# Kyaw-Thiha/animal-vision

Hardware: AMD Instinct MI355X
Metric: megapixels/sec per-frame pipeline (higher is better)
Workload: dtype f16

## Files before the change

animal-vision_amd/_lib.py:

```python
from __future__ import annotations

import ctypes
import os

_HERE = os.path.dirname(os.path.abspath(__file__))
LIB_PATH = os.path.join(_HERE, "libavx.so")

AVX_OK = 0
AVX_ERR_INVALID, AVX_ERR_NO_DEVICE, AVX_ERR_HIP, AVX_ERR_UNSUPPORTED, AVX_ERR_NOMEM = -1, -2, -3, -4, -5
AVX_COLOR_MATRIX, AVX_COLOR_CAT_MERGE = 0, 1
AVX_POST_NONE, AVX_POST_GAUSS, AVX_POST_ROWGAIN, AVX_POST_STREAK = 0, 1, 2, 3
AVX_MAX_KSIZE = 33
AVX_PIX_FMTS = {"yuv420p": 0, "nv12": 1, "yuv422p": 2, "yuv444p": 3, "gray": 4, "yuv420p10le": 5, "yuv422p10le": 6, "yuv444p10le": 7,
                "p010le": 8}
AVX_TRANSFERS = {"pq": 1, "hlg": 2}
AVX_TONEMAPS = {"clip": 0, "mobius": 1}


class AvxError(RuntimeError):
    def __init__(self, code: int, msg: str):
        super().__init__(f"libavx error {code}: {msg}")
        self.code = code


# ... 9 lines not shown
        ("ksize", ctypes.c_int32),
        ("taps_host", ctypes.POINTER(ctypes.c_double)),
        ("row_gain_host", ctypes.POINTER(ctypes.c_float)),
        ("row_gain_clamp", ctypes.c_int32),
        ("chroma_enable", ctypes.c_int32),
        ("chroma_keep", ctypes.c_float),
        ("variant", ctypes.c_int32),
        ("streak_rows_host", ctypes.POINTER(ctypes.c_float)),
        ("streak_stride", ctypes.c_int32),
        ("in_f32", ctypes.c_int32),
    ]


class DichromatLaunchInfo(ctypes.Structure):

    _fields_ = [("struct_size", ctypes.c_uint32)] + [
        (n, ctypes.c_int32)
        for n in ("family", "R", "f64", "NG", "spec", "sw", "nstrips", "ch", "nchunks", "xcd_remap", "narrow", "tuned_now", "grid", "per_cu")
    ]


AVX_LAUNCH_FAMILIES = ("none", "reference", "tiled", "march", "streak")


class HoneybeeDesc(ctypes.Structure):

    _fields_ = [
        ("struct_size", ctypes.c_uint32),
        ("source", ctypes.c_int32),
        ("rgb_matrix", ctypes.c_float * 9),
        ("hsi", ctypes.c_void_p),
        ("hsi_layout", ctypes.c_int32),
        ("hsi_dtype", ctypes.c_int32),
        ("bands", ctypes.c_int32),
        ("weights_host", ctypes.POINTER(ctypes.c_float)),
        ("adaptation", ctypes.c_int32),
        ("eps", ctypes.c_float),
        ("blur_ksize", ctypes.c_int32),
        ("blur_taps_host", ctypes.POINTER(ctypes.c_double)),
        ("mapping", ctypes.c_int32),
        ("custom_matrix", ctypes.c_float * 9),
        ("mixed_alpha", ctypes.c_float),
        ("out_float", ctypes.c_int32),
        ("catches", ctypes.c_void_p),
        ("catch_partials", ctypes.c_void_p),
        ("n_catch_partials", ctypes.c_int32),
    ]


_fp, _dp = ctypes.POINTER(ctypes.c_float), ctypes.POINTER(ctypes.c_double)


class MantisDesc(ctypes.Structure):

    _fields_ = [
        ("struct_size", ctypes.c_uint32),
        ("n_bands", ctypes.c_int32),
        ("band_matrix_host", _fp),
        ("band_lut_host", _fp),
        ("n_wavelengths", ctypes.c_int32),
        ("lobe_gains_host", _fp),
        ("lobe_denom", ctypes.c_float),
        ("band_weights_host", _fp),
        ("pano_new_w", ctypes.c_int32),
        ("hsi_small_h", ctypes.c_int32),
        ("hsi_small_w", ctypes.c_int32),
        ("red_keep", ctypes.c_float),
        ("haze", ctypes.c_float),
        ("haze_keep", ctypes.c_float),
        ("haze_tint", ctypes.c_float * 3),
        ("pre_soft_ksize", ctypes.c_int32),
        ("pre_soft_taps_host", _dp),
        ("cos2_global", ctypes.c_float),
        ("sin2_global", ctypes.c_float),
        ("orientation_mix", ctypes.c_float),
        ("pol_linear_strength", ctypes.c_float),
        ("pol_linear_gamma", ctypes.c_float),
        ("pol_circular_strength", ctypes.c_float),
        ("unsharp_ksize", ctypes.c_int32),
        ("unsharp_taps_host", _dp),
        ("unsharp_amount", ctypes.c_float),
        ("barcode_saturation", ctypes.c_float),
        ("barcode_opacity", ctypes.c_float),
        ("winner_take_most", ctypes.c_float),
        ("rows_host", _fp),
        ("scan_row_gain", ctypes.c_float),
        ("scan_ksize", ctypes.c_int32),
        ("scan_taps_host", _dp),
        ("periph_ksize", ctypes.c_int32),
        ("periph_taps_host", _dp),
        ("xx_host", _fp),
        ("yy_host", _fp),
        ("periph_radius", ctypes.c_float),
        ("periph_softness", ctypes.c_float),
        ("lin_hwc_in", ctypes.c_void_p),
        ("out_float", ctypes.c_int32),
    ]


class BandStackDesc(ctypes.Structure):

    _fields_ = [
        ("struct_size", ctypes.c_uint32),
        ("n_bands", ctypes.c_int32),
        ("band_matrix_host", _fp),
        ("n_wavelengths", ctypes.c_int32),
        ("lobe_gains_host", _fp),
        ("lobe_denom", ctypes.c_float),
        ("band_weights_host", _fp),
        ("small_h", ctypes.c_int32),
        ("small_w", ctypes.c_int32),
    ]


class GalleryTile(ctypes.Structure):

    _fields_ = [
        ("src", ctypes.c_void_p),
        ("dtype", ctypes.c_int32),
        ("H", ctypes.c_int32),
        ("W", ctypes.c_int32),
        ("h", ctypes.c_int32),
        ("w", ctypes.c_int32),
        ("seg_offset", ctypes.c_int32),
        ("seg_count", ctypes.c_int32),
    ]


class FrameMetricsRecord(ctypes.Structure):

    _fields_ = [("abs_hist", (ctypes.c_uint32 * 256) * 3), ("ssim", ctypes.c_double * 3)]


AVX_METRICS_MAX_FRAMES = 16


class PlaneMetricsRecord(ctypes.Structure):

    _fields_ = [("abs_hist", (ctypes.c_uint32 * 1024) * 3), ("ssim", ctypes.c_double * 3)]


assert ctypes.sizeof(PlaneMetricsRecord) == 3 * 1024 * 4 + 3 * 8


class MsSsimRecord(ctypes.Structure):

    _fields_ = [("cs", (ctypes.c_double * 5) * 3), ("ssim", (ctypes.c_double * 5) * 3)]


assert ctypes.sizeof(MsSsimRecord) == 240

class EwInsn(ctypes.Structure):
    _fields_ = [("op", ctypes.c_uint8), ("dst", ctypes.c_uint8), ("a", ctypes.c_uint8), ("b", ctypes.c_uint8), ("imm", ctypes.c_uint32)]


class EwPlane(ctypes.Structure):
    _fields_ = [("ptr", ctypes.c_void_p), ("stride", ctypes.c_int32), ("kind", ctypes.c_int32)]


class EwProgram(ctypes.Structure):

    _fields_ = [
        ("struct_size", ctypes.c_uint32),
        ("H", ctypes.c_int32),
        ("W", ctypes.c_int32),
        ("n_insn", ctypes.c_int32),
        ("insn_host", ctypes.POINTER(EwInsn)),
        ("n_planes", ctypes.c_int32),
        ("planes_host", ctypes.POINTER(EwPlane)),
        ("n_acc", ctypes.c_int32),
        ("acc_host", ctypes.POINTER(ctypes.c_int32)),
        ("scalars_dev", ctypes.c_void_p),
        ("n_scalars", ctypes.c_int32),
    ]


AVX_EW_MAX_INSN, AVX_EW_MAX_PLANES, AVX_EW_MAX_REGS, AVX_EW_MAX_ACC = 384, 24, 32, 16
AVX_EW_MAX_FRAMES = 16
_EW_OPS = ("CONST SCALAR LOAD STORE ADD SUB MUL DIV MIN MAX POW ATAN2 NEG ABS SQRT EXP LOG SIN COS FLOOR CEIL CLIP01 TANH "
           "LT LE GT GE EQ AND OR NOT SELECT ACCMIN ACCMAX ACCSUM").split()
EW = {name: i + 1 for i, name in enumerate(_EW_OPS)}
EW_PLANE = {"f32": 0, "u8": 1, "u8_lut": 2, "col": 3, "row": 4, "u8_enc": 5}
EW_ACC = {"min": 0, "max": 1, "sum": 2, "mean": 3}

AVX_MAP = {"falsecolor": 0, "custom_matrix": 1, "opponent": 2, "uv_purple_yellow": 3, "falsecolor_uv_mixed": 4}

if not os.path.exists(LIB_PATH):
    raise ImportError(
        f"{LIB_PATH} not found: build it with `python -c 'import __graft_entry__ as g; g.build()'` "
        "or `make -C animal-vision_amd/csrc` (hipcc --offload-arch=gfx950). There is no CPU fallback."
    )


def _preload_torch_hip_runtime():
    import importlib.util

    try:
        spec = importlib.util.find_spec("torch")
    except (ImportError, ValueError):
        spec = None
    if spec is None or not spec.submodule_search_locations:
        return
    cand = os.path.join(list(spec.submodule_search_locations)[0], "lib", "libamdhip64.so")
    if os.path.exists(cand):
        try:
            ctypes.CDLL(cand, mode=ctypes.RTLD_GLOBAL)
        except OSError:
            pass


_preload_torch_hip_runtime()
lib = ctypes.CDLL(LIB_PATH)

_vp, _i, _sz = ctypes.c_void_p, ctypes.c_int, ctypes.c_size_t
_SIGS = {
    "avx_abi_version": (_i, []),
    "avx_device_count": (_i, []),
    "avx_init": (_i, [_i, ctypes.POINTER(_vp)]),
    "avx_destroy": (None, [_vp]),
    "avx_last_error": (ctypes.c_char_p, [_vp]),
    "avx_malloc": (_i, [_vp, _sz, ctypes.POINTER(_vp)]),
    "avx_free": (_i, [_vp, _vp]),
    "avx_host_alloc": (_i, [_vp, _sz, ctypes.POINTER(_vp)]),
    "avx_host_free": (_i, [_vp, _vp]),
    "avx_memcpy_h2d": (_i, [_vp, _vp, _vp, _sz, _vp]),
    "avx_memcpy_d2h": (_i, [_vp, _vp, _vp, _sz, _vp]),
    "avx_memcpy_d2d": (_i, [_vp, _vp, _vp, _sz, _vp]),
    "avx_memset": (_i, [_vp, _vp, _i, _sz, _vp]),
    "avx_stream_create": (_i, [_vp, ctypes.POINTER(_vp)]),
    "avx_stream_destroy": (_i, [_vp, _vp]),
    "avx_sync": (_i, [_vp, _vp]),
    "avx_stream_wait": (_i, [_vp, _vp, _vp]),
    "avx_device_sync": (_i, [_vp]),
    "avx_timer_start": (_i, [_vp, _vp]),
    "avx_timer_stop": (_i, [_vp, _vp, ctypes.POINTER(ctypes.c_float)]),
    "avx_dichromat_u8": (_i, [_vp, _vp, _vp, _i, _i, _i, ctypes.POINTER(DichromatDesc), _vp]),
    "avx_dichromat_last_launch": (_i, [_vp, ctypes.POINTER(DichromatLaunchInfo)]),
    "avx_get_table": (_i, [_i, _vp, _sz]),
    "avx_percentile": (_i, [_vp, _vp, _sz, ctypes.c_double, ctypes.POINTER(ctypes.c_double), _vp]),
    "avx_spectral_integrate": (_i, [_vp, _vp, _i, _i, _i, _i, _i, _vp, _i, _vp, _vp, _vp]),
    "avx_plane_stats": (_i, [_vp, _vp, _i, _sz, _i, ctypes.c_float, _vp, _vp]),
    "avx_planes_gaussian_blur": (_i, [_vp, _vp, _vp, _i, _i, _i, _i, _vp, _i, _vp]),
    "avx_planes_gaussian_blur_batch": (_i, [_vp, _vp, _sz, _vp, _sz, _i, _i, _i, _i, _i, _vp, _i, _vp]),
    "avx_streak_planes_f32": (_i, [_vp, _vp, _vp, _i, _i, _vp, _i, _vp]),
    "avx_rgb_to_hsi_lobes": (_i, [_vp, _vp, _i, _i, _i, _i, _vp, ctypes.c_float, _vp, _vp]),
    "avx_honeybee_u8": (_i, [_vp, _vp, _vp, _i, _i, _i, ctypes.POINTER(HoneybeeDesc), _vp, _vp]),
    "avx_catch_planes_up": (_i, [_vp, _vp, _i, _i, _vp, _i, _i, _vp, ctypes.POINTER(ctypes.c_int), _vp]),
    "avx_uv_front_u8": (_i, [_vp, _vp, _i, _i, _i, _vp, _vp, _vp]),
    "avx_uv_front_u8_batch": (_i, [_vp, _vp, _i, _sz, _i, _i, _i, _vp, _sz, _vp, _sz, _vp]),
    "avx_panorama_warp_f32": (_i, [_vp, _vp, _i, _i, _i, _vp, _vp]),
    "avx_band_stack": (_i, [_vp, _vp, _i, _i, ctypes.POINTER(BandStackDesc), _vp, _vp]),
    "avx_band_stack_batch": (_i, [_vp, _vp, _i, _sz, _i, _i, ctypes.POINTER(BandStackDesc), _vp, _sz, _vp]),
    "avx_percentile_dev": (_i, [_vp, _vp, _sz, ctypes.c_double, _vp, _vp]),
    "avx_percentiles_dev": (_i, [_vp, _i, ctypes.POINTER(ctypes.c_void_p), ctypes.POINTER(ctypes.c_size_t), ctypes.POINTER(ctypes.c_double),
                                 ctypes.POINTER(ctypes.c_void_p), _vp]),
    "avx_ew_run": (_i, [_vp, ctypes.POINTER(EwProgram), _vp]),
    "avx_ew_run_batch": (_i, [_vp, ctypes.POINTER(EwProgram), _i, ctypes.POINTER(ctypes.c_size_t), _sz, _vp]),
    "avx_ew_spec_stats": (_i, [ctypes.POINTER(ctypes.c_ulonglong), ctypes.POINTER(ctypes.c_ulonglong)]),
    "avx_mantis_u8": (_i, [_vp, _vp, _vp, _vp, _i, _i, ctypes.POINTER(MantisDesc), _vp]),
    "avx_mantis_u8_batch": (_i, [_vp, _vp, _vp, _vp, _i, _i, _i, ctypes.POINTER(MantisDesc), _vp]),
    "avx_resize_hwc": (_i, [_vp, _vp, _i, _i, _i, _i, _vp, _i, _i, _i, _vp]),
    "avx_binocular_warp_u8": (_i, [_vp, _vp, _i, _i, _vp, _vp, _vp, _vp, _vp, _i, _i, _vp, _vp]),
    "avx_cat_wide_u8": (_i, [_vp, _vp, _vp, _i, _i, _i, ctypes.POINTER(DichromatDesc), _vp, _vp, _vp, _vp, _vp, _vp]),
    "avx_center_zoom_u8": (_i, [_vp, _vp, _vp, _i, _i, _i, _i, _i, _i, _i, _vp]),
    "avx_split_compose_u8": (_i, [_vp, _vp, _vp, _vp, _i, _i, _i, _vp]),
    "avx_draw_label_u8": (_i, [_vp, _vp, _i, _i, ctypes.POINTER(ctypes.c_int), _fp, _i, ctypes.c_float, ctypes.c_float, _i, _vp]),
    "avx_gallery_compose_u8": (_i, [_vp, ctypes.POINTER(GalleryTile), _i, _fp, _i, _i, _i, _i, ctypes.POINTER(ctypes.c_int), _vp, _i, _i, _vp]),
    "avx_wall_max_tiles": (_i, []),
    "avx_wall_layout_create": (_i, [_vp, _i, _i, _i, _i, _i, ctypes.POINTER(ctypes.c_int), ctypes.POINTER(ctypes.c_int), _fp, _i, _i, _i, _i,
                                    ctypes.POINTER(ctypes.c_int), ctypes.POINTER(_vp)]),
    "avx_wall_layout_destroy": (_i, [_vp, _vp]),
    "avx_wall_canvas_size": (_i, [_vp, ctypes.POINTER(_i), ctypes.POINTER(_i)]),
    "avx_wall_layout_info": (_i, [_vp, ctypes.POINTER(_i), ctypes.POINTER(_i), ctypes.POINTER(_i), ctypes.POINTER(_sz)]),
    "avx_wall_compose_u8": (_i, [_vp, _vp, ctypes.POINTER(_vp), _sz, _i, _vp, _sz, _vp]),
    "avx_i420_to_rgb_u8": (_i, [_vp, _vp, _vp, _i, _i, _i, _i, _i, _vp]),
    "avx_rgb_to_i420_u8": (_i, [_vp, _vp, _vp, _i, _i, _i, _i, _i, _vp]),
    "avx_yuv_coefficients": (_i, [_i, _i, ctypes.POINTER(ctypes.c_int), ctypes.POINTER(ctypes.c_int)]),
    "avx_yuv_coefficients_d": (_i, [_i, _i, _i, ctypes.POINTER(ctypes.c_int), ctypes.POINTER(ctypes.c_int)]),
    "avx_yuv_frame_size": (_sz, [_i, _i, _i]),
    "avx_yuv_to_rgb_u8": (_i, [_vp, _i, _vp, _vp, _i, _i, _i, _i, _i, _vp]),
    "avx_rgb_to_yuv_u8": (_i, [_vp, _i, _vp, _vp, _i, _i, _i, _i, _i, _vp]),
    "avx_yuv_hdr_to_rgb_u8": (_i, [_vp, _i, _vp, _vp, _i, _i, _i, _i, _i, _i, ctypes.c_double, ctypes.c_double, _vp]),
    "avx_yuv_to_rgb_scaled_u8": (_i, [_vp, _i, _vp, _vp, _i, _i, _i, _i, _i, _i, _i, _vp]),
    "avx_yuv_hdr_to_rgb_scaled_u8": (_i, [_vp, _i, _vp, _vp, _i, _i, _i, _i, _i, _i, _i, _i, ctypes.c_double, ctypes.c_double, _vp]),
    "avx_frame_metrics_u8": (_i, [_vp, _vp, _vp, _i, _i, _i, _i, _vp, _vp]),
    "avx_plane_metrics": (_i, [_vp, _i, _vp, _i, _vp, _i, _i, _i, _i, _vp, _vp]),
    "avx_frame_metrics_ms_u8": (_i, [_vp, _vp, _vp, _i, _i, _i, _vp, _vp, _vp]),
    "avx_remap_linear_planes": (_i, [_vp, _vp, _i, _i, _i, _vp, _vp, _vp, ctypes.c_float, _vp]),
    "avx_sobel3_plane": (_i, [_vp, _vp, _i, _i, _vp, _vp, _vp]),
    "avx_mst_gram": (_i, [_vp, _vp, _i, _sz, _i, _i, _vp, _vp, _vp, _vp]),
    "avx_mst_qkv_gram": (_i, [_vp, _vp, _vp, _sz, _i, _vp, _vp, _vp, _vp, _vp]),
    "avx_mst_qkv_gram16": (_i, [_vp, _vp, _vp, _sz, _i, _vp, _vp, _vp, _vp, _vp]),
    "avx_mst_ln_gemm_gelu": (_i, [_vp, _vp, _vp, _vp, ctypes.c_float, _vp, _sz, _i, _vp, _vp]),
    "avx_mst_convt2x2": (_i, [_vp, _vp, _vp, _vp, _vp, _i, _i, _i, _i, _vp]),
    "avx_mst_convt2x2_fuse": (_i, [_vp, _vp, _vp, _vp, _vp, _vp, _vp, _i, _i, _i, _i, _vp]),
    "avx_mst_posemb": (_i, [_vp, _vp, _vp, _vp, _vp, _vp, _vp, _i, _i, _i, _i, _vp]),
    "avx_mst_conv3x3_add": (_i, [_vp, _vp, _vp, _vp, _vp, _i, _i, _i, _i, _vp]),
    "avx_mst_attn_pack": (_i, [_vp, _vp, _vp, _vp, _vp, _vp, _i, _vp, _vp]),
    "avx_mst_rowgemm_add": (_i, [_vp, _vp, _vp, _vp, _vp, _vp, _vp, _sz, _i, _vp]),
    "avx_mst_conv_in_u8": (_i, [_vp, _vp, _i, _i, _i, _i, _i, _i, _vp, _vp, _vp]),
    "avx_mst_conv3x3_lds": (_i, [_vp, _vp, _vp, _vp, _vp, _i, _i, _i, _i, _vp]),
    "avx_mst_down4x4": (_i, [_vp, _vp, _vp, _vp, _i, _i, _i, _i, _vp]),
    "avx_mst_conv3x3_lds_gram": (_i, [_vp, _vp, _vp, _vp, _vp, _i, _i, _i, _vp, _vp, _vp, _vp, _vp]),
    "avx_mst_convt2x2_fuse_gram": (_i, [_vp, _vp, _vp, _vp, _vp, _vp, _vp, _i, _i, _i, _vp, _vp, _vp, _vp, _vp]),
    "avx_mst_attn_pack16": (_i, [_vp, _vp, _vp, _vp, _vp, _vp, _i, _vp, _vp]),
    "avx_mst_attn_pack_mx": (_i, [_vp, _vp, _vp, _vp, _vp, _vp, _i, _vp, _vp]),
    "avx_mst_attn_tail_mx": (_i, [_vp, _vp, _vp, _vp, _vp, _vp, _vp, _vp, _i, _i, _i, _i, _vp]),
    "avx_mst_attn_tail_sp": (_i, [_vp, _vp, _vp, _vp, _vp, _vp, _vp, _vp, _i, _i, _i, _i, _vp]),
    "avx_mst_attn_tail": (_i, [_vp, _vp, _vp, _vp, _vp, _vp, _vp, _vp, _i, _i, _i, _i, _vp]),
    "avx_mst_attn_tail_x": (_i, [_vp, _vp, _vp, _vp, _vp, _vp, _vp, _vp, _i, _i, _i, _i, _vp]),
    "avx_mst_ffn_fused": (_i, [_vp, _vp, _vp, _vp, ctypes.c_float, _vp, _vp, _vp, _vp, _i, _i, _i, _i, _vp]),
    "avx_mst_conv3x3_lds_spectral": (_i, [_vp, _vp, _vp, _vp, _i, _i, _i, _fp, _i, _i, _i, _i, _vp, _vp, ctypes.POINTER(ctypes.c_int), _vp]),
    "avx_mst_ffn_fused_mx": (_i, [_vp, _vp, _vp, _vp, ctypes.c_float, _vp, _vp, _vp, _vp, _i, _i, _i, _i, _vp]),
    "avx_mst_ffn_fused_sp": (_i, [_vp, _vp, _vp, _vp, ctypes.c_float, _vp, _vp, _vp, _vp, _i, _i, _i, _i, _vp]),
    "avx_mst_gelu_prescale": (ctypes.c_float, []),
    "avx_mst_tile_order": (_i, [_i, _i, _i, _i, _i, ctypes.POINTER(ctypes.c_longlong), _i, ctypes.POINTER(ctypes.c_int)]),
    "avx_mst_dw_gemm_add": (_i, [_vp, _vp, _vp, _vp, _vp, _vp, _i, _i, _i, _i, _vp]),
    "avx_dwconv3x3_nhwc_add": (_i, [_vp, _vp, _vp, _vp, _i, _i, _i, _i, _i, _vp, _vp, _vp]),
    "avx_dwconv3x3_nhwc": (_i, [_vp, _vp, _vp, _vp, _i, _i, _i, _i, _i, _i, _vp]),
    "avx_layernorm_rows": (_i, [_vp, _vp, _vp, _vp, _vp, _i, _sz, _i, ctypes.c_float, _vp]),
    "avx_layernorm_rows_grouped": (_i, [_vp, _vp, _vp, _vp, _vp, _i, _sz, _i, ctypes.c_float, _i, _i, _vp]),
}
for _name, (_res, _args) in _SIGS.items():
    _fn = getattr(lib, _name)
    _fn.restype = _res
    _fn.argtypes = _args

if lib.avx_abi_version() != 1:
    raise ImportError(f"libavx.so ABI {lib.avx_abi_version()} != 1 expected by this package: rebuild")
```

animal-vision_amd/csrc/mst_fused.hip:

```cpp
#include <hip/hip_fp16.h>

#include <cstdio>
#include <cstdlib>
#include <cstring>

#include "avx_internal.h"
#include "mst_common.h"
#include "mst_tile_order.h"

namespace {

typedef float float4_t __attribute__((ext_vector_type(4)));
#ifndef AVX_FFN32_GM2
#define AVX_FFN32_GM2 1
#endif
constexpr int kFT = 512;
constexpr int TS = 16;
constexpr int HS = TS + 2;
#ifndef AVX_FFN_TH
#define AVX_FFN_TH 16
#endif
constexpr int kFfnTH = AVX_FFN_TH;
static_assert(kFfnTH == 14 || kFfnTH == 16, "FeedForward tile rows");
constexpr int kFfnNGRP = (HS * (kFfnTH + 2) + 31) / 32;
// ... 614 lines not shown
}

template <int C, int MINW>
int launch_attn_tail(avx_ctx* ctx, const void* v, const void* x, const void* mpack, const void* taps1, const void* taps2, const float* bias, void* out, int B,
                     int H, int W, hipStream_t s, const void* wvpack) {
    constexpr int PP = C * 2 + 16, VRP = (VS * PP + 255) / 256 * 256, MRP = VRP;
    const size_t lds = (size_t)2 * VS * VRP + (size_t)2 * 9 * C * 2 + sizeof(float) * C;
    (void)MRP;
    const long total = (long)B * ((H + TS - 1) / TS) * ((W + TS - 1) / TS);
    const long cap = (long)ctx->num_cus * (MINW / 2);
    auto k = k_mst_attn_tail<C, MINW>;
    AVX_HIP(ctx, hipFuncSetAttribute((const void*)k, hipFuncAttributeMaxDynamicSharedMemorySize, (int)lds));
    hipLaunchKernelGGL(k, dim3((unsigned)(total < cap ? total : cap)), dim3(kFT), lds, s, (const __half*)v, (const __half*)x, (const uint4*)mpack,
                       (const __half*)taps1, (const __half*)taps2, bias, (__half*)out, B, H, W, (const uint4*)wvpack);
    AVX_HIP(ctx, hipGetLastError());
    return AVX_OK;
}


template <int C, int TR, int MINW, bool STAMP = false, int NW = 8, bool DWS = false>
__global__ __launch_bounds__(64 * NW, MINW) void k_mst_attn_tail_mx(const __half* __restrict__ x , const uint4* __restrict__ wvpack ,
                                                                const uint4* __restrict__ mpack , const uint4* __restrict__ dw1 ,
                                                                const uint4* __restrict__ dw2 , const float* __restrict__ bias ,
                                                                __half* __restrict__ out, int B, int H, int W, unsigned long long* __restrict__ stamps , int order ) {
    constexpr int TW = 14, VW = 18, VR = TR + 4, MR = TR + 2, NOCT = C / 8, NK = C / 16, NT = C / 32, NS = C / 16, LNV = C / 16;
    constexpr int PP = C * 2 + 16, RP = (VW * PP + 255) / 256 * 256, MP = 16 * PP;
    constexpr int NTHR = 64 * NW, NG = (VR * VW + 31) / 32, NGW = (NG + NW - 1) / NW;
    constexpr int WPO = NOCT >= NW ? 1 : NW / NOCT, OPW = NOCT > NW ? NOCT / NW : 1;
    constexpr int NOUT = (TR / 2) / WPO, NMID = NOUT + 1;
    static_assert(C == 32 || C == 64 || C == 128, "31-, 62- or 124-channel blocks");
    static_assert(MP % 256 == 0 && (NW % NOCT == 0 || NOCT % NW == 0) && (TR / 2) % WPO == 0, "pitches / row split");
    extern __shared__ __align__(16) unsigned char smem[];
    unsigned char* vt = smem;
    unsigned char* mt = vt + (size_t)VR * RP;
    uint4* wvl = reinterpret_cast<uint4*>(mt + (size_t)MR * MP);
    constexpr bool STASH = C <= 64 && NW == 8;
    unsigned char* xs = reinterpret_cast<unsigned char*>(wvl + NT * NS * 64);
    const int tid = threadIdx.x, lane = tid & 63, wave = tid >> 6, p = lane & 31, h = lane >> 5, n16 = lane & 15, q = lane >> 4;
    unsigned long long seg[8] = {0, 0, 0, 0, 0, 0, 0, 0}, tlast = 0;
    auto stamp = [&](int kk) {
        if constexpr (STAMP) {
            const unsigned long long now = __builtin_readcyclecounter();
            seg[kk] += now - tlast;
            tlast = now;
        }
    };
    if constexpr (STAMP) tlast = __builtin_readcyclecounter();
    const int tx = (W + TW - 1) / TW, ty = (H + TR - 1) / TR;
    for (int i = tid; i < NT * NS * 64; i += NTHR) wvl[i] = wvpack[i];
    const int o = wave % NOCT, rpo = (wave / NOCT) * NOUT;
    half8_t a1[3], a2[3], am[NK];
    float bs[4];
    auto load_frags = [&](int oc) {
#pragma unroll
        for (int i = 0; i < 3; ++i) {
            a1[i] = dw_frag<DWS>(dw1 + ((size_t)oc * 3 + i) * 64 + lane, i);
            a2[i] = dw_frag<DWS>(dw2 + ((size_t)oc * 3 + i) * 64 + lane, i);
        }
#pragma unroll
        for (int t2 = 0; t2 < NK; ++t2) am[t2] = __builtin_bit_cast(half8_t, mpack[((size_t)oc * NK + t2) * 64 + lane]);
#pragma unroll
        for (int j = 0; j < 4; ++j) bs[j] = bias ? bias[8 * oc + 4 * (q & 1) + j] : 0.f;
    };
    load_frags(o);
#pragma unroll
    for (int i = 0; i < 3; ++i) asm volatile("" ::"v"(a1[i]), "v"(a2[i]));
#pragma unroll
    for (int t2 = 0; t2 < NK; ++t2) asm volatile("" ::"v"(am[t2]));
    asm volatile("" ::"v"(bs[0]), "v"(bs[1]), "v"(bs[2]), "v"(bs[3]));
    const unsigned char* rbB = vt + (size_t)q * RP + (size_t)n16 * PP + 16 * o;
    unsigned char* wbB = mt + (size_t)(q >> 1) * MP + (size_t)n16 * PP + 16 * o + 8 * (q & 1);
    const unsigned char* rbC = mt + (size_t)q * MP + (size_t)n16 * PP + 16 * o;
    const unsigned char* rbG = vt + (size_t)(2 + (q & 1)) * RP + (size_t)(n16 + 2) * PP + 16 * (q >> 1);
    unsigned f_rel[NGW];
    int v_dst[NGW], p_row[NGW], p_col[NGW];
#pragma unroll
    for (int gi = 0; gi < NGW; ++gi) {
        const int g = wave + NW * gi, qq = 32 * g + p, qc = qq < VR * VW ? qq : VR * VW - 1;
        p_row[gi] = qc / VW; p_col[gi] = qc % VW;
        f_rel[gi] = (unsigned)((p_row[gi] * W + p_col[gi]) * C + h * (C / 2)) * 2u;
        v_dst[gi] = (g < NG && qq < VR * VW) ? p_row[gi] * RP + p_col[gi] * PP + 32 * h : -1;
    }
    uint4 pre[NGW][LNV];
    auto fetch = [&](const Tile& t) {
        if (t.y0 >= 2 && t.y0 + VR - 2 <= H && t.x0 >= 2 && t.x0 + VW - 2 <= W) {
            const char* origin = reinterpret_cast<const char*>(x + ((t.b * H + t.y0 - 2) * (size_t)W + t.x0 - 2) * C);
#pragma unroll
            for (int gi = 0; gi < NGW; ++gi) {
                if (wave + NW * gi >= NG) break;
                unsigned of = f_rel[gi];
                asm volatile("" : "+v"(of));
                const uint4* src = reinterpret_cast<const uint4*>(origin + of);
#pragma unroll
                for (int v = 0; v < LNV; ++v) pre[gi][v] = src[v];
            }
            return;
        }
#pragma unroll
        for (int gi = 0; gi < NGW; ++gi) {
            if (wave + NW * gi >= NG) break;
            const int yy = t.y0 - 2 + p_row[gi], xx = t.x0 - 2 + p_col[gi];
            const bool ok = yy >= 0 && yy < H && xx >= 0 && xx < W;
            const int yc = yy < 0 ? 0 : (yy >= H ? H - 1 : yy), xc = xx < 0 ? 0 : (xx >= W ? W - 1 : xx);
            const uint4* src = reinterpret_cast<const uint4*>(x + ((t.b * H + yc) * (size_t)W + xc) * C + h * (C / 2));
#pragma unroll
            for (int v = 0; v < LNV; ++v) {
                uint4 r = src[v];
                r.x = ok ? r.x : 0u; r.y = ok ? r.y : 0u; r.z = ok ? r.z : 0u; r.w = ok ? r.w : 0u;
                pre[gi][v] = r;
            }
        }
    };
    TileWalk ahead;
    ahead.init(blockIdx.x, gridDim.x, B, ty, tx, order);
    if (!ahead.live) return;
    Tile t = tile_at(ahead, TW, TR);
    ahead.advance();
    fetch(t);
    __syncthreads();
    for (;;) {
#pragma unroll
        for (int gi = 0; gi < NGW; ++gi) {
            if (wave + NW * gi >= NG) break;
#pragma unroll
            for (int nt = 0; nt < NT; ++nt) {
                float16_t d;
#pragma unroll
                for (int vv = 0; vv < 16; ++vv) d[vv] = 0.f;
#pragma unroll
                for (int s2 = 0; s2 < NS; ++s2) d = mfma16(__builtin_bit_cast(half8_t, wvl[(nt * NS + s2) * 64 + lane]), __builtin_bit_cast(half8_t, pre[gi][s2]), d);
                if (v_dst[gi] >= 0) {
                    half8_t w0, w1;
#pragma unroll
                    for (int vv = 0; vv < 8; ++vv) { w0[vv] = (_Float16)d[vv]; w1[vv] = (_Float16)d[8 + vv]; }
                    reinterpret_cast<uint4*>(vt + v_dst[gi] + 64 * nt)[0] = __builtin_bit_cast(uint4, w0);
                    reinterpret_cast<uint4*>(vt + v_dst[gi] + 64 * nt)[1] = __builtin_bit_cast(uint4, w1);
                }
            }
            if constexpr (STASH) {
                const unsigned sr = (unsigned)(p_row[gi] - 2), sc = (unsigned)(p_col[gi] - 2);
                if (v_dst[gi] >= 0 && sr < (unsigned)TR && sc < (unsigned)TW) {
                    unsigned char* dst = xs + (sr * TW + sc) * PP + h * C;
#pragma unroll
                    for (int v = 0; v < LNV; ++v) *reinterpret_cast<uint4*>(dst + 16 * v) = pre[gi][v];
                }
            }
        }
        stamp(0);
        __syncthreads();
        stamp(1);
        if (ahead.live) fetch(tile_at(ahead, TW, TR));
#pragma unroll
        for (int kk = 0; kk < OPW; ++kk) {
        const int oc = o + NW * kk, ob = 16 * NW * kk;
        if constexpr (OPW > 1) load_frags(oc);
        uint2 xr[STASH ? 1 : NOUT];
        const int yo0 = t.y0 + 2 * rpo + (q >> 1), xo = t.x0 + n16;
        const bool livex = n16 < TW && xo < W;
        const size_t e0 = ((t.b * H + (yo0 < H ? yo0 : 0)) * (size_t)W + (livex ? xo : 0)) * C + 8 * oc + 4 * (q & 1), estep = (size_t)2 * W * C;
        auto live = [&](int u) { return livex && yo0 + 2 * u < H; };
        if constexpr (!STASH) {
#pragma unroll
            for (int u = 0; u < NOUT; ++u) xr[u] = live(u) ? *reinterpret_cast<const uint2*>(x + e0 + u * estep) : uint2{0, 0};
        }
        {
            const bool mid_inside = t.y0 >= 1 && t.y0 + MR - 1 <= H && t.x0 >= 1 && t.x0 + 15 <= W;
            uint4 bq[3];
            auto rd = [&](int u) {
#pragma unroll
                for (int i = 0; i < 3; ++i) bq[i] = *reinterpret_cast<const uint4*>(rbB + (size_t)(2 * (rpo + u)) * RP + i * PP + ob);
            };
            auto finish = [&](int u, float4_t a) {
                float2_t gp[2] = {float2_t{a[0], a[1]}, float2_t{a[2], a[3]}};
                if constexpr (C >= 64) gelu_mx<2>(gp);
                else { float2_t g0[1] = {gp[0]}, g1[1] = {gp[1]}; gelu_mx<1>(g0); gelu_mx<1>(g1); gp[0] = g0[0]; gp[1] = g1[0]; }
                uint2 ov = uint2{pack_f16(gp[0].x, gp[0].y), pack_f16(gp[1].x, gp[1].y)};
                if (!mid_inside) {
                    const int yy = t.y0 - 1 + 2 * (rpo + u) + (q >> 1), xx = t.x0 - 1 + n16;
                    const unsigned keep = (yy >= 0 && yy < H && xx >= 0 && xx < W) ? 0xffffffffu : 0u;
                    ov.x &= keep; ov.y &= keep;
                }
                *reinterpret_cast<uint2*>(wbB + (size_t)(2 * (rpo + u)) * MP + ob) = ov;
            };
            rd(0);
            float4_t prev = {0.f, 0.f, 0.f, 0.f};
#pragma unroll
            for (int u = 0; u < NMID; ++u) {
                const float4_t acc = dw_unit<DWS>(a1, bq);
                if (u + 1 < NMID) rd(u + 1);
                __builtin_amdgcn_sched_barrier(0);
                if (u > 0) finish(u - 1, prev);
                __builtin_amdgcn_sched_barrier(0);
                prev = acc;
            }
            finish(NMID - 1, prev);
        }
        stamp(2);
        {
            uint4 bq[3], bg[NK];
            uint2 xn = uint2{0, 0};
            const unsigned char* rbX = xs + (size_t)((q >> 1) * TW + n16) * PP + 16 * o + 8 * (q & 1);
            auto rd = [&](int u) {
#pragma unroll
                for (int i = 0; i < 3; ++i) bq[i] = *reinterpret_cast<const uint4*>(rbC + (size_t)(2 * (rpo + u)) * MP + i * PP + ob);
#pragma unroll
                for (int t2 = 0; t2 < NK; ++t2) bg[t2] = *reinterpret_cast<const uint4*>(rbG + (size_t)(2 * (rpo + u)) * RP + 32 * t2);
                if constexpr (STASH) xn = *reinterpret_cast<const uint2*>(rbX + (size_t)(2 * (rpo + u)) * TW * PP);
            };
            auto finish = [&](int u, float4_t acc, uint2 xu) {
                if (live(u)) {
                    constexpr unsigned kOnes = 0x3c003c00u;
                    float s0 = acc[0] + bs[0], s1 = acc[1] + bs[1], s2 = acc[2] + bs[2], s3 = acc[3] + bs[3];
                    fma_mix_lo(s0, xu.x, kOnes); fma_mix_hi(s1, xu.x, kOnes);
                    fma_mix_lo(s2, xu.y, kOnes); fma_mix_hi(s3, xu.y, kOnes);
                    *reinterpret_cast<uint2*>(out + e0 + u * estep) = uint2{pack_f16(s0, s1), pack_f16(s2, s3)};
                }
            };
            rd(0);
#ifndef AVX_TAIL_PIPE2
#define AVX_TAIL_PIPE2 1
#endif
            if constexpr (STASH && (AVX_TAIL_PIPE2 == 2 || (AVX_TAIL_PIPE2 == 1 && C == 64))) {
                float4_t prev = {0.f, 0.f, 0.f, 0.f};
                uint2 xp = uint2{0, 0};
#pragma unroll
                for (int u = 0; u < NOUT; ++u) {
                    const uint2 xu = xn;
                    float4_t acc = dw_unit<DWS>(a2, bq);
#pragma unroll
                    for (int t2 = 0; t2 < NK; ++t2) acc = __builtin_amdgcn_mfma_f32_16x16x32_f16(am[t2], __builtin_bit_cast(half8_t, bg[t2]), acc, 0, 0, 0);
                    if (u + 1 < NOUT) rd(u + 1);
                    __builtin_amdgcn_sched_barrier(0);
                    if (u > 0) finish(u - 1, prev, xp);
                    __builtin_amdgcn_sched_barrier(0);
                    prev = acc; xp = xu;
                }
                finish(NOUT - 1, prev, xp);
            } else {
#pragma unroll
                for (int u = 0; u < NOUT; ++u) {
                    const uint2 xu = STASH ? xn : xr[STASH ? 0 : u];
                    float4_t acc = dw_unit<DWS>(a2, bq);
#pragma unroll
                    for (int t2 = 0; t2 < NK; ++t2) acc = __builtin_amdgcn_mfma_f32_16x16x32_f16(am[t2], __builtin_bit_cast(half8_t, bg[t2]), acc, 0, 0, 0);
                    if (u + 1 < NOUT) rd(u + 1);
                    finish(u, acc, xu);
                }
            }
        }
        }
        stamp(3);
        if (!ahead.live) break;
        t = tile_at(ahead, TW, TR);
        ahead.advance();
        __syncthreads();
        stamp(4);
    }
    if constexpr (STAMP) {
        if (lane == 0 && stamps)
#pragma unroll
            for (int kk = 0; kk < 8; ++kk) stamps[((size_t)blockIdx.x * NW + wave) * 8 + kk] = seg[kk];
    }
}

template <int C, int TR, int MINW, int NW = 8, bool DWS = false>
int launch_attn_tail_mx(avx_ctx* ctx, const void* x, const void* wvpack, const void* mpack, const void* dw1, const void* dw2, const float* bias, void* out, int B, int H, int W,
                        hipStream_t s) {
    constexpr int PP = C * 2 + 16, RP = (18 * PP + 255) / 256 * 256;
    const size_t lds = (size_t)(TR + 4) * RP + (size_t)(TR + 2) * 16 * PP + (size_t)(C / 32) * (C / 16) * 1024 + ((C <= 64 && NW == 8) ? (size_t)(TR * 14 + 2) * PP : 0) ;
    const long total = (long)B * ((H + TR - 1) / TR) * ((W + 13) / 14);
    const long cap = (long)ctx->num_cus * (NW == 16 ? 1 : MINW / 2);
    AVX_REQUIRE(ctx, total <= 0x7fffffffl, "avx_mst_attn_tail_mx: 2^31 tiles or more");
    const unsigned blocks = (unsigned)(total < cap ? total : cap);
    if (getenv("AVX_TAIL_STAMPS")) {
        auto ks = k_mst_attn_tail_mx<C, TR, MINW, true, NW, DWS>;
        unsigned long long* d_st = nullptr;
        const size_t n = (size_t)blocks * NW * 8;
        AVX_HIP(ctx, hipMalloc((void**)&d_st, n * sizeof(unsigned long long)));
        AVX_HIP(ctx, hipFuncSetAttribute((const void*)ks, hipFuncAttributeMaxDynamicSharedMemorySize, (int)lds));
        hipLaunchKernelGGL(ks, dim3(blocks), dim3(64 * NW), lds, s, (const __half*)x, (const uint4*)wvpack, (const uint4*)mpack, (const uint4*)dw1, (const uint4*)dw2, bias, (__half*)out, B, H, W, d_st, mst_tile_order());
        AVX_HIP(ctx, hipStreamSynchronize(s));
        unsigned long long* h_st = (unsigned long long*)malloc(n * sizeof(unsigned long long));
        AVX_HIP(ctx, hipMemcpy(h_st, d_st, n * sizeof(unsigned long long), hipMemcpyDeviceToHost));
        double tot[8] = {0}, all = 0;
        for (size_t i = 0; i < n; ++i) { tot[i & 7] += (double)h_st[i]; all += (double)h_st[i]; }
        const char* nm[8] = {"v from x", "bar1", "conv1+gelu", "conv2+proj+store", "bar2", "-", "-", "-"};
        fprintf(stderr, "[tail stamps C=%d] %u blocks, %ld tiles, mean cycles per wave %.0f:", C, blocks, total, all / (blocks * (double)NW));
        for (int k2 = 0; k2 < 8; ++k2) fprintf(stderr, "  %s %.1f%%", nm[k2], 100 * tot[k2] / all);
        fprintf(stderr, "\n");
        free(h_st);
        (void)hipFree(d_st);
        return AVX_OK;
    }
    auto k = k_mst_attn_tail_mx<C, TR, MINW, false, NW, DWS>;
    AVX_HIP(ctx, hipFuncSetAttribute((const void*)k, hipFuncAttributeMaxDynamicSharedMemorySize, (int)lds));
    hipLaunchKernelGGL(k, dim3(blocks), dim3(64 * NW), lds, s, (const __half*)x, (const uint4*)wvpack, (const uint4*)mpack, (const uint4*)dw1,
                       (const uint4*)dw2, bias, (__half*)out, B, H, W, (unsigned long long*)nullptr, mst_tile_order());
    AVX_HIP(ctx, hipGetLastError());
    return AVX_OK;
}


struct SpecStat3 { float mn, mx; double sum; };
template <int MINW, bool GRAM, bool SPEC = false>
__global__ __launch_bounds__(kFT, MINW) void k_mst_conv3x3_lds(const __half* __restrict__ x , const uint4* __restrict__ wpack ,
                                                               const __half* __restrict__ add , __half* __restrict__ out, int B, int H, int W,
                                                               const uint4* __restrict__ wqk , float* __restrict__ partial ,
                                                               const float* __restrict__ specw = nullptr ,
                                                               float* __restrict__ planes = nullptr , SpecStat3* __restrict__ spart = nullptr ,
                                                               int crop_t = 0, int crop_l = 0, int Hc = 0, int Wc = 0, int order = AVX_TILE_ORDER_RASTER ) {
    constexpr int C = 32, PP = C * 2 + 16, RP = (HS * PP + 255) / 256 * 256, NFILL = (HS * HS * 4 + kFT - 1) / kFT;
    __shared__ __align__(16) unsigned char xt[HS * RP];
    __shared__ uint4 wl[18 * 64];
    const int tid = threadIdx.x, lane = tid & 63, wave = tid >> 6, p = lane & 31, h = lane >> 5;
    for (int i = tid; i < 18 * 64; i += kFT) wl[i] = wpack[i];
    __shared__ uint4 wq[GRAM ? 4 * 64 : 1];
    float16_t G;
    float nq = 0.f, nk = 0.f;
    if constexpr (GRAM) {
        if (tid < 4 * 64) wq[tid] = wqk[tid];
#pragma unroll
        for (int v = 0; v < 16; ++v) G[v] = 0.f;
    }
    float smn[3] = {3.4e38f, 3.4e38f, 3.4e38f}, smx[3] = {-3.4e38f, -3.4e38f, -3.4e38f};
    double ssum[3] = {0.0, 0.0, 0.0};
    const int tx = (W + TS - 1) / TS, ty = (H + TS - 1) / TS;
    uint4 pre[NFILL];
    unsigned f_rel[NFILL];
#pragma unroll
    for (int k = 0; k < NFILL; ++k) {
        const int it = tid + k * kFT, itc = it < HS * HS * 4 ? it : 0, q = itc >> 2, part = itc & 3;
        f_rel[k] = (unsigned)(((q / HS) * W + q % HS) * C + 8 * part) * 2u;
    }
    auto fetch = [&](const Tile& t) {
        if (t.y0 >= 1 && t.y0 + HS - 1 <= H && t.x0 >= 1 && t.x0 + HS - 1 <= W) {
            const char* origin = reinterpret_cast<const char*>(x + ((t.b * H + t.y0 - 1) * (size_t)W + t.x0 - 1) * C);
#pragma unroll
            for (int k = 0; k < NFILL; ++k) {
                unsigned o = f_rel[k];
                asm volatile("" : "+v"(o));
                pre[k] = *reinterpret_cast<const uint4*>(origin + o);
            }
            return;
        }
#pragma unroll
        for (int k = 0; k < NFILL; ++k) {
            const int it = tid + k * kFT, q = it >> 2, part = it & 3;
            const int yy = t.y0 - 1 + q / HS, xx = t.x0 - 1 + q % HS;
            const bool ok = it < HS * HS * 4 && yy >= 0 && yy < H && xx >= 0 && xx < W;
            const int yc = yy < 0 ? 0 : (yy >= H ? H - 1 : yy), xc = xx < 0 ? 0 : (xx >= W ? W - 1 : xx);
            uint4 r = *reinterpret_cast<const uint4*>(x + ((t.b * H + yc) * (size_t)W + xc) * C + 8 * part);
            r.x = ok ? r.x : 0u; r.y = ok ? r.y : 0u; r.z = ok ? r.z : 0u; r.w = ok ? r.w : 0u;
            pre[k] = r;
        }
    };
    TileWalk ahead;
    ahead.init(blockIdx.x, gridDim.x, B, ty, tx, (GRAM || SPEC) ? (int)AVX_TILE_ORDER_RASTER : order);
    if (!ahead.live) return;
    Tile t = tile_at(ahead, TS, TS);
    ahead.advance();
    fetch(t);
    for (;;) {
#pragma unroll
        for (int k = 0; k < NFILL; ++k) {
            const int it = tid + k * kFT, q = it >> 2, part = it & 3;
            if (it < HS * HS * 4) *reinterpret_cast<uint4*>(xt + (size_t)(q / HS) * RP + (size_t)(q % HS) * PP + 16 * part) = pre[k];
        }
        __syncthreads();
        if (ahead.live) fetch(tile_at(ahead, TS, TS));
        {
            const int r = 2 * wave + (p >> 4), c = p & 15;
            const int yo = t.y0 + r, xo = t.x0 + c;
            const bool live = yo < H && xo < W;
            const size_t off = ((t.b * H + (live ? yo : 0)) * (size_t)W + (live ? xo : 0)) * C + 16 * h;
            uint4 ar[2] = {uint4{0, 0, 0, 0}, uint4{0, 0, 0, 0}};
            if (add) { ar[0] = reinterpret_cast<const uint4*>(add + off)[0]; ar[1] = reinterpret_cast<const uint4*>(add + off)[1]; }
            float16_t d;
#pragma unroll
            for (int v = 0; v < 16; ++v) d[v] = 0.f;
            const unsigned char* src = xt + (size_t)r * RP + (size_t)c * PP + 16 * h;
#pragma unroll
            for (int tap = 0; tap < 9; ++tap)
#pragma unroll
                for (int s2 = 0; s2 < 2; ++s2)
                    d = mfma16(__builtin_bit_cast(half8_t, wl[(2 * tap + s2) * 64 + lane]), __builtin_bit_cast(half8_t, *reinterpret_cast<const uint4*>(src + (size_t)(tap / 3) * RP + (size_t)(tap % 3) * PP + 32 * s2)), d);
            half8_t o0, o1;
            {
                const half8_t r0 = __builtin_bit_cast(half8_t, ar[0]), r1 = __builtin_bit_cast(half8_t, ar[1]);
#pragma unroll
                for (int v = 0; v < 8; ++v) { o0[v] = (_Float16)(d[v] + (float)r0[v]); o1[v] = (_Float16)(d[8 + v] + (float)r1[v]); }
            }
            if constexpr (SPEC) {
                float a3[3] = {0.f, 0.f, 0.f};
                auto chain = [&]() {
#pragma unroll
                    for (int j = 0; j < 16; ++j) {
                        const float v = (float)(j < 8 ? o0[j] : o1[j - 8]);
                        const float* wb = specw + (16 * h + j) * 4;
#pragma unroll
                        for (int k = 0; k < 3; ++k) a3[k] = __builtin_fmaf(v, wb[k], a3[k]);
                    }
                };
                if (h == 0) chain();
#pragma unroll
                for (int k = 0; k < 3; ++k) { const float lo = __shfl_xor(a3[k], 32); a3[k] = h ? lo : a3[k]; }
                if (h == 1) chain();
                const int yc = yo - crop_t, xc = xo - crop_l;
                if (h == 1 && live && yc >= 0 && yc < Hc && xc >= 0 && xc < Wc) {
#pragma unroll
                    for (int k = 0; k < 3; ++k) {
                        planes[(size_t)k * Hc * Wc + (size_t)yc * Wc + xc] = a3[k];
                        smn[k] = fminf(smn[k], a3[k]); smx[k] = fmaxf(smx[k], a3[k]); ssum[k] += (double)a3[k];
                    }
                }
            } else if (live) {
                reinterpret_cast<uint4*>(out + off)[0] = __builtin_bit_cast(uint4, o0);
                reinterpret_cast<uint4*>(out + off)[1] = __builtin_bit_cast(uint4, o1);
            }
            if constexpr (GRAM) {
                if (!live) { o0 = half8_t{0, 0, 0, 0, 0, 0, 0, 0}; o1 = o0; }
                float16_t dq, dk;
#pragma unroll
                for (int v = 0; v < 16; ++v) { dq[v] = 0.f; dk[v] = 0.f; }
                dq = mfma16(o0, __builtin_bit_cast(half8_t, wq[0 * 64 + lane]), dq);
                dq = mfma16(o1, __builtin_bit_cast(half8_t, wq[1 * 64 + lane]), dq);
                dk = mfma16(o0, __builtin_bit_cast(half8_t, wq[2 * 64 + lane]), dk);
                dk = mfma16(o1, __builtin_bit_cast(half8_t, wq[3 * 64 + lane]), dk);
                unsigned aq[8], ak[8];
#pragma unroll
                for (int j = 0; j < 8; ++j) {
                    aq[j] = pack_f16(dq[2 * j], dq[2 * j + 1]);
                    ak[j] = pack_f16(dk[2 * j], dk[2 * j + 1]);
                    fma_mix_lo(nq, aq[j], aq[j]); fma_mix_hi(nq, aq[j], aq[j]);
                    fma_mix_lo(nk, ak[j], ak[j]); fma_mix_hi(nk, ak[j], ak[j]);
                }
#pragma unroll
                for (int b2 = 0; b2 < 2; ++b2)
                    G = mfma16(__builtin_bit_cast(half8_t, uint4{ak[4 * b2], ak[4 * b2 + 1], ak[4 * b2 + 2], ak[4 * b2 + 3]}),
                               __builtin_bit_cast(half8_t, uint4{aq[4 * b2], aq[4 * b2 + 1], aq[4 * b2 + 2], aq[4 * b2 + 3]}), G);
            }
        }
        if (!ahead.live) break;
        t = tile_at(ahead, TS, TS);
        ahead.advance();
        __syncthreads();
    }
    if constexpr (SPEC) {
        __syncthreads();
        float* redf = reinterpret_cast<float*>(xt);
        double* redd = reinterpret_cast<double*>(xt + 256);
#pragma unroll
        for (int k = 0; k < 3; ++k) {
            float a = smn[k], b2 = smx[k];
            double c2 = ssum[k];
#pragma unroll
            for (int o = 32; o > 0; o >>= 1) { a = fminf(a, __shfl_xor(a, o)); b2 = fmaxf(b2, __shfl_xor(b2, o)); c2 += __shfl_xor(c2, o); }
            if (lane == 0) { redf[(wave * 3 + k) * 2] = a; redf[(wave * 3 + k) * 2 + 1] = b2; redd[wave * 3 + k] = c2; }
        }
        __syncthreads();
        if (tid < 3) {
            float a = 3.4e38f, b2 = -3.4e38f;
            double c2 = 0.0;
            for (int w8 = 0; w8 < 8; ++w8) { a = fminf(a, redf[(w8 * 3 + tid) * 2]); b2 = fmaxf(b2, redf[(w8 * 3 + tid) * 2 + 1]); c2 += redd[w8 * 3 + tid]; }
            spart[(size_t)blockIdx.x * 3 + tid] = SpecStat3{a, b2, c2};
        }
    }
    if constexpr (GRAM) {
        static_assert(sizeof(xt) >= sizeof(float) * 4 * 34 * 32, "the halo tile's LDS holds four waves' results at a time");
        float* red = reinterpret_cast<float*>(xt);
        const float sq = nq + __shfl_xor(nq, 32), sk = nk + __shfl_xor(nk, 32);
        float sum[3] = {0.f, 0.f, 0.f};
#pragma unroll
        for (int half = 0; half < 2; ++half) {
            __syncthreads();
            if ((wave >> 2) == half) {
                float* mine = red + (size_t)(wave & 3) * 34 * 32;
#pragma unroll
                for (int v = 0; v < 16; ++v) mine[(8 * (v / 4) + 4 * h + (v % 4)) * 32 + p] = G[v];
                if (h == 0) { mine[32 * 32 + p] = sq; mine[33 * 32 + p] = sk; }
            }
            __syncthreads();
#pragma unroll
            for (int q = 0; q < 3; ++q) {
                const int i = tid + q * kFT;
                if (i < 34 * 32)
#pragma unroll
                    for (int w4 = 0; w4 < 4; ++w4) sum[q] += red[(size_t)w4 * 34 * 32 + i];
            }
        }
#pragma unroll
        for (int q = 0; q < 3; ++q) {
            const int i = tid + q * kFT;
            if (i < 34 * 32) partial[(size_t)blockIdx.x * 34 * 32 + i] = sum[q];
        }
    }
}


template <int C>
struct DownGeo {
    static constexpr int OH = C == 32 ? 8 : 4, OW = 16, IH = 2 * OH + 2, IW = 2 * OW + 2;
    static constexpr int NP = C / 8;
    static constexpr int RPS = IW * NP + (C == 32 ? 2 : 4);
    static constexpr int NI = ((IH * RPS + 63) / 64 + 7) / 8 * 8;
    static constexpr int PER_WAVE = NI / 8, BUF = NI * 1024, NBUF = C == 32 ? 3 : 2, GROUPS = OH / 2;
    static constexpr int PART = C == 32 ? 0 : 2 * 4 * 4096;
    __device__ static int swz(int col) { return C == 32 ? (col >> 2) & 3 : (col >> 1) & 7; }
};
#pragma clang diagnostic push
#pragma clang diagnostic ignored "-Winline-asm"
__device__ __forceinline__ void lds_dma16(const void* g, unsigned lds_base ) {
    asm volatile("s_mov_b32 m0, %0\n\ts_nop 0\n\tglobal_load_lds_dwordx4 %1, off" ::"s"(__builtin_amdgcn_readfirstlane(lds_base)), "v"(g) : "memory", "m0");
}
__device__ __forceinline__ void lds_dma16(const void* base , unsigned ofs, unsigned lds_base) {
    asm volatile("s_mov_b32 m0, %0\n\ts_nop 0\n\tglobal_load_lds_dwordx4 %1, %2" ::"s"(__builtin_amdgcn_readfirstlane(lds_base)), "v"(ofs), "s"(base) : "memory", "m0");
}
#pragma clang diagnostic pop
template <int C>
__global__ __launch_bounds__(kFT, 2) void k_mst_down4x4_dma(const __half* __restrict__ x , const uint4* __restrict__ wpack ,
                                                            __half* __restrict__ out , const void* __restrict__ zero, int B, int H, int W, int order ) {
    using G = DownGeo<C>;
    constexpr int CO = 2 * C, NT = CO / 32, KS = C / 16;
    __shared__ __align__(1024) unsigned char lds[G::NBUF * G::BUF + G::PART];
    const int tid = threadIdx.x, lane = tid & 63, wave = __builtin_amdgcn_readfirstlane(tid >> 6) , p = lane & 31, h = lane >> 5;
    const int g0 = C == 32 ? wave & 3 : 0, nt = C == 32 ? wave >> 2 : wave & 3, kh = C == 32 ? 0 : wave >> 2;
    half8_t wf[32];
#pragma unroll
    for (int i = 0; i < 32; ++i) {
        const int tap = C == 32 ? i >> 1 : 8 * kh + (i >> 2), s2 = C == 32 ? i & 1 : i & 3;
        wf[i] = __builtin_bit_cast(half8_t, wpack[((size_t)(tap * NT + nt) * KS + s2) * 64 + lane]);
    }
    const int Ho = H / 2, Wo = W / 2;
    const int tx = (Wo + G::OW - 1) / G::OW, ty = (Ho + G::OH - 1) / G::OH;
    struct T2 { int ox0, oy0, b; };
    auto tile_at = [&](const TileWalk& w) { return T2{w.xi * G::OW, w.yi * G::OH, w.b}; };
    int rel[G::PER_WAVE], rc[G::PER_WAVE];
#pragma unroll
    for (int k = 0; k < G::PER_WAVE; ++k) {
        const int L = (wave + 8 * k) * 64 + lane, row = L / G::RPS, rem = L - row * G::RPS, col = rem / G::NP, j = (rem - col * G::NP) ^ G::swz(col);
        const bool inside = row < G::IH && col < G::IW;
        rel[k] = inside ? (row * W + col) * (C * 2) + 16 * j : 0;
        rc[k] = inside ? row << 8 | col : -1;
    }
    const unsigned lds0 = __builtin_amdgcn_readfirstlane((unsigned)(size_t)(__attribute__((address_space(3))) unsigned char*)lds);
    auto fill = [&](const TileWalk& w, int slot) {
        const bool exists = w.live;
        const T2 t = tile_at(w);
        const int y0 = 2 * t.oy0 - 1, x0 = 2 * t.ox0 - 1;
        const char* origin = reinterpret_cast<const char*>(x) + (((long)t.b * H + y0) * W + x0) * (long)(C * 2);
        const unsigned lb = lds0 + slot * G::BUF + wave * 1024;
        if (exists && y0 >= 0 && y0 + G::IH <= H && x0 >= 0 && x0 + G::IW <= W) {
#pragma unroll
            for (int k = 0; k < G::PER_WAVE; ++k) lds_dma16(origin , (unsigned)rel[k], lb + k * 8192);
        } else {
#pragma unroll
            for (int k = 0; k < G::PER_WAVE; ++k) {
                const int yy = y0 + (rc[k] >> 8), xx = x0 + (rc[k] & 255);
                const bool ok = exists && rc[k] >= 0 && yy >= 0 && yy < H && xx >= 0 && xx < W;
                lds_dma16(ok ? (const void*)(origin + rel[k]) : zero, lb + k * 8192);
            }
        }
    };
    TileWalk walk, look;
    walk.init(blockIdx.x, gridDim.x, B, ty, tx, order);
    if (!walk.live) return;
    look = walk;
#pragma unroll
    for (int a = 0; a < G::NBUF - 1; ++a) { fill(look, a); look.advance(); }
    const int c2 = 2 * (p & 15);
    int colofs[4];
#pragma unroll
    for (int kx = 0; kx < 4; ++kx) colofs[kx] = (c2 + kx) * G::NP;
    int slot = 0, plain_stores = 0;
    for (;;) {
        if (plain_stores == G::NBUF - 1 && (C == 32 || kh == 0)) asm volatile("s_waitcnt vmcnt(%0)" ::"n"(G::PER_WAVE * (G::NBUF - 2) + 2 * (C == 32 ? 1 : G::GROUPS) * (G::NBUF - 1)) : "memory");
        else asm volatile("s_waitcnt vmcnt(%0)" ::"n"(G::PER_WAVE * (G::NBUF - 2)) : "memory");
        __syncthreads();
        {
            int nslot = slot + G::NBUF - 1;
            nslot -= nslot >= G::NBUF ? G::NBUF : 0;
            fill(look, nslot);
            look.advance();
        }
        const T2 t = tile_at(walk);
        const bool whole = t.oy0 + G::OH <= Ho && t.ox0 + G::OW <= Wo;
        const unsigned char* bt = lds + slot * G::BUF;
#pragma unroll 1
        for (int g = g0; g < (C == 32 ? g0 + 1 : G::GROUPS); ++g) {
            const int r = 2 * g + (p >> 4);
            float16_t d, d1;
#pragma unroll
            for (int v = 0; v < 16; ++v) d[v] = 0.f, d1[v] = 0.f;
            const unsigned char* src = bt + (size_t)(2 * r) * (G::RPS * 16);
            auto frag = [&](int i) {
                const int tap = C == 32 ? i >> 1 : 8 * kh + (i >> 2), s2 = C == 32 ? i & 1 : i & 3, ky = tap >> 2, kx = tap & 3;
                return *reinterpret_cast<const uint4*>(src + ky * (G::RPS * 16) + (colofs[kx] + ((2 * s2 + h) ^ G::swz(c2 + kx))) * 16);
            };
            constexpr int AHEAD = 6;
            uint4 bq[AHEAD];
#pragma unroll
            for (int i = 0; i < AHEAD; ++i) bq[i] = frag(i);
#pragma unroll
            for (int i = 0; i < 32; ++i) {
                if (i & 1) d1 = mfma16(wf[i], __builtin_bit_cast(half8_t, bq[i % AHEAD]), d1);
                else d = mfma16(wf[i], __builtin_bit_cast(half8_t, bq[i % AHEAD]), d);
                if (i + AHEAD < 32) bq[i % AHEAD] = frag(i + AHEAD);
            }
            __builtin_amdgcn_sched_group_barrier(0x100, AHEAD, 0);
#pragma unroll
            for (int i = 0; i < 32; ++i) {
                __builtin_amdgcn_sched_group_barrier(0x008, 1, 0);
                if (i + AHEAD < 32) __builtin_amdgcn_sched_group_barrier(0x100, 1, 0);
            }
#pragma unroll
            for (int v = 0; v < 16; ++v) d[v] += d1[v];
            if constexpr (C == 64) {
                float4* part = reinterpret_cast<float4*>(lds + G::NBUF * G::BUF + ((g & 1) * 4 + nt) * 4096);
                if (kh == 1) {
#pragma unroll
                    for (int v4 = 0; v4 < 4; ++v4) part[v4 * 64 + lane] = float4{d[4 * v4], d[4 * v4 + 1], d[4 * v4 + 2], d[4 * v4 + 3]};
                }
                __syncthreads();
                if (kh == 1) continue;
#pragma unroll
                for (int v4 = 0; v4 < 4; ++v4) {
                    const float4 q = part[v4 * 64 + lane];
                    d[4 * v4] += q.x; d[4 * v4 + 1] += q.y; d[4 * v4 + 2] += q.z; d[4 * v4 + 3] += q.w;
                }
            }
            const int yo = t.oy0 + r, xo = t.ox0 + (p & 15);
            half8_t o0, o1;
#pragma unroll
            for (int v = 0; v < 8; ++v) { o0[v] = (_Float16)d[v]; o1[v] = (_Float16)d[8 + v]; }
            __half* dst = out + (((size_t)t.b * Ho + yo) * Wo + xo) * CO + 32 * nt + 16 * h;
            if (whole) {
                reinterpret_cast<uint4*>(dst)[0] = __builtin_bit_cast(uint4, o0);
                reinterpret_cast<uint4*>(dst)[1] = __builtin_bit_cast(uint4, o1);
            } else if (yo < Ho && xo < Wo) {
                reinterpret_cast<uint4*>(dst)[0] = __builtin_bit_cast(uint4, o0);
                reinterpret_cast<uint4*>(dst)[1] = __builtin_bit_cast(uint4, o1);
            }
        }
        plain_stores = whole ? (plain_stores < G::NBUF - 1 ? plain_stores + 1 : plain_stores) : 0;
        walk.advance();
        if (!walk.live) break;
        slot = slot + 1 == G::NBUF ? 0 : slot + 1;
    }
    asm volatile("s_waitcnt vmcnt(0)" ::: "memory");
}

__global__ __launch_bounds__(256) void k_mst_conv_in_u8(const uint8_t* __restrict__ frame , const float* __restrict__ w ,
                                                        __half* __restrict__ out , int H, int W, int pt, int pl, int Hp, int Wp) {
    __shared__ __align__(16) float wl[27 * 32];
    for (int i = threadIdx.x; i < 27 * 32; i += 256) wl[i] = w[i];
    __syncthreads();
    const size_t total = (size_t)Hp * Wp;
    for (size_t i = (size_t)blockIdx.x * 256 + threadIdx.x; i < total; i += (size_t)gridDim.x * 256) {
        const int y = (int)(i / Wp), x = (int)(i - (size_t)y * Wp);
        float in[27];
#pragma unroll
        for (int t = 0; t < 9; ++t) {
            const int yy = y + t / 3 - 1, xx = x + t % 3 - 1;
            const bool ok = yy >= 0 && yy < Hp && xx >= 0 && xx < Wp;
            int sy = (ok ? yy : 0) - pt, sx = (ok ? xx : 0) - pl;
            sy = sy < 0 ? -sy : (sy >= H ? 2 * (H - 1) - sy : sy);
            sx = sx < 0 ? -sx : (sx >= W ? 2 * (W - 1) - sx : sx);
            const uint8_t* q = frame + ((size_t)sy * W + sx) * 3;
#pragma unroll
            for (int c = 0; c < 3; ++c) in[3 * t + c] = ok ? (float)(_Float16)((float)q[c] / 255.0f) : 0.f;
        }
        uint4* dst = reinterpret_cast<uint4*>(out + i * 32);
#pragma unroll 1
        for (int v = 0; v < 4; ++v) {
            float acc[8];
#pragma unroll
            for (int j = 0; j < 8; ++j) acc[j] = 0.f;
#pragma unroll
            for (int k = 0; k < 27; ++k) {
                const float4 wa = *reinterpret_cast<const float4*>(wl + k * 32 + 8 * v), wb = *reinterpret_cast<const float4*>(wl + k * 32 + 8 * v + 4);
                acc[0] = __builtin_fmaf(in[k], wa.x, acc[0]); acc[1] = __builtin_fmaf(in[k], wa.y, acc[1]);
                acc[2] = __builtin_fmaf(in[k], wa.z, acc[2]); acc[3] = __builtin_fmaf(in[k], wa.w, acc[3]);
                acc[4] = __builtin_fmaf(in[k], wb.x, acc[4]); acc[5] = __builtin_fmaf(in[k], wb.y, acc[5]);
                acc[6] = __builtin_fmaf(in[k], wb.z, acc[6]); acc[7] = __builtin_fmaf(in[k], wb.w, acc[7]);
            }
            half8_t o8;
#pragma unroll
            for (int j = 0; j < 8; ++j) o8[j] = (_Float16)acc[j];
            dst[v] = __builtin_bit_cast(uint4, o8);
        }
    }
}

__global__ __launch_bounds__(256) void k_mst_conv_in_u8_mfma(const uint8_t* __restrict__ frame , const float* __restrict__ w ,
                                                             __half* __restrict__ out , int H, int W, int pt, int pl, int Hp, int Wp) {
    const int lane = threadIdx.x & 63, p = lane & 31, h = lane >> 5;
    const int col = 16 * ((p % 8) / 4) + 4 * (p / 8) + p % 4;
    const int tap0 = 5 * h, ntap = 5 - h;
    half8_t af[2];
#pragma unroll
    for (int s = 0; s < 2; ++s)
#pragma unroll
        for (int j = 0; j < 8; ++j) {
            const int q = 8 * s + j, k = 3 * tap0 + q;
            af[s][j] = q < 3 * ntap ? (_Float16)w[k * 32 + col] : (_Float16)0.f;
        }
    int dy[5], dx[5];
#pragma unroll
    for (int t = 0; t < 5; ++t) {
        const int tap = tap0 + (t < ntap ? t : 0);
        dy[t] = tap / 3 - 1; dx[t] = tap % 3 - 1;
    }
    const size_t total = (size_t)Hp * Wp, ngroups = (total + 31) / 32;
    const float inv255 = 1.0f / 255.0f;
    for (size_t g = (size_t)blockIdx.x * 4 + (threadIdx.x >> 6); g < ngroups; g += (size_t)gridDim.x * 4) {
        const size_t i = g * 32 + p, ic = i < total ? i : total - 1;
        const int y = (int)(ic / Wp), x = (int)(ic - (size_t)y * Wp);
        float v[16];
        v[15] = 0.f;
#pragma unroll
        for (int t = 0; t < 5; ++t) {
            const int yy = y + dy[t], xx = x + dx[t];
            const bool ok = t < ntap && yy >= 0 && yy < Hp && xx >= 0 && xx < Wp;
            int sy = (ok ? yy : 0) - pt, sx = (ok ? xx : 0) - pl;
            sy = sy < 0 ? -sy : (sy >= H ? 2 * (H - 1) - sy : sy);
            sx = sx < 0 ? -sx : (sx >= W ? 2 * (W - 1) - sx : sx);
            const uint8_t* q = frame + ((size_t)sy * W + sx) * 3;
#pragma unroll
            for (int c = 0; c < 3; ++c) v[3 * t + c] = ok ? (float)q[c] * inv255 : 0.f;
        }
        const half8_t b0 = __builtin_bit_cast(half8_t, uint4{pack_f16(v[0], v[1]), pack_f16(v[2], v[3]), pack_f16(v[4], v[5]), pack_f16(v[6], v[7])});
        const half8_t b1 = __builtin_bit_cast(half8_t, uint4{pack_f16(v[8], v[9]), pack_f16(v[10], v[11]), pack_f16(v[12], v[13]), pack_f16(v[14], v[15])});
        float16_t d;
#pragma unroll
        for (int vv = 0; vv < 16; ++vv) d[vv] = 0.f;
        d = mfma16(af[0], b0, d);
        d = mfma16(af[1], b1, d);
        if (i < total) {
            unsigned o[8];
#pragma unroll
            for (int vv = 0; vv < 8; ++vv) o[vv] = pack_f16(d[2 * vv], d[2 * vv + 1]);
            reinterpret_cast<uint4*>(out + i * 32 + 16 * h)[0] = uint4{o[0], o[1], o[2], o[3]};
            reinterpret_cast<uint4*>(out + i * 32 + 16 * h)[1] = uint4{o[4], o[5], o[6], o[7]};
        }
    }
}

}

static int ffn_fused_launch(avx_ctx* ctx, const void* x, const float* gamma, const float* beta, float eps, const void* w1pack, const void* taps_9xhid, const void* dwpack,
                            const void* w2pack, void* out, int B, int H, int W, int C, void* stream, bool sparse = false);

extern "C" float avx_mst_gelu_prescale(void) { return kGeluPrescale; }

extern "C" int avx_mst_tile_order(int frames, int ty, int tx, int nwg, int raster, long long* visit, int steps_cap, int* steps_out) {
    if (frames <= 0 || ty <= 0 || tx <= 0 || nwg <= 0 || (visit && steps_cap <= 0) || (long long)frames * ty * tx > 0x7fffffffll) return AVX_ERR_INVALID;
    int most = 0;
    for (int wg = 0; wg < nwg; ++wg) {
        TileWalk wk;
        wk.init((unsigned)wg, (unsigned)nwg, frames, ty, tx, raster ? AVX_TILE_ORDER_RASTER : AVX_TILE_ORDER_XCD);
        int k = 0;
        for (; wk.live; wk.advance(), ++k)
            if (visit && k < steps_cap) visit[(size_t)wg * steps_cap + k] = ((long long)wk.b * ty + wk.yi) * tx + wk.xi;
        if (visit)
            for (int r = k; r < steps_cap; ++r) visit[(size_t)wg * steps_cap + r] = -1;
        most = k > most ? k : most;
    }
    if (steps_out) *steps_out = most;
    return AVX_OK;
}

extern "C" int avx_mst_ffn_fused(avx_ctx* ctx, const void* x, const float* gamma, const float* beta, float eps, const void* w1pack, const void* taps_9xhid,
                                 const void* w2pack, void* out, int B, int H, int W, int C, void* stream) {
    if (!ctx) return AVX_ERR_INVALID;
    AVX_REQUIRE(ctx, taps_9xhid, "avx_mst_ffn_fused: NULL pointer");
    return ffn_fused_launch(ctx, x, gamma, beta, eps, w1pack, taps_9xhid, nullptr, w2pack, out, B, H, W, C, stream);
}

extern "C" int avx_mst_ffn_fused_mx(avx_ctx* ctx, const void* x, const float* gamma, const float* beta, float eps, const void* w1pack, const void* dwpack,
                                    const void* w2pack, void* out, int B, int H, int W, int C, void* stream) {
    if (!ctx) return AVX_ERR_INVALID;
    AVX_REQUIRE(ctx, dwpack && (((uintptr_t)dwpack) & 15u) == 0, "avx_mst_ffn_fused_mx: dwpack NULL or not 16-byte aligned");
    return ffn_fused_launch(ctx, x, gamma, beta, eps, w1pack, nullptr, dwpack, w2pack, out, B, H, W, C, stream);
}

extern "C" int avx_mst_ffn_fused_sp(avx_ctx* ctx, const void* x, const float* gamma, const float* beta, float eps, const void* w1pack, const void* dwpack,
                                    const void* w2pack, void* out, int B, int H, int W, int C, void* stream) {
    if (!ctx) return AVX_ERR_INVALID;
    AVX_REQUIRE(ctx, dwpack && (((uintptr_t)dwpack) & 15u) == 0, "avx_mst_ffn_fused_sp: dwpack NULL or not 16-byte aligned");
    return ffn_fused_launch(ctx, x, gamma, beta, eps, w1pack, nullptr, dwpack, w2pack, out, B, H, W, C, stream, true);
}

static int ffn_fused_launch(avx_ctx* ctx, const void* x, const float* gamma, const float* beta, float eps, const void* w1pack, const void* taps_9xhid, const void* dwpack,
                            const void* w2pack, void* out, int B, int H, int W, int C, void* stream, bool sparse) {
    AVX_REQUIRE(ctx, x && gamma && beta && w1pack && w2pack && out && B > 0 && H > 0 && W > 0, "avx_mst_ffn_fused: NULL pointer or empty tensor");
    AVX_REQUIRE(ctx, C == 32 || C == 64 || C == 128, "avx_mst_ffn_fused: C=%d (32, 64 or 128: 31-channel groups stored 32 wide)", C);
    AVX_REQUIRE(ctx, ((((uintptr_t)x | (uintptr_t)w1pack | (uintptr_t)w2pack | (uintptr_t)out | (uintptr_t)taps_9xhid)) & 15u) == 0,
                "avx_mst_ffn_fused: pointers must be 16-byte aligned");
    AVX_REQUIRE(ctx, x != out, "avx_mst_ffn_fused: neighbouring tiles read each other's halo: the output cannot be the input");
    AVX_HIP(ctx, hipSetDevice(ctx->device));
    hipStream_t s = avx_pick_stream(ctx, stream);
    const long total = (long)B * ((H + kFfnTH - 1) / kFfnTH) * ((W + TS - 1) / TS);
    const char* hp = getenv("AVX_MST_FFN_HPASS");
    const bool small = C == 32 && !(hp && atoi(hp) == 128);
    const int hpass = (small || C == 128) ? 64 : 128, hpitch = hpass * 2 + 16, rpitch = (HS * hpitch + 255) / 256 * 256;
    const long cap = (long)ctx->num_cus * (small ? 2 : 1);
    const bool nw16 = C == 64 && dwpack && !(getenv("AVX_MST_FFN_NW") && atoi(getenv("AVX_MST_FFN_NW")) == 8);
    const size_t lds = (size_t)kFfnNGRP * 32 * (C * 2 + 16) + (size_t)(kFfnTH + 2) * rpitch + (dwpack ? 0 : (size_t)9 * 4 * C * 2) + sizeof(float) * 2 * C + (nw16 ? (size_t)(C / 32) * (hpass / 16) * 1024 : 0);
    AVX_REQUIRE(ctx, total <= 0x7fffffffl, "avx_mst_ffn_fused: 2^31 tiles or more");
    const dim3 grid((unsigned)(total < cap ? total : cap));
    const int order = mst_tile_order();
#define AVX_FFN1S(CV, HP, MW, DW, NWV, SP)                                                                                                       \
    {                                                                                                                                            \
        auto k = k_mst_ffn_fused<CV, HP, MW, DW, false, NWV, SP>;                                                                                \
        AVX_HIP(ctx, hipFuncSetAttribute((const void*)k, hipFuncAttributeMaxDynamicSharedMemorySize, (int)lds));                                 \
        hipLaunchKernelGGL(k, grid, dim3(64 * NWV), lds, s, (const __half*)x, gamma, beta, eps, (const uint4*)w1pack, (const __half*)taps_9xhid, \
                           (const uint4*)w2pack, (__half*)out, B, H, W, (const uint4*)dwpack, (unsigned long long*)nullptr, order);              \
    }
#define AVX_FFN1(CV, HP, MW, DW, NWV) AVX_FFN1S(CV, HP, MW, DW, NWV, false)
#define AVX_FFN(CV, HP, MW) { if (dwpack && sparse) AVX_FFN1S(CV, HP, MW, true, 8, true) else if (dwpack) AVX_FFN1(CV, HP, MW, true, 8) else AVX_FFN1(CV, HP, MW, false, 8) }
    if (dwpack && getenv("AVX_FFN_STAMPS") && ((C == 32 && small) || C == 64 || C == 128)) {
        unsigned long long* d_st = nullptr;
        const int nwv = nw16 ? 16 : 8;
        const size_t n = (size_t)grid.x * nwv * 8;
        AVX_HIP(ctx, hipMalloc((void**)&d_st, n * sizeof(unsigned long long)));
#define AVX_FFN_ST1(CV, HP, MW, NWV, SP)                                                                                                         \
    {                                                                                                                                            \
        auto k = k_mst_ffn_fused<CV, HP, MW, true, true, NWV, SP>;                                                                               \
        AVX_HIP(ctx, hipFuncSetAttribute((const void*)k, hipFuncAttributeMaxDynamicSharedMemorySize, (int)lds));                                 \
        hipLaunchKernelGGL(k, grid, dim3(64 * NWV), lds, s, (const __half*)x, gamma, beta, eps, (const uint4*)w1pack, (const __half*)taps_9xhid, \
                           (const uint4*)w2pack, (__half*)out, B, H, W, (const uint4*)dwpack, d_st, order);                                      \
    }
#define AVX_FFN_ST(CV, HP, MW, NWV) { if (sparse) AVX_FFN_ST1(CV, HP, MW, NWV, true) else AVX_FFN_ST1(CV, HP, MW, NWV, false) }
        if (C == 32) AVX_FFN_ST(32, 64, 4, 8) else if (nw16) AVX_FFN_ST(64, 128, 1, 16) else if (C == 64) AVX_FFN_ST(64, 128, 2, 8) else AVX_FFN_ST(128, 64, 2, 8)
#undef AVX_FFN_ST
#undef AVX_FFN_ST1
        AVX_HIP(ctx, hipStreamSynchronize(s));
        unsigned long long* h_st = (unsigned long long*)malloc(n * sizeof(unsigned long long));
        AVX_HIP(ctx, hipMemcpy(h_st, d_st, n * sizeof(unsigned long long), hipMemcpyDeviceToHost));
        double tot[8] = {0}, w0[8] = {0}, w7[8] = {0};
        for (size_t i = 0; i < n; ++i) { tot[i & 7] += (double)h_st[i]; if (((i >> 3) % nwv) == 0) w0[i & 7] += (double)h_st[i]; if (((i >> 3) % nwv) == (size_t)nwv - 1) w7[i & 7] += (double)h_st[i]; }
        double all = 0;
        for (int k2 = 0; k2 < 8; ++k2) all += tot[k2];
        fprintf(stderr, "[ffn stamps C=%d] %u blocks x %d waves, mean cycles per wave %.0f; share per segment (all waves | first wave | last wave): ", C, grid.x, nwv, all / (grid.x * (double)nwv));
        const char* nm[8] = {"bar1", "phase1", "bar2", "phase2a", "bar3", "phase2b", "epilogue", "ln+fetch"};
        for (int k2 = 0; k2 < 8; ++k2) fprintf(stderr, "%s %.1f%% | %.1f%% | %.1f%%  ", nm[k2], 100 * tot[k2] / all, 100 * w0[k2] * nwv / all, 100 * w7[k2] * nwv / all);
        fprintf(stderr, "\n");
        free(h_st);
        (void)hipFree(d_st);
    } else if (C == 32 && small) AVX_FFN(32, 64, 4) else if (C == 32) AVX_FFN(32, 128, 2)
    else if (nw16 && sparse) AVX_FFN1S(64, 128, 1, true, 16, true)
    else if (nw16) AVX_FFN1(64, 128, 1, true, 16)
    else if (C == 64) AVX_FFN(64, 128, 2) else AVX_FFN(128, 64, 2)
#undef AVX_FFN
#undef AVX_FFN1
#undef AVX_FFN1S
    AVX_HIP(ctx, hipGetLastError());
    return AVX_OK;
}

extern "C" int avx_mst_attn_tail(avx_ctx* ctx, const void* v, const void* x, const void* mpack16, const void* taps1_9xc, const void* taps2_9xc, const float* bias,
                                 void* out, int B, int H, int W, int C, void* stream) {
    if (!ctx) return AVX_ERR_INVALID;
    AVX_REQUIRE(ctx, v && x && mpack16 && taps1_9xc && taps2_9xc && out && B > 0 && H > 0 && W > 0, "avx_mst_attn_tail: NULL pointer or empty tensor");
    AVX_REQUIRE(ctx, C == 32 || C == 64, "avx_mst_attn_tail: C=%d (32 or 64)", C);
    AVX_REQUIRE(ctx, ((((uintptr_t)v | (uintptr_t)x | (uintptr_t)mpack16 | (uintptr_t)out | (uintptr_t)taps1_9xc | (uintptr_t)taps2_9xc)) & 15u) == 0,
                "avx_mst_attn_tail: pointers must be 16-byte aligned");
    AVX_REQUIRE(ctx, v != out, "avx_mst_attn_tail: tiles read their neighbours' rows of v: the output cannot be v (it may be x)");
    AVX_HIP(ctx, hipSetDevice(ctx->device));
    hipStream_t s = avx_pick_stream(ctx, stream);
    if (C == 32) return launch_attn_tail<32, 4>(ctx, v, x, mpack16, taps1_9xc, taps2_9xc, bias, out, B, H, W, s, nullptr);
    return launch_attn_tail<64, 2>(ctx, v, x, mpack16, taps1_9xc, taps2_9xc, bias, out, B, H, W, s, nullptr);
}

extern "C" int avx_mst_attn_tail_x(avx_ctx* ctx, const void* x, const void* wvpack16, const void* mpack16, const void* taps1_9xc, const void* taps2_9xc,
                                   const float* bias, void* out, int B, int H, int W, int C, void* stream) {
    if (!ctx) return AVX_ERR_INVALID;
    AVX_REQUIRE(ctx, x && wvpack16 && mpack16 && taps1_9xc && taps2_9xc && out && B > 0 && H > 0 && W > 0, "avx_mst_attn_tail_x: NULL pointer or empty tensor");
    AVX_REQUIRE(ctx, C == 32 || C == 64, "avx_mst_attn_tail_x: C=%d (32 or 64)", C);
    AVX_REQUIRE(ctx, ((((uintptr_t)x | (uintptr_t)wvpack16 | (uintptr_t)mpack16 | (uintptr_t)out | (uintptr_t)taps1_9xc | (uintptr_t)taps2_9xc)) & 15u) == 0,
                "avx_mst_attn_tail_x: pointers must be 16-byte aligned");
    AVX_REQUIRE(ctx, x != out, "avx_mst_attn_tail_x: tiles read their neighbours' rows of x: the output cannot be x");
    AVX_HIP(ctx, hipSetDevice(ctx->device));
    hipStream_t s = avx_pick_stream(ctx, stream);
    if (C == 32) return launch_attn_tail<32, 4>(ctx, x, x, mpack16, taps1_9xc, taps2_9xc, bias, out, B, H, W, s, wvpack16);
    return launch_attn_tail<64, 2>(ctx, x, x, mpack16, taps1_9xc, taps2_9xc, bias, out, B, H, W, s, wvpack16);
}

template <bool DWS>
static int attn_tail_mx_launch(avx_ctx* ctx, const void* x, const void* wvpack16, const void* mpack_mx, const void* dw1pack, const void* dw2pack, const float* bias, void* out,
                               int B, int H, int W, int C, void* stream) {
    AVX_REQUIRE(ctx, x && wvpack16 && mpack_mx && dw1pack && dw2pack && out && B > 0 && H > 0 && W > 0, "avx_mst_attn_tail_mx: NULL pointer or empty tensor");
    AVX_REQUIRE(ctx, C == 32 || C == 64 || C == 128, "avx_mst_attn_tail_mx: C=%d (32, 64 or 128)", C);
    AVX_REQUIRE(ctx, ((((uintptr_t)x | (uintptr_t)wvpack16 | (uintptr_t)mpack_mx | (uintptr_t)out | (uintptr_t)dw1pack | (uintptr_t)dw2pack)) & 15u) == 0,
                "avx_mst_attn_tail_mx: pointers must be 16-byte aligned");
    AVX_REQUIRE(ctx, x != out, "avx_mst_attn_tail_mx: tiles read their neighbours' rows of x: the output cannot be x");
    AVX_HIP(ctx, hipSetDevice(ctx->device));
    hipStream_t s = avx_pick_stream(ctx, stream);
    if (C == 32) return launch_attn_tail_mx<32, 16, 4, 8, DWS>(ctx, x, wvpack16, mpack_mx, dw1pack, dw2pack, bias, out, B, H, W, s);
    if (C == 128) return launch_attn_tail_mx<128, 8, 2, 8, DWS>(ctx, x, wvpack16, mpack_mx, dw1pack, dw2pack, bias, out, B, H, W, s);
    if (getenv("AVX_MST_TAIL_NW") && atoi(getenv("AVX_MST_TAIL_NW")) == 16) return launch_attn_tail_mx<64, 16, 1, 16, DWS>(ctx, x, wvpack16, mpack_mx, dw1pack, dw2pack, bias, out, B, H, W, s);
    return launch_attn_tail_mx<64, 16, 2, 8, DWS>(ctx, x, wvpack16, mpack_mx, dw1pack, dw2pack, bias, out, B, H, W, s);
}
extern "C" int avx_mst_attn_tail_mx(avx_ctx* ctx, const void* x, const void* wvpack16, const void* mpack_mx, const void* dw1pack, const void* dw2pack,
                                    const float* bias, void* out, int B, int H, int W, int C, void* stream) {
    if (!ctx) return AVX_ERR_INVALID;
    return attn_tail_mx_launch<false>(ctx, x, wvpack16, mpack_mx, dw1pack, dw2pack, bias, out, B, H, W, C, stream);
}
extern "C" int avx_mst_attn_tail_sp(avx_ctx* ctx, const void* x, const void* wvpack16, const void* mpack_mx, const void* dw1pack, const void* dw2pack,
                                    const float* bias, void* out, int B, int H, int W, int C, void* stream) {
    if (!ctx) return AVX_ERR_INVALID;
    return attn_tail_mx_launch<true>(ctx, x, wvpack16, mpack_mx, dw1pack, dw2pack, bias, out, B, H, W, C, stream);
}

extern "C" int avx_mst_conv3x3_lds(avx_ctx* ctx, const void* x, const void* wpack16, const void* add, void* out, int B, int H, int W, int C, void* stream) {
    if (!ctx) return AVX_ERR_INVALID;
    AVX_REQUIRE(ctx, x && wpack16 && out && B > 0 && H > 0 && W > 0, "avx_mst_conv3x3_lds: NULL pointer or empty tensor");
    AVX_REQUIRE(ctx, C == 32, "avx_mst_conv3x3_lds: C=%d (32: the 31-channel full-resolution convs)", C);
    AVX_REQUIRE(ctx, ((((uintptr_t)x | (uintptr_t)wpack16 | (uintptr_t)add | (uintptr_t)out)) & 15u) == 0, "avx_mst_conv3x3_lds: pointers must be 16-byte aligned");
    AVX_REQUIRE(ctx, x != out, "avx_mst_conv3x3_lds: in-place convolution is not possible");
    AVX_HIP(ctx, hipSetDevice(ctx->device));
    hipStream_t s = avx_pick_stream(ctx, stream);
    const long total = (long)B * ((H + TS - 1) / TS) * ((W + TS - 1) / TS);
    const long cap = (long)ctx->num_cus * 3;
    AVX_REQUIRE(ctx, total <= 0x7fffffffl, "avx_mst_conv3x3_lds: 2^31 tiles or more");
    hipLaunchKernelGGL((k_mst_conv3x3_lds<6, false>), dim3((unsigned)(total < cap ? total : cap)), dim3(kFT), 0, s, (const __half*)x, (const uint4*)wpack16, (const __half*)add,
                       (__half*)out, B, H, W, (const uint4*)nullptr, (float*)nullptr, (const float*)nullptr, (float*)nullptr, (SpecStat3*)nullptr, 0, 0, 0, 0, mst_tile_order());
    AVX_HIP(ctx, hipGetLastError());
    return AVX_OK;
}

extern "C" int avx_mst_conv3x3_lds_spectral(avx_ctx* ctx, const void* x, const void* wpack16, const void* add, int H, int W, int C, const float* weights_host, int crop_t,
                                            int crop_l, int Hc, int Wc, float* planes_out, void* partials_out, int* n_partials, void* stream) {
    if (!ctx) return AVX_ERR_INVALID;
    AVX_REQUIRE(ctx, x && wpack16 && weights_host && planes_out && partials_out && n_partials && H > 0 && W > 0, "avx_mst_conv3x3_lds_spectral: NULL pointer or empty tensor");
    AVX_REQUIRE(ctx, C == 32, "avx_mst_conv3x3_lds_spectral: C=%d (32: the 31-band cube as stored)", C);
    AVX_REQUIRE(ctx, crop_t >= 0 && crop_l >= 0 && Hc > 0 && Wc > 0 && crop_t + Hc <= H && crop_l + Wc <= W, "avx_mst_conv3x3_lds_spectral: the crop window must lie inside the frame");
    AVX_REQUIRE(ctx, ((((uintptr_t)x | (uintptr_t)wpack16 | (uintptr_t)add | (uintptr_t)partials_out)) & 15u) == 0, "avx_mst_conv3x3_lds_spectral: pointers must be 16-byte aligned");
    AVX_HIP(ctx, hipSetDevice(ctx->device));
    hipStream_t s = avx_pick_stream(ctx, stream);
    avx_ws* ws = avx_workspace(ctx, s);
    if (!ws) return AVX_ERR_NOMEM;
    float wT[32 * 4];
    for (int b = 0; b < 32; ++b)
        for (int k = 0; k < 4; ++k) wT[b * 4 + k] = k < 3 ? weights_host[(size_t)k * 32 + b] : 0.0f;
    float* dwT = nullptr;
    int rc = avx_const_upload(ctx, ws, 2, wT, sizeof(wT), s, (void**)&dwT);
    if (rc) return rc;
    const long total = (long)((H + TS - 1) / TS) * ((W + TS - 1) / TS);
    const long cap = (long)ctx->num_cus * 2;
    const long blocks = total < cap ? total : cap;
    *n_partials = (int)blocks;
    hipLaunchKernelGGL((k_mst_conv3x3_lds<4, false, true>), dim3((unsigned)blocks), dim3(kFT), 0, s, (const __half*)x, (const uint4*)wpack16, (const __half*)add, (__half*)nullptr, 1, H, W,
                       (const uint4*)nullptr, (float*)nullptr, (const float*)dwT, planes_out, (SpecStat3*)partials_out, crop_t, crop_l, Hc, Wc);
    AVX_HIP(ctx, hipGetLastError());
    return AVX_OK;
}

extern "C" int avx_mst_conv3x3_lds_gram(avx_ctx* ctx, const void* x, const void* wpack16, const void* add, void* out, int H, int W, int C, const void* wqk16, float* gram,
                                        float* nq, float* nk, void* stream) {
    if (!ctx) return AVX_ERR_INVALID;
    AVX_REQUIRE(ctx, x && wpack16 && out && wqk16 && gram && nq && nk && H > 0 && W > 0, "avx_mst_conv3x3_lds_gram: NULL pointer or empty tensor");
    AVX_REQUIRE(ctx, C == 32, "avx_mst_conv3x3_lds_gram: C=%d (32: the 31-channel full-resolution convs)", C);
    AVX_REQUIRE(ctx, ((((uintptr_t)x | (uintptr_t)wpack16 | (uintptr_t)add | (uintptr_t)out | (uintptr_t)wqk16)) & 15u) == 0, "avx_mst_conv3x3_lds_gram: pointers must be 16-byte aligned");
    AVX_REQUIRE(ctx, x != out, "avx_mst_conv3x3_lds_gram: in-place convolution is not possible");
    AVX_HIP(ctx, hipSetDevice(ctx->device));
    hipStream_t s = avx_pick_stream(ctx, stream);
    avx_ws* ws = avx_workspace(ctx, s);
    if (!ws) return AVX_ERR_NOMEM;
    const long total = (long)((H + TS - 1) / TS) * ((W + TS - 1) / TS);
    const long cap = (long)ctx->num_cus * 2;
    const long blocks = total < cap ? total : cap;
    int rc = avx_ensure_scratch(ctx, ws, sizeof(float) * (size_t)blocks * 34 * 32);
    if (rc) return rc;
    float* partial = (float*)ws->d_scratch;
    hipLaunchKernelGGL((k_mst_conv3x3_lds<4, true>), dim3((unsigned)blocks), dim3(kFT), 0, s, (const __half*)x, (const uint4*)wpack16, (const __half*)add, (__half*)out, 1, H, W,
                       (const uint4*)wqk16, partial);
    AVX_HIP(ctx, hipGetLastError());
    return avx_mst_qkv_final_launch(ctx, partial, (int)blocks, 1, gram, nq, nk, s);
}

extern "C" int avx_mst_conv_in_u8(avx_ctx* ctx, const uint8_t* frame_hwc, int H, int W, int pad_top, int pad_bottom, int pad_left, int pad_right,
                                  const float* w_27x32_dev, void* out, void* stream) {
    if (!ctx) return AVX_ERR_INVALID;
    AVX_REQUIRE(ctx, frame_hwc && w_27x32_dev && out && H > 1 && W > 1, "avx_mst_conv_in_u8: NULL pointer or a frame too small to reflect");
    AVX_REQUIRE(ctx, pad_top >= 0 && pad_bottom >= 0 && pad_left >= 0 && pad_right >= 0 && pad_top < H && pad_bottom < H && pad_left < W && pad_right < W,
                "avx_mst_conv_in_u8: reflect padding must be smaller than the frame");
    AVX_REQUIRE(ctx, ((uintptr_t)out & 15u) == 0, "avx_mst_conv_in_u8: out must be 16-byte aligned");
    AVX_HIP(ctx, hipSetDevice(ctx->device));
    hipStream_t s = avx_pick_stream(ctx, stream);
    const int Hp = H + pad_top + pad_bottom, Wp = W + pad_left + pad_right;
    const size_t total = (size_t)Hp * Wp;
    const size_t want = (total + 255) / 256, cap = (size_t)ctx->num_cus * 16;
    if (getenv("AVX_MST_CONV_IN_VALU"))
        hipLaunchKernelGGL(k_mst_conv_in_u8, dim3((unsigned)(want < cap ? want : cap)), dim3(256), 0, s, frame_hwc, w_27x32_dev, (__half*)out, H, W, pad_top, pad_left, Hp, Wp);
    else {
        const size_t wantm = (total + 127) / 128;
        hipLaunchKernelGGL(k_mst_conv_in_u8_mfma, dim3((unsigned)(wantm < cap ? wantm : cap)), dim3(256), 0, s, frame_hwc, w_27x32_dev, (__half*)out, H, W, pad_top,
                           pad_left, Hp, Wp);
    }
    AVX_HIP(ctx, hipGetLastError());
    return AVX_OK;
}

extern "C" int avx_mst_down4x4(avx_ctx* ctx, const void* x, const void* wpack16, void* out, int B, int H, int W, int C, void* stream) {
    if (!ctx) return AVX_ERR_INVALID;
    AVX_REQUIRE(ctx, x && wpack16 && out && B > 0 && H > 0 && W > 0, "avx_mst_down4x4: NULL pointer or empty tensor");
    AVX_REQUIRE(ctx, C == 32 || C == 64, "avx_mst_down4x4: C=%d (32 or 64: the encoder steps 31 -> 62 and 62 -> 124 channels as stored)", C);
    AVX_REQUIRE(ctx, H % 2 == 0 && W % 2 == 0, "avx_mst_down4x4: H and W must be even (the model pads frames to multiples of 8)");
    AVX_REQUIRE(ctx, (long)B * H * W * C * 2 < (1l << 31), "avx_mst_down4x4: input larger than 2 GiB");
    AVX_REQUIRE(ctx, ((((uintptr_t)x | (uintptr_t)wpack16 | (uintptr_t)out)) & 15u) == 0, "avx_mst_down4x4: pointers must be 16-byte aligned");
    AVX_HIP(ctx, hipSetDevice(ctx->device));
    hipStream_t s = avx_pick_stream(ctx, stream);
    const long cap = (long)ctx->num_cus;
    if (C == 32) {
        using G = DownGeo<32>;
        const long total = (long)B * ((H / 2 + G::OH - 1) / G::OH) * ((W / 2 + G::OW - 1) / G::OW);
        hipLaunchKernelGGL(k_mst_down4x4_dma<32>, dim3((unsigned)(total < cap ? total : cap)), dim3(kFT), 0, s, (const __half*)x, (const uint4*)wpack16, (__half*)out, (const void*)ctx->d_zero, B, H, W, mst_tile_order());
    } else {
        using G = DownGeo<64>;
        const long total = (long)B * ((H / 2 + G::OH - 1) / G::OH) * ((W / 2 + G::OW - 1) / G::OW);
        hipLaunchKernelGGL(k_mst_down4x4_dma<64>, dim3((unsigned)(total < cap ? total : cap)), dim3(kFT), 0, s, (const __half*)x, (const uint4*)wpack16, (__half*)out, (const void*)ctx->d_zero, B, H, W, mst_tile_order());
    }
    AVX_HIP(ctx, hipGetLastError());
    return AVX_OK;
}
```

animal-vision_amd/ml/mst_plus_plus.py:

```python
from __future__ import annotations

from typing import Dict, List

import torch
import torch.nn.functional as F

DIM = 31
PAD = 32


def padded(n: int) -> int:
    assert n % DIM == 0
    return n // DIM * PAD


def pad_index(n: int, device=None) -> torch.Tensor:
    i = torch.arange(n, device=device)
    return (i // DIM) * PAD + i % DIM


def pad_channels(t: torch.Tensor, dims) -> torch.Tensor:
    for d in dims:
        n = t.shape[d]
        shape = list(t.shape)
        shape[d] = padded(n)
        out = torch.zeros(shape, dtype=t.dtype, device=t.device)
        out.index_copy_(d, pad_index(n, t.device), t)
        t = out
    return t


def pack_fragments(w_kn: torch.Tensor, transposed: bool) -> torch.Tensor:
    K, N = w_kn.shape
    assert K % 32 == 0 and N % 32 == 0
    dev = w_kn.device
    key = (K, N, transposed, str(dev))
    idx = _FRAG_INDEX.get(key)
    if idx is None:
        lane = torch.arange(64, device=dev)
        c, h = lane % 32, lane // 32
        if transposed:
            c = 16 * ((c % 8) // 4) + 4 * (c // 8) + c % 4
        s = torch.arange(K // 8, device=dev)
        j = torch.arange(4, device=dev)
        k = (h[None, :, None] * (K // 2) + 4 * s[:, None, None] + j[None, None, :])[None]
        col = 32 * torch.arange(N // 32, device=dev)[:, None, None, None] + c[None, None, :, None]
        idx = (k * N + col).contiguous()
        _FRAG_INDEX[key] = idx
    return torch.take(w_kn.contiguous(), idx)


_FRAG_INDEX: Dict[tuple, torch.Tensor] = {}


def pack_fragments16(w_kn: torch.Tensor, halfrow: bool = False) -> torch.Tensor:
    K, N = w_kn.shape
    assert K % 16 == 0 and N % 32 == 0
    dev = w_kn.device
    key = (K, N, "k16h" if halfrow else "k16", str(dev))
    idx = _FRAG_INDEX.get(key)
    if idx is None:
        lane = torch.arange(64, device=dev)
        m, h = lane % 32, lane // 32
        col = 16 * ((m % 8) // 4) + 4 * (m // 8) + m % 4
        s = torch.arange(K // 16, device=dev)
        j = torch.arange(8, device=dev)
        if halfrow:
            k = (8 * s[:, None, None] + (K // 2) * h[None, :, None] + j[None, None, :])[None]
        else:
            k = (16 * s[:, None, None] + 8 * h[None, :, None] + j[None, None, :])[None]
        n = 32 * torch.arange(N // 32, device=dev)[:, None, None, None] + col[None, None, :, None]
        idx = (k * N + n).contiguous()
        _FRAG_INDEX[key] = idx
    return torch.take(w_kn.contiguous(), idx)


def pack_qkv16(wqkv: torch.Tensor) -> torch.Tensor:
    K, N = wqkv.shape
    assert N == 3 * K and K % 32 == 0
    dev = wqkv.device
    key = (K, N, "qkv16", str(dev))
    idx = _FRAG_INDEX.get(key)
    if idx is None:
        lane = torch.arange(64, device=dev)
        m, h = lane % 32, lane // 32
        perm = 16 * ((m % 8) // 4) + 4 * (m // 8) + m % 4
        t = torch.arange(N // 32, device=dev)
        col = 32 * t[:, None] + torch.where(t[:, None] >= 2 * (K // 32), perm[None, :], m[None, :])
        q = torch.arange(K // 16, device=dev)
        j = torch.arange(8, device=dev)
        k = h[None, :, None] * (K // 2) + 8 * q[:, None, None] + j[None, None, :]
        idx = (k[None] * N + col[:, None, :, None]).contiguous()
        _FRAG_INDEX[key] = idx
    return torch.take(wqkv.contiguous(), idx)


def pack_dw_mfma(w: torch.Tensor) -> torch.Tensor:
    ch = w.shape[0]
    assert ch % 8 == 0 and tuple(w.shape[1:]) == (1, 3, 3)
    dev = w.device
    lane = torch.arange(64, device=dev)
    m, q = lane % 16, lane // 16
    s_, c = m // 8, m % 8
    dy = q - s_
    ok = (dy >= 0) & (dy <= 2)
    w8 = w.reshape(ch // 8, 8, 3, 3)
    vals = w8[:, c, dy.clamp(0, 2), :]
    vals = torch.where(ok[None, :, None], vals, torch.zeros_like(vals))
    out = torch.zeros((ch // 8, 3, 64, 8), dtype=w.dtype, device=dev)
    out[:, :, lane, c] = vals.permute(0, 2, 1)
    return out.contiguous()


def pack_dw_smfmac(w: torch.Tensor) -> torch.Tensor:
    ch = w.shape[0]
    assert ch % 8 == 0 and tuple(w.shape[1:]) == (1, 3, 3)
    dev = w.device
    lane = torch.arange(64, device=dev)
    m, qa = lane % 16, lane // 16
    s_, c = m // 8, m % 8
    w8 = w.reshape(ch // 8, 8, 3, 3)
    out = torch.zeros((ch // 8, 3, 64, 8), dtype=w.dtype, device=dev)
    out[:, 1] = pack_dw_mfma(w)[:, 2]
    t = c % 4
    idx = torch.full((64,), 0x4444, dtype=torch.int64, device=dev)
    for hh in range(2):
        r = 2 * (qa % 2) + hh
        dy = r - s_
        ok = (dy >= 0) & (dy <= 2)
        vals = w8[:, c, dy.clamp(0, 2), qa // 2]
        vals = torch.where(ok[None, :], vals, torch.zeros_like(vals))
        e = 4 * hh + 2 * (c // 4) + (t == 3).long()
        out[:, 0, lane, e] = vals
        pair = torch.where(t == 3, 2 | (3 << 2), t | (3 << 2))
        sh = 4 * (2 * hh + c // 4)
        idx = (idx & ~(0xF << sh)) | (pair << sh)
    lo = (((idx & 0xFFFF) ^ 0x8000) - 0x8000).to(torch.int16)
    out.view(torch.int16)[:, 2, :, 0] = lo[None]
    return out.contiguous()


def fold_layernorm(w1_kn: torch.Tensor, gamma: torch.Tensor, beta: torch.Tensor, scale: float) -> torch.Tensor:
    w = w1_kn.float()
    out = w * gamma.float()[:, None]
    out[31, :] = beta.float() @ w
    return (out / scale).contiguous()


def pack_down4x4(w: torch.Tensor) -> torch.Tensor:
    return torch.stack([pack_fragments16(w[:, :, t // 4, t % 4].t().contiguous()) for t in range(16)]).contiguous()


class _AvxOps:

    def __init__(self):
        import os

        self.enabled = os.environ.get("AVX_MST_TORCH_ONLY", "") == ""
        self._mfma = os.environ.get("AVX_MST_NO_MFMA", "") == ""
        self._ffn2 = os.environ.get("AVX_MST_NO_FFN2", "") == ""
        self._posemb = os.environ.get("AVX_MST_NO_POSEMB", "") == ""
        self._conv_lds = os.environ.get("AVX_MST_NO_CONV_LDS", "") == ""
        self._conv_in = os.environ.get("AVX_MST_NO_CONV_IN", "") == ""
        self._upfuse = os.environ.get("AVX_MST_NO_UPFUSE", "") == ""
        self._tail = os.environ.get("AVX_MST_NO_TAIL", "") == ""
        self._tailx = os.environ.get("AVX_MST_NO_TAILX", "") == ""
        self._down = os.environ.get("AVX_MST_NO_DOWN4X4", "") == ""
        self._qkv16 = os.environ.get("AVX_MST_NO_QKV16", "") == ""
        self._convgram = os.environ.get("AVX_MST_NO_CONVGRAM", "") == ""
        self._ffn = os.environ.get("AVX_MST_NO_FFN_FUSED", "") == ""
        self._gelu_pre = None
        self._dwmx = os.environ.get("AVX_MST_NO_DW_MFMA", "") == ""
        self._dwsp = os.environ.get("AVX_MST_NO_DW_SPARSE", "") == ""
        self.DW_SPARSE_FFN_C = (32, 64, 128)
        self.DW_SPARSE_TAIL_C = (32, 64)
        self._specfuse = os.environ.get("AVX_MST_NO_SPEC_FUSE", "") == ""
        self.FFN_FUSED_C = tuple(int(v) for v in os.environ.get("AVX_MST_FFN_FUSED_C", "32,64,128").split(",") if v)
        self._ctx = {}

    def ctx(self, device: torch.device):
        from ..runtime import get_context

        idx = device.index if device.index is not None else torch.cuda.current_device()
        c = get_context(idx)
        if c.device != idx:
            raise RuntimeError(f"libavx context is on device {c.device}, tensor on cuda:{idx} (one process per GPU)")
        return c

    @staticmethod
    def _dt(t: torch.Tensor) -> int:
        if t.dtype == torch.float32:
            return 0
        if t.dtype == torch.float16:
            return 1
        raise TypeError(f"csrc/mst.hip kernels take float32/float16, got {t.dtype}")

    def gram(self, qkv: torch.Tensor, heads: int):
        from .._lib import lib

        b, n, c3 = qkv.shape
        c = c3 // 3
        d = c // heads
        ctx = self.ctx(qkv.device)
        g = torch.empty((b, heads, 32, 32), dtype=torch.float32, device=qkv.device)
        nq = torch.empty((b, c), dtype=torch.float32, device=qkv.device)
        nk = torch.empty((b, c), dtype=torch.float32, device=qkv.device)
        st = torch.cuda.current_stream(qkv.device).cuda_stream
        for i in range(b):
            ctx._check(lib.avx_mst_gram(ctx._h, qkv[i].data_ptr(), self._dt(qkv), n, c, heads, g[i].data_ptr(), nq[i].data_ptr(), nk[i].data_ptr(), st))
        return g[:, :, :d, :d], nq, nk

    def gelu_prescale(self) -> float:
        if self._gelu_pre is None:
            from .. import _lib
            self._gelu_pre = float(_lib.lib.avx_mst_gelu_prescale())
        return self._gelu_pre

    def fused_ok(self, x: torch.Tensor) -> bool:
        return self.enabled and x.is_cuda and x.dtype == torch.float16 and x.shape[-1] in (32, 64, 128) and self._mfma

    def qkv_gram(self, x2: torch.Tensor, wpack: torch.Tensor, heads: int, want_v: bool = True, k16: bool = False):
        from .._lib import lib

        b, n, c = x2.shape
        x2 = x2.contiguous()
        ctx = self.ctx(x2.device)
        v = torch.empty_like(x2) if want_v else None
        g = torch.empty((b, heads, 32, 32), dtype=torch.float32, device=x2.device)
        nq = torch.empty((b, c), dtype=torch.float32, device=x2.device)
        nk = torch.empty((b, c), dtype=torch.float32, device=x2.device)
        st = torch.cuda.current_stream(x2.device).cuda_stream
        fn = lib.avx_mst_qkv_gram16 if k16 else lib.avx_mst_qkv_gram
        for i in range(b):
            ctx._check(fn(ctx._h, x2[i].data_ptr(), wpack.data_ptr(), n, c, v[i].data_ptr() if want_v else None, g[i].data_ptr(), nq[i].data_ptr(), nk[i].data_ptr(), st))
        return v, g, nq, nk

    def ln_gemm_gelu(self, x2: torch.Tensor, gamma: torch.Tensor, beta: torch.Tensor, wpack: torch.Tensor, eps: float = 1e-5) -> torch.Tensor:
        from .._lib import lib

        rows, c = x2.shape
        x2 = x2.contiguous()
        ctx = self.ctx(x2.device)
        out = torch.empty((rows, 4 * c), dtype=torch.float16, device=x2.device)
        ctx._check(lib.avx_mst_ln_gemm_gelu(ctx._h, x2.data_ptr(), gamma.data_ptr(), beta.data_ptr(), eps, wpack.data_ptr(), rows, c, out.data_ptr(),
                                            torch.cuda.current_stream(x2.device).cuda_stream))
        return out

    def convt2x2(self, x: torch.Tensor, wpack: torch.Tensor, bias: torch.Tensor, skip: torch.Tensor = None, wskip: torch.Tensor = None) -> torch.Tensor:
        from .._lib import lib

        b, h, w, c = x.shape
        x = x.contiguous()
        out = torch.empty((b, 2 * h, 2 * w, c // 2), dtype=torch.float16, device=x.device)
        ctx = self.ctx(x.device)
        st = torch.cuda.current_stream(x.device).cuda_stream
        if skip is None:
            ctx._check(lib.avx_mst_convt2x2(ctx._h, x.data_ptr(), wpack.data_ptr(), bias.data_ptr(), out.data_ptr(), b, h, w, c, st))
        else:
            assert skip.is_contiguous() and skip.shape == out.shape
            ctx._check(lib.avx_mst_convt2x2_fuse(ctx._h, x.data_ptr(), wpack.data_ptr(), bias.data_ptr(), skip.data_ptr(), wskip.data_ptr(), out.data_ptr(), b, h, w, c, st))
        return out

    def convt2x2_gram(self, x: torch.Tensor, wpack: torch.Tensor, bias: torch.Tensor, skip: torch.Tensor, wskip: torch.Tensor, wqk16: torch.Tensor):
        from .._lib import lib

        b, h, w, c = x.shape
        assert c == 64 and skip.is_contiguous() and skip.shape == (b, 2 * h, 2 * w, 32)
        x = x.contiguous()
        out = torch.empty((b, 2 * h, 2 * w, 32), dtype=torch.float16, device=x.device)
        g = torch.empty((b, 1, 32, 32), dtype=torch.float32, device=x.device)
        nq = torch.empty((b, 32), dtype=torch.float32, device=x.device)
        nk = torch.empty((b, 32), dtype=torch.float32, device=x.device)
        ctx = self.ctx(x.device)
        st = torch.cuda.current_stream(x.device).cuda_stream
        for i in range(b):
            ctx._check(lib.avx_mst_convt2x2_fuse_gram(ctx._h, x[i].data_ptr(), wpack.data_ptr(), bias.data_ptr(), skip[i].data_ptr(), wskip.data_ptr(), out[i].data_ptr(), h, w, c,
                                                      wqk16.data_ptr(), g[i].data_ptr(), nq[i].data_ptr(), nk[i].data_ptr(), st))
        return out, g, nq, nk

    def posemb(self, v: torch.Tensor, w1_c9: torch.Tensor, w2_c9: torch.Tensor, residual: torch.Tensor = None, bias: torch.Tensor = None) -> torch.Tensor:
        from .._lib import lib

        b, h, w, c = v.shape
        v = v.contiguous()
        residual = residual.contiguous() if residual is not None else None
        out = torch.empty_like(v)
        ctx = self.ctx(v.device)
        ctx._check(lib.avx_mst_posemb(ctx._h, v.data_ptr(), w1_c9.data_ptr(), w2_c9.data_ptr(), residual.data_ptr() if residual is not None else None,
                                      bias.data_ptr() if bias is not None else None, out.data_ptr(), b, h, w, c, torch.cuda.current_stream(v.device).cuda_stream))
        return out

    def conv3x3(self, x: torch.Tensor, wpack: torch.Tensor, add: torch.Tensor = None) -> torch.Tensor:
        from .._lib import lib

        b, h, w, c = x.shape
        x = x.contiguous()
        add = add.contiguous() if add is not None else None
        out = torch.empty_like(x)
        ctx = self.ctx(x.device)
        ctx._check(lib.avx_mst_conv3x3_add(ctx._h, x.data_ptr(), wpack.data_ptr(), add.data_ptr() if add is not None else None, out.data_ptr(), b, h, w, c,
                                           torch.cuda.current_stream(x.device).cuda_stream))
        return out

    def conv_in_u8(self, frame: torch.Tensor, pads, w_27x32: torch.Tensor) -> torch.Tensor:
        from .._lib import lib

        H, W, _ = frame.shape
        t, b, l, r = pads
        frame = frame.contiguous()
        out = torch.empty((1, H + t + b, W + l + r, 32), dtype=torch.float16, device=frame.device)
        ctx = self.ctx(frame.device)
        ctx._check(lib.avx_mst_conv_in_u8(ctx._h, frame.data_ptr(), H, W, t, b, l, r, w_27x32.data_ptr(), out.data_ptr(),
                                          torch.cuda.current_stream(frame.device).cuda_stream))
        return out

    def down4x4(self, x: torch.Tensor, wpack16: torch.Tensor) -> torch.Tensor:
        from .._lib import lib

        b, h, w, c = x.shape
        assert x.is_contiguous() and c in (32, 64) and h % 2 == 0 and w % 2 == 0
        out = torch.empty((b, h // 2, w // 2, 2 * c), dtype=torch.float16, device=x.device)
        ctx = self.ctx(x.device)
        st = torch.cuda.current_stream(x.device).cuda_stream
        per = max(1, (2**31 - 1) // (h * w * c * 2))
        for i in range(0, b, per):
            ctx._check(lib.avx_mst_down4x4(ctx._h, x[i : i + per].data_ptr(), wpack16.data_ptr(), out[i : i + per].data_ptr(), min(per, b - i), h, w, c, st))
        return out

    def conv3x3_lds_gram(self, x: torch.Tensor, wpack16: torch.Tensor, add: torch.Tensor, wqk16: torch.Tensor):
        from .._lib import lib

        b, h, w, c = x.shape
        x = x.contiguous()
        add = add.contiguous() if add is not None else None
        out = torch.empty_like(x)
        g = torch.empty((b, 1, 32, 32), dtype=torch.float32, device=x.device)
        nq = torch.empty((b, c), dtype=torch.float32, device=x.device)
        nk = torch.empty((b, c), dtype=torch.float32, device=x.device)
        ctx = self.ctx(x.device)
        st = torch.cuda.current_stream(x.device).cuda_stream
        for i in range(b):
            ctx._check(lib.avx_mst_conv3x3_lds_gram(ctx._h, x[i].data_ptr(), wpack16.data_ptr(), add[i].data_ptr() if add is not None else None, out[i].data_ptr(), h, w, c,
                                                    wqk16.data_ptr(), g[i].data_ptr(), nq[i].data_ptr(), nk[i].data_ptr(), st))
        return out, g, nq, nk

    def conv3x3_lds_spectral(self, x: torch.Tensor, wpack16: torch.Tensor, add: torch.Tensor, weights, crop):
        import ctypes

        import numpy as np

        from .._lib import lib

        b, h, w, c = x.shape
        assert b == 1 and c == 32 and x.is_contiguous() and (add is None or add.is_contiguous())
        t, l, H, W = crop
        ctx = self.ctx(x.device)
        planes = torch.empty((3, H, W), dtype=torch.float32, device=x.device)
        ncu = torch.cuda.get_device_properties(x.device).multi_processor_count
        partials = torch.empty((ncu * 3, 3, 2), dtype=torch.float64, device=x.device)
        wh = np.ascontiguousarray(weights, dtype=np.float32)
        assert wh.shape == (3, 32)
        n = ctypes.c_int(0)
        ctx._check(lib.avx_mst_conv3x3_lds_spectral(ctx._h, x.data_ptr(), wpack16.data_ptr(), add.data_ptr() if add is not None else None, h, w, c,
                                                    wh.ctypes.data_as(ctypes.POINTER(ctypes.c_float)), t, l, H, W, planes.data_ptr(), partials.data_ptr(), ctypes.byref(n),
                                                    torch.cuda.current_stream(x.device).cuda_stream))
        return planes, partials, int(n.value)

    def conv3x3_lds(self, x: torch.Tensor, wpack16: torch.Tensor, add: torch.Tensor = None) -> torch.Tensor:
        from .._lib import lib

        b, h, w, c = x.shape
        x = x.contiguous()
        add = add.contiguous() if add is not None else None
        out = torch.empty_like(x)
        ctx = self.ctx(x.device)
        ctx._check(lib.avx_mst_conv3x3_lds(ctx._h, x.data_ptr(), wpack16.data_ptr(), add.data_ptr() if add is not None else None, out.data_ptr(), b, h, w, c,
                                           torch.cuda.current_stream(x.device).cuda_stream))
        return out

    def attn_pack(self, gram: torch.Tensor, nq: torch.Tensor, nk: torch.Tensor, rescale: torch.Tensor, wproj_t: torch.Tensor) -> torch.Tensor:
        from .._lib import lib

        c = nq.numel()
        ctx = self.ctx(gram.device)
        out = torch.empty((c // 32, c // 8, 64, 4), dtype=torch.float16, device=gram.device)
        ctx._check(lib.avx_mst_attn_pack(ctx._h, gram.data_ptr(), nq.data_ptr(), nk.data_ptr(), rescale.data_ptr(), wproj_t.data_ptr(), c, out.data_ptr(),
                                         torch.cuda.current_stream(gram.device).cuda_stream))
        return out

    def attn_pack16(self, gram: torch.Tensor, nq: torch.Tensor, nk: torch.Tensor, rescale: torch.Tensor, wproj_t: torch.Tensor) -> torch.Tensor:
        from .._lib import lib

        c = nq.numel()
        ctx = self.ctx(gram.device)
        out = torch.empty((c // 32, c // 16, 64, 8), dtype=torch.float16, device=gram.device)
        ctx._check(lib.avx_mst_attn_pack16(ctx._h, gram.data_ptr(), nq.data_ptr(), nk.data_ptr(), rescale.data_ptr(), wproj_t.data_ptr(), c, out.data_ptr(),
                                           torch.cuda.current_stream(gram.device).cuda_stream))
        return out

    def attn_pack_mx(self, gram: torch.Tensor, nq: torch.Tensor, nk: torch.Tensor, rescale: torch.Tensor, wproj_t: torch.Tensor) -> torch.Tensor:
        from .._lib import lib

        c = nq.numel()
        ctx = self.ctx(gram.device)
        out = torch.empty((c // 8, c // 16, 64, 8), dtype=torch.float16, device=gram.device)
        ctx._check(lib.avx_mst_attn_pack_mx(ctx._h, gram.data_ptr(), nq.data_ptr(), nk.data_ptr(), rescale.data_ptr(), wproj_t.data_ptr(), c, out.data_ptr(),
                                            torch.cuda.current_stream(gram.device).cuda_stream))
        return out

    def attn_tail_mx(self, x: torch.Tensor, wvpack16: torch.Tensor, mpack_mx: torch.Tensor, dw1: torch.Tensor, dw2: torch.Tensor, bias: torch.Tensor,
                     out: torch.Tensor = None, sparse: bool = False) -> torch.Tensor:
        from .._lib import lib

        h, w, c = x.shape
        assert x.is_contiguous()
        out = torch.empty_like(x) if out is None else out
        ctx = self.ctx(x.device)
        fn = lib.avx_mst_attn_tail_sp if sparse else lib.avx_mst_attn_tail_mx
        ctx._check(fn(ctx._h, x.data_ptr(), wvpack16.data_ptr(), mpack_mx.data_ptr(), dw1.data_ptr(), dw2.data_ptr(), bias.data_ptr(),
                      out.data_ptr(), 1, h, w, c, torch.cuda.current_stream(x.device).cuda_stream))
        return out

    def attn_tail(self, v: torch.Tensor, x: torch.Tensor, mpack16: torch.Tensor, taps1: torch.Tensor, taps2: torch.Tensor, bias: torch.Tensor,
                  out: torch.Tensor = None) -> torch.Tensor:
        from .._lib import lib

        h, w, c = v.shape
        assert v.is_contiguous() and x.is_contiguous() and x.shape == v.shape
        out = torch.empty_like(v) if out is None else out
        ctx = self.ctx(v.device)
        ctx._check(lib.avx_mst_attn_tail(ctx._h, v.data_ptr(), x.data_ptr(), mpack16.data_ptr(), taps1.data_ptr(), taps2.data_ptr(), bias.data_ptr(), out.data_ptr(),
                                         1, h, w, c, torch.cuda.current_stream(v.device).cuda_stream))
        return out

    def attn_tail_x(self, x: torch.Tensor, wvpack16: torch.Tensor, mpack16: torch.Tensor, taps1: torch.Tensor, taps2: torch.Tensor, bias: torch.Tensor,
                    out: torch.Tensor = None) -> torch.Tensor:
        from .._lib import lib

        h, w, c = x.shape
        assert x.is_contiguous()
        out = torch.empty_like(x) if out is None else out
        ctx = self.ctx(x.device)
        ctx._check(lib.avx_mst_attn_tail_x(ctx._h, x.data_ptr(), wvpack16.data_ptr(), mpack16.data_ptr(), taps1.data_ptr(), taps2.data_ptr(), bias.data_ptr(),
                                           out.data_ptr(), 1, h, w, c, torch.cuda.current_stream(x.device).cuda_stream))
        return out

    def rowgemm_add(self, a: torch.Tensor, wpack: torch.Tensor, add: torch.Tensor = None, a2: torch.Tensor = None, wpack2: torch.Tensor = None) -> torch.Tensor:
        from .._lib import lib

        rows, c = a.shape
        assert a.is_contiguous() and (add is None or (add.is_contiguous() and add.shape == a.shape)) and (a2 is None or (a2.is_contiguous() and a2.shape == a.shape))
        out = add if add is not None else torch.empty_like(a)
        ctx = self.ctx(a.device)
        ctx._check(lib.avx_mst_rowgemm_add(ctx._h, a.data_ptr(), wpack.data_ptr(), a2.data_ptr() if a2 is not None else None,
                                           wpack2.data_ptr() if a2 is not None else None, add.data_ptr() if add is not None else None, out.data_ptr(), rows, c,
                                           torch.cuda.current_stream(a.device).cuda_stream))
        return out

    def ffn_fused(self, x: torch.Tensor, gamma: torch.Tensor, beta: torch.Tensor, w1p: torch.Tensor, taps: torch.Tensor, w2p: torch.Tensor,
                  eps: float = 1e-5, dwpack: torch.Tensor = None, sparse: bool = False) -> torch.Tensor:
        from .._lib import lib

        b, h, w, c = x.shape
        x = x.contiguous()
        out = torch.empty_like(x)
        ctx = self.ctx(x.device)
        st = torch.cuda.current_stream(x.device).cuda_stream
        if dwpack is not None:
            fn = lib.avx_mst_ffn_fused_sp if sparse else lib.avx_mst_ffn_fused_mx
            ctx._check(fn(ctx._h, x.data_ptr(), gamma.data_ptr(), beta.data_ptr(), eps, w1p.data_ptr(), dwpack.data_ptr(), w2p.data_ptr(), out.data_ptr(), b, h, w, c, st))
        else:
            ctx._check(lib.avx_mst_ffn_fused(ctx._h, x.data_ptr(), gamma.data_ptr(), beta.data_ptr(), eps, w1p.data_ptr(), taps.data_ptr(), w2p.data_ptr(),
                                             out.data_ptr(), b, h, w, c, st))
        return out

    def dw_gemm_add(self, hidden: torch.Tensor, w_c9: torch.Tensor, w2pack: torch.Tensor, x: torch.Tensor) -> torch.Tensor:
        from .._lib import lib

        b, h, w, c = x.shape
        assert hidden.is_contiguous() and x.is_contiguous() and hidden.shape == (b, h, w, 4 * c)
        ctx = self.ctx(x.device)
        ctx._check(lib.avx_mst_dw_gemm_add(ctx._h, hidden.data_ptr(), w_c9.data_ptr(), w2pack.data_ptr(), x.data_ptr(), x.data_ptr(), b, h, w, c,
                                           torch.cuda.current_stream(x.device).cuda_stream))
        return x

    def dwconv(self, x: torch.Tensor, w_c9: torch.Tensor, gelu: bool, residual: torch.Tensor = None, bias: torch.Tensor = None) -> torch.Tensor:
        from .._lib import lib

        b, h, w, c = x.shape
        x = x.contiguous()
        y = torch.empty_like(x)
        ctx = self.ctx(x.device)
        if residual is not None or bias is not None:
            residual = residual.contiguous() if residual is not None else None
            ctx._check(lib.avx_dwconv3x3_nhwc_add(ctx._h, x.data_ptr(), w_c9.data_ptr(), y.data_ptr(), b, h, w, c, 1 if gelu else 0,
                                                  residual.data_ptr() if residual is not None else None, bias.data_ptr() if bias is not None else None,
                                                  torch.cuda.current_stream(x.device).cuda_stream))
            return y
        ctx._check(lib.avx_dwconv3x3_nhwc(ctx._h, x.data_ptr(), w_c9.data_ptr(), y.data_ptr(), self._dt(x), b, h, w, c, 1 if gelu else 0,
                                          torch.cuda.current_stream(x.device).cuda_stream))
        return y

    def layernorm(self, x: torch.Tensor, gamma: torch.Tensor, beta: torch.Tensor, eps: float = 1e-5, group: int = 0, real: int = 0) -> torch.Tensor:
        from .._lib import lib

        c = x.shape[-1]
        x = x.contiguous()
        y = torch.empty_like(x)
        ctx = self.ctx(x.device)
        ctx._check(lib.avx_layernorm_rows_grouped(ctx._h, x.data_ptr(), gamma.data_ptr(), beta.data_ptr(), y.data_ptr(), self._dt(x), x.numel() // c, c, eps,
                                                  group or c, real or c, torch.cuda.current_stream(x.device).cuda_stream))
        return y


_AVX = _AvxOps()


def _msab_keys(prefix: str, dim: int) -> Dict[str, tuple]:
    a, f = f"{prefix}.blocks.0.0", f"{prefix}.blocks.0.1"
    return {
        f"{a}.to_q.weight": (dim, dim), f"{a}.to_k.weight": (dim, dim), f"{a}.to_v.weight": (dim, dim),
        f"{a}.rescale": (dim // DIM, 1, 1), f"{a}.proj.weight": (dim, dim), f"{a}.proj.bias": (dim,),
        f"{a}.pos_emb.0.weight": (dim, 1, 3, 3), f"{a}.pos_emb.2.weight": (dim, 1, 3, 3),
        f"{f}.fn.net.0.weight": (4 * dim, dim, 1, 1), f"{f}.fn.net.2.weight": (4 * dim, 1, 3, 3),
        f"{f}.fn.net.4.weight": (dim, 4 * dim, 1, 1), f"{f}.norm.weight": (dim,), f"{f}.norm.bias": (dim,),
    }


def reference_key_names(stage: int = 3) -> Dict[str, tuple]:
    keys: Dict[str, tuple] = {"conv_in.weight": (DIM, 3, 3, 3)}
    for s in range(stage):
        p = f"body.{s}"
        keys[f"{p}.embedding.weight"] = (DIM, DIM, 3, 3)
        d = DIM
        for i in range(2):
            keys.update(_msab_keys(f"{p}.encoder_layers.{i}.0", d))
            keys[f"{p}.encoder_layers.{i}.1.weight"] = (2 * d, d, 4, 4)
            d *= 2
        keys.update(_msab_keys(f"{p}.bottleneck", d))
        for i in range(2):
            keys[f"{p}.decoder_layers.{i}.0.weight"] = (d, d // 2, 2, 2)
            keys[f"{p}.decoder_layers.{i}.0.bias"] = (d // 2,)
            keys[f"{p}.decoder_layers.{i}.1.weight"] = (d // 2, d, 1, 1)
            keys.update(_msab_keys(f"{p}.decoder_layers.{i}.2", d // 2))
            d //= 2
        keys[f"{p}.mapping.weight"] = (DIM, DIM, 3, 3)
    keys["conv_out.weight"] = (DIM, DIM, 3, 3)
    return keys


class MSTPlusPlus(torch.nn.Module):
    def __init__(self, stage: int = 3):
        super().__init__()
        self.stage = stage
        self._shapes = reference_key_names(stage)
        self.w = torch.nn.ParameterDict({self._pk(k): torch.nn.Parameter(torch.zeros(s), requires_grad=False) for k, s in self._shapes.items()})
        self._prepared: Dict[str, torch.Tensor] = {}
        self.capture_attn = None

    def _capture(self, gram: torch.Tensor, nq: torch.Tensor, nk: torch.Tensor, p: str, heads: int):
        b = gram.shape[0]
        a = gram[:, :, :DIM, :DIM].float() / (nk.reshape(b, heads, PAD, 1)[:, :, :DIM].clamp_min(1e-12) * nq.reshape(b, heads, 1, PAD)[..., :DIM].clamp_min(1e-12))
        a = a * self._p(p + ".rescale").float().reshape(1, heads, 1, 1)
        self.capture_attn.append(a.softmax(dim=-1).cpu())

    @staticmethod
    def _pk(k: str) -> str:
        return k.replace(".", "__")

    def load_reference_state_dict(self, sd: Dict[str, torch.Tensor], strict: bool = True) -> "MSTPlusPlus":
        if "state_dict" in sd and not any(k.endswith(".weight") for k in sd):
            sd = sd["state_dict"]
        sd = {k.replace("module.", "", 1) if k.startswith("module.") else k: v for k, v in sd.items()}
        missing = [k for k in self._shapes if k not in sd]
        extra = [k for k in sd if k not in self._shapes]
        if strict and (missing or extra):
            raise KeyError(f"state_dict mismatch: missing {missing[:3]}..., unexpected {extra[:3]}...")
        with torch.no_grad():
            for k, shape in self._shapes.items():
                if k in sd:
                    t = torch.as_tensor(sd[k])
                    if tuple(t.shape) != tuple(shape):
                        raise ValueError(f"{k}: shape {tuple(t.shape)} != {shape}")
                    self.w[self._pk(k)].copy_(t.to(self.w[self._pk(k)].dtype))
        self._prepared.clear()
        return self

    def reference_state_dict(self) -> Dict[str, torch.Tensor]:
        return {k: self.w[self._pk(k)].detach() for k in self._shapes}

    def init_seeded(self, seed: int = 0) -> "MSTPlusPlus":
        g = torch.Generator().manual_seed(seed)
        with torch.no_grad():
            for k, shape in self._shapes.items():
                p = self.w[self._pk(k)]
                if k.endswith("norm.weight") or k.endswith("rescale"):
                    p.fill_(1.0)
                elif k.endswith("bias"):
                    p.zero_()
                elif len(shape) == 2:
                    p.copy_(torch.randn(shape, generator=g) * 0.02)
                else:
                    fan_in = shape[1] * shape[2] * shape[3]
                    bound = (1.0 / fan_in) ** 0.5
                    p.copy_((torch.rand(shape, generator=g) * 2 - 1) * bound)
        self._prepared.clear()
        return self

    def _p(self, k: str) -> torch.Tensor:
        return self.w[self._pk(k)]

    def _prep(self, name: str, build):
        ref = self._p("conv_in.weight")
        key = f"{name}|{ref.dtype}|{ref.device}"
        t = self._prepared.get(key)
        if t is None:
            t = build()
            self._prepared[key] = t
        return t

    def _w(self, k: str, dims) -> torch.Tensor:
        return self._prep(k + ".pad" + "".join(map(str, dims)), lambda: pad_channels(self._p(k), dims).contiguous())

    def _conv3(self, x: torch.Tensor, key: str, add: torch.Tensor = None) -> torch.Tensor:
        if _AVX.fused_ok(x) and x.shape[-1] == 32 and _AVX._conv_lds:
            wq = self._prep(key + ".frag9k16", lambda: torch.stack([pack_fragments16(self._w(key, (0, 1))[:, :, t // 3, t % 3].t().contiguous()) for t in range(9)]).contiguous())
            return _AVX.conv3x3_lds(x, wq, add)
        if _AVX.fused_ok(x) and x.shape[-1] == 32:
            wp = self._prep(key + ".frag9", lambda: torch.stack([pack_fragments(self._w(key, (0, 1))[:, :, t // 3, t % 3].t().contiguous(), True) for t in range(9)]).contiguous())
            return _AVX.conv3x3(x, wp, add)
        y = self._conv_nhwc(x, self._w(key, (0, 1)), padding=1)
        return y + add if add is not None else y

    def _conv_nhwc(self, x: torch.Tensor, w: torch.Tensor, **kw) -> torch.Tensor:
        y = F.conv2d(x.permute(0, 3, 1, 2), w, **kw)
        return y.permute(0, 2, 3, 1)

    def _ms_msa(self, x: torch.Tensor, p: str, heads: int, pre=None) -> torch.Tensor:
        b, h, w, c = x.shape
        n = h * w
        x2 = x.reshape(b, n, c)
        wqkv = self._prep(p + ".qkv", lambda: torch.cat([self._w(p + ".to_q.weight", (0, 1)), self._w(p + ".to_k.weight", (0, 1)),
                                                         self._w(p + ".to_v.weight", (0, 1))], 0).t().contiguous())
        d = c // heads
        if _AVX.fused_ok(x):
            tailx = _AVX._tail and _AVX._tailx and (c in (32, 64) or (c == 128 and _AVX._dwmx))
            if _AVX._qkv16:
                wpk = self._prep(p + ".qkv.frag16", lambda: pack_qkv16(wqkv))
            else:
                wpk = self._prep(p + ".qkv.frag", lambda: torch.cat([pack_fragments(wqkv[:, : 2 * c], False), pack_fragments(wqkv[:, 2 * c :], True)], 0).contiguous())
            if pre is not None and tailx:
                v, (gram, nq, nk) = None, pre
            else:
                v, gram, nq, nk = _AVX.qkv_gram(x2, wpk, heads, want_v=not tailx, k16=_AVX._qkv16)
            if self.capture_attn is not None:
                self._capture(gram, nq, nk, p, heads)
            resc = self._prep(p + ".rescale32", lambda: self._p(p + ".rescale").float().reshape(heads).contiguous())
            wpt = self._prep(p + ".proj.t32", lambda: self._w(p + ".proj.weight", (0, 1)).t().float().contiguous())
            bias32 = self._prep(p + ".proj.bias32", lambda: self._w(p + ".proj.bias", (0,)).float().contiguous())
            vi = v.reshape(b, h, w, c) if v is not None else None
            if _AVX._tail and (c in (32, 64) or tailx):
                k1, k2 = p + ".pos_emb.0.weight", p + ".pos_emb.2.weight"
                t1 = self._prep(k1 + ".t9h", lambda: self._w(k1, (0,)).reshape(c, 9).t().contiguous())
                t2 = self._prep(k2 + ".t9h", lambda: self._w(k2, (0,)).reshape(c, 9).t().contiguous())
                xc = x.contiguous()
                out = torch.empty_like(xc)
                if tailx and _AVX._dwmx:
                    wv16 = self._prep(p + ".wv.frag16h", lambda: pack_fragments16(wqkv[:, 2 * c :].contiguous(), halfrow=True))
                    gs = _AVX.gelu_prescale()
                    sp = _AVX._dwsp and c in _AVX.DW_SPARSE_TAIL_C
                    pk, tag = (pack_dw_smfmac, ".dwsp") if sp else (pack_dw_mfma, ".dwmx")
                    d1 = self._prep(k1 + f"{tag}/{gs}", lambda: pk((self._w(k1, (0,)).float() / gs).to(x.dtype)))
                    d2 = self._prep(k2 + f"{tag}*{gs}", lambda: pk((self._w(k2, (0,)).float() * gs).to(x.dtype)))
                    for i in range(b):
                        _AVX.attn_tail_mx(xc[i], wv16, _AVX.attn_pack_mx(gram[i], nq[i], nk[i], resc, wpt), d1, d2, bias32, out[i], sparse=sp)
                    return out
                if tailx:
                    wv16 = self._prep(p + ".wv.frag16", lambda: pack_fragments16(wqkv[:, 2 * c :].contiguous()))
                    for i in range(b):
                        _AVX.attn_tail_x(xc[i], wv16, _AVX.attn_pack16(gram[i], nq[i], nk[i], resc, wpt), t1, t2, bias32, out[i])
                    return out
                for i in range(b):
                    _AVX.attn_tail(vi[i], xc[i], _AVX.attn_pack16(gram[i], nq[i], nk[i], resc, wpt), t1, t2, bias32, out[i])
                return out
            if _AVX._posemb:
                k1, k2 = p + ".pos_emb.0.weight", p + ".pos_emb.2.weight"
                w91 = self._prep(k1 + ".c9f32", lambda: self._w(k1, (0,)).reshape(c, 9).float().contiguous())
                w92 = self._prep(k2 + ".c9f32", lambda: self._w(k2, (0,)).reshape(c, 9).float().contiguous())
                pe = _AVX.posemb(vi, w91, w92, x, bias32)
            else:
                pe = self._dw(self._dw(vi, p + ".pos_emb.0.weight", gelu=True), p + ".pos_emb.2.weight", gelu=False, residual=x, bias=bias32)
            for i in range(b):
                _AVX.rowgemm_add(v[i], _AVX.attn_pack(gram[i], nq[i], nk[i], resc, wpt), pe[i].reshape(n, c))
            return pe
        qkv = x2 @ wqkv
        q, k, v = qkv[..., :c], qkv[..., c : 2 * c], qkv[..., 2 * c :]
        if x.is_cuda and _AVX.enabled:
            gram, nq, nk = _AVX.gram(qkv, heads)
            nq = nq.reshape(b, heads, 1, d).clamp_min(1e-12)
            nk = nk.reshape(b, heads, d, 1).clamp_min(1e-12)
        else:
            qh = q.reshape(b, n, heads, d).permute(0, 2, 1, 3)
            kh = k.reshape(b, n, heads, d).permute(0, 2, 1, 3)
            gram = torch.matmul(kh.transpose(-2, -1), qh).float()
            nq = torch.linalg.vector_norm(q.float(), dim=1).reshape(b, heads, 1, d).clamp_min(1e-12)
            nk = torch.linalg.vector_norm(k.float(), dim=1).reshape(b, heads, d, 1).clamp_min(1e-12)
        attn = gram / (nk * nq)
        attn = attn * self._p(p + ".rescale").float().reshape(1, heads, 1, 1)
        attn[..., DIM:] = float("-inf")
        attn = attn.softmax(dim=-1)
        if self.capture_attn is not None:
            self.capture_attn.append(attn[:, :, :DIM, :DIM].float().cpu())
        wp = self._w(p + ".proj.weight", (0, 1))
        wp_h = wp.t().reshape(heads, d, c).float()
        M = torch.matmul(attn.transpose(-2, -1), wp_h.unsqueeze(0)).reshape(b, c, c).to(x.dtype)
        vi = v.reshape(b, h, w, c)
        out_c = torch.baddbmm(self._w(p + ".proj.bias", (0,)).to(x.dtype).reshape(1, 1, c), v, M).reshape(b, h, w, c)
        pe = self._dw(self._dw(vi, p + ".pos_emb.0.weight", gelu=True), p + ".pos_emb.2.weight", gelu=False)
        return out_c + pe + x

    def _dw(self, x: torch.Tensor, key: str, gelu: bool, residual: torch.Tensor = None, bias: torch.Tensor = None) -> torch.Tensor:
        c = x.shape[-1]
        if x.is_cuda and _AVX.enabled:
            w9 = self._prep(key + ".c9f32", lambda: self._w(key, (0,)).reshape(c, 9).float().contiguous())
            return _AVX.dwconv(x, w9, gelu, residual, bias)
        y = self._conv_nhwc(x, self._w(key, (0,)), padding=1, groups=c)
        y = F.gelu(y) if gelu else y
        if residual is not None:
            y = y + residual
        return y + bias.to(y.dtype) if bias is not None else y

    def _ffn(self, x: torch.Tensor, p: str) -> torch.Tensor:
        b, h, w, c = x.shape
        g32 = self._prep(p + ".g32", lambda: self._w(p + ".norm.weight", (0,)).float().contiguous())
        b32 = self._prep(p + ".b32", lambda: self._w(p + ".norm.bias", (0,)).float().contiguous())
        w2 = self._prep(p + ".w2", lambda: self._w(p + ".fn.net.4.weight", (0, 1)).reshape(c, 4 * c).t().contiguous())
        if _AVX.fused_ok(x) and _AVX._ffn and c in _AVX.FFN_FUSED_C:
            key = p + ".fn.net.2.weight"
            if _AVX._dwmx:
                gs = _AVX.gelu_prescale()
                w1s = self._prep(p + f".w1.frag16.ln/{gs}", lambda: pack_fragments16(fold_layernorm(self._w(p + ".fn.net.0.weight", (0, 1)).reshape(4 * c, c).t(), g32, b32, gs).to(x.dtype)))
                w2s = self._prep(p + f".w2.frag16*{gs}", lambda: pack_fragments16((w2.float() * gs).to(x.dtype).contiguous()))
                if _AVX._dwsp and c in _AVX.DW_SPARSE_FFN_C:
                    return _AVX.ffn_fused(x, g32, b32, w1s, None, w2s, dwpack=self._prep(key + ".dwsp", lambda: pack_dw_smfmac(self._w(key, (0,)))), sparse=True)
                return _AVX.ffn_fused(x, g32, b32, w1s, None, w2s, dwpack=self._prep(key + ".dwmx", lambda: pack_dw_mfma(self._w(key, (0,)))))
            w1q = self._prep(p + ".w1.frag16", lambda: pack_fragments16(self._w(p + ".fn.net.0.weight", (0, 1)).reshape(4 * c, c).t().contiguous()))
            w2q = self._prep(p + ".w2.frag16", lambda: pack_fragments16(w2))
            t9 = self._prep(key + ".t9h", lambda: self._w(key, (0,)).reshape(4 * c, 9).t().contiguous())
            return _AVX.ffn_fused(x, g32, b32, w1q, t9, w2q)
        if _AVX.fused_ok(x):
            w1p = self._prep(p + ".w1.frag", lambda: pack_fragments(self._w(p + ".fn.net.0.weight", (0, 1)).reshape(4 * c, c).t().contiguous(), True))
            y = _AVX.ln_gemm_gelu(x.reshape(b * h * w, c), g32, b32, w1p).reshape(b, h, w, 4 * c)
            if c in (32, 64) and x.is_contiguous() and _AVX._ffn2:
                key = p + ".fn.net.2.weight"
                w9 = self._prep(key + ".c9f32", lambda: self._w(key, (0,)).reshape(4 * c, 9).float().contiguous())
                w2p = self._prep(p + ".w2.frag", lambda: pack_fragments(w2, True))
                return _AVX.dw_gemm_add(y, w9, w2p, x)
            y = self._dw(y, p + ".fn.net.2.weight", gelu=True)
            return x.reshape(b * h * w, c).addmm_(y.reshape(b * h * w, 4 * c), w2).reshape(b, h, w, c)
        if x.is_cuda and _AVX.enabled:
            y = _AVX.layernorm(x, g32, b32, group=PAD, real=DIM)
        else:
            real = self._prep(p + ".real", lambda: pad_index(c // PAD * DIM, x.device))
            yr = F.layer_norm(x.float().index_select(-1, real), (real.numel(),), g32.index_select(0, real), b32.index_select(0, real))
            y = torch.zeros_like(x, dtype=torch.float32).index_copy_(-1, real, yr).to(x.dtype)
        w1 = self._prep(p + ".w1", lambda: self._w(p + ".fn.net.0.weight", (0, 1)).reshape(4 * c, c).t().contiguous())
        y = F.gelu(y.reshape(b, h * w, c) @ w1).reshape(b, h, w, 4 * c)
        y = self._dw(y, p + ".fn.net.2.weight", gelu=True)
        return (y.reshape(b, h * w, 4 * c) @ w2).reshape(b, h, w, c) + x

    def _msab(self, x: torch.Tensor, p: str, heads: int, pre=None) -> torch.Tensor:
        x = self._ms_msa(x, p + ".blocks.0.0", heads, pre)
        return self._ffn(x, p + ".blocks.0.1")

    def _mst(self, x: torch.Tensor, p: str) -> torch.Tensor:
        pre = None
        ekey, a0 = p + ".embedding.weight", f"{p}.encoder_layers.0.0.blocks.0.0"
        if _AVX.fused_ok(x) and x.shape[-1] == 32 and _AVX._conv_lds and _AVX._convgram and _AVX._qkv16 and _AVX._tail and _AVX._tailx:
            wq = self._prep(ekey + ".frag9k16", lambda: torch.stack([pack_fragments16(self._w(ekey, (0, 1))[:, :, t // 3, t % 3].t().contiguous()) for t in range(9)]).contiguous())
            wqkv = self._prep(a0 + ".qkv", lambda: torch.cat([self._w(a0 + ".to_q.weight", (0, 1)), self._w(a0 + ".to_k.weight", (0, 1)),
                                                              self._w(a0 + ".to_v.weight", (0, 1))], 0).t().contiguous())
            wqk = self._prep(a0 + ".qkv.frag16", lambda: pack_qkv16(wqkv))
            fea, g, nq, nk = _AVX.conv3x3_lds_gram(x, wq, None, wqk)
            pre = (g, nq, nk)
        else:
            fea = self._conv3(x, ekey)
        skips: List[torch.Tensor] = []
        heads = 1
        for i in range(2):
            fea = self._msab(fea, f"{p}.encoder_layers.{i}.0", heads, pre if i == 0 else None)
            skips.append(fea)
            dkey = f"{p}.encoder_layers.{i}.1.weight"
            if _AVX.fused_ok(fea) and _AVX._down and fea.shape[-1] in (32, 64) and fea.is_contiguous():
                fea = _AVX.down4x4(fea, self._prep(dkey + ".frag16", lambda: pack_down4x4(self._w(dkey, (0, 1)))))
            else:
                fea = self._conv_nhwc(fea, self._w(dkey, (0, 1)), stride=2, padding=1)
            heads *= 2
        fea = self._msab(fea, p + ".bottleneck", heads)
        for i in range(2):
            kw = f"{p}.decoder_layers.{i}.0.weight"
            if _AVX.fused_ok(fea) and fea.shape[-1] in (64, 128) and _AVX._upfuse:
                ch = fea.shape[-1] // 2
                wfk = f"{p}.fuse{i}"
                wf_ = self._prep(wfk, lambda: self._w(f"{p}.decoder_layers.{i}.1.weight", (0, 1)).reshape(ch, 2 * ch).t().contiguous())
                gt = self._prep(kw + ".upfuse4", lambda: torch.stack([pack_fragments((self._w(kw, (0, 1))[:, :, t // 2, t % 2].float() @ wf_[:ch].float()).half().contiguous(), True)
                                                                     for t in range(4)]).contiguous())
                gb = self._prep(kw + ".upfuse.bias", lambda: (self._w(f"{p}.decoder_layers.{i}.0.bias", (0,)).float() @ wf_[:ch].float()).contiguous())
                wbot_ = self._prep(f"{p}.fuse{i}.bot", lambda: pack_fragments(wf_[ch:].contiguous(), True))
                heads //= 2
                a2 = f"{p}.decoder_layers.{i}.2.blocks.0.0"
                if ch == 32 and _AVX._convgram and _AVX._qkv16 and _AVX._tail and _AVX._tailx:
                    wqkv2 = self._prep(a2 + ".qkv", lambda: torch.cat([self._w(a2 + ".to_q.weight", (0, 1)), self._w(a2 + ".to_k.weight", (0, 1)),
                                                                       self._w(a2 + ".to_v.weight", (0, 1))], 0).t().contiguous())
                    wqk2 = self._prep(a2 + ".qkv.frag16", lambda: pack_qkv16(wqkv2))
                    fea, g2, nq2, nk2 = _AVX.convt2x2_gram(fea, gt, gb, skips[1 - i].contiguous(), wbot_, wqk2)
                    fea = self._msab(fea, f"{p}.decoder_layers.{i}.2", heads, (g2, nq2, nk2))
                    continue
                fea = _AVX.convt2x2(fea, gt, gb, skips[1 - i].contiguous(), wbot_)
                fea = self._msab(fea, f"{p}.decoder_layers.{i}.2", heads)
                continue
            if _AVX.fused_ok(fea) and fea.shape[-1] in (64, 128):
                wt = self._prep(kw + ".frag4", lambda: torch.stack([pack_fragments(self._w(kw, (0, 1))[:, :, t // 2, t % 2].contiguous(), True) for t in range(4)]).contiguous())
                bt = self._prep(kw + ".bias32", lambda: self._w(f"{p}.decoder_layers.{i}.0.bias", (0,)).float().contiguous())
                up = _AVX.convt2x2(fea, wt, bt)
            else:
                up = F.conv_transpose2d(fea.permute(0, 3, 1, 2), self._w(kw, (0, 1)), self._w(f"{p}.decoder_layers.{i}.0.bias", (0,)), stride=2).permute(0, 2, 3, 1)
            heads //= 2
            skip = skips[1 - i]
            b, h, w, ch = up.shape
            c2 = 2 * ch
            wf = self._prep(f"{p}.fuse{i}", lambda: self._w(f"{p}.decoder_layers.{i}.1.weight", (0, 1)).reshape(c2 // 2, c2).t().contiguous())
            if _AVX.fused_ok(skip):
                up, skip = up.contiguous(), skip.contiguous()
                wtop = self._prep(f"{p}.fuse{i}.top", lambda: pack_fragments(wf[:ch].contiguous(), True))
                wbot = self._prep(f"{p}.fuse{i}.bot", lambda: pack_fragments(wf[ch:].contiguous(), True))
                fea = _AVX.rowgemm_add(up.reshape(b * h * w, ch), wtop, None, skip.reshape(b * h * w, ch), wbot).reshape(b, h, w, ch)
            else:
                cat = torch.cat([up, skip], dim=-1)
                fea = (cat.reshape(b, h * w, c2) @ wf).reshape(b, h, w, c2 // 2)
            fea = self._msab(fea, f"{p}.decoder_layers.{i}.2", heads)
        return self._conv3(fea, p + ".mapping.weight", add=x)

    @torch.no_grad()
    def forward_from_u8(self, frame: torch.Tensor, pads, spectral=None):
        w27 = self._prep("conv_in.w27x32", lambda: self._w("conv_in.weight", (0,)).permute(2, 3, 1, 0).reshape(27, PAD).float().contiguous())
        x = _AVX.conv_in_u8(frame, pads, w27)
        assert x.shape[1] % 8 == 0 and x.shape[2] % 8 == 0, "pad the frame to a multiple of 8 (predict_torch.py pads to 16)"
        if spectral is None:
            return self._body(x)
        H, W, _ = frame.shape
        return self._body(x, spectral=(spectral, (pads[0], pads[2], H, W)))

    def can_fuse_spectral(self) -> bool:
        return self.can_fuse_conv_in() and _AVX._conv_lds and _AVX._specfuse

    def _body(self, x: torch.Tensor, spectral=None):
        hfe = x
        for s in range(self.stage):
            hfe = self._mst(hfe, f"body.{s}")
        if spectral is not None:
            key = "conv_out.weight"
            wq = self._prep(key + ".frag9k16", lambda: torch.stack([pack_fragments16(self._w(key, (0, 1))[:, :, t // 3, t % 3].t().contiguous()) for t in range(9)]).contiguous())
            return _AVX.conv3x3_lds_spectral(hfe.contiguous(), wq, x.contiguous(), spectral[0], spectral[1])
        return self._conv3(hfe, "conv_out.weight", add=x)

    def can_fuse_conv_in(self) -> bool:
        ref = self._p("conv_in.weight")
        return _AVX.enabled and _AVX._mfma and _AVX._conv_in and ref.is_cuda and ref.dtype == torch.float16

    @torch.no_grad()
    def forward_nhwc(self, x: torch.Tensor) -> torch.Tensor:
        b, c, h_inp, w_inp = x.shape
        pad_h, pad_w = (8 - h_inp % 8) % 8, (8 - w_inp % 8) % 8
        if pad_h or pad_w:
            x = F.pad(x, [0, pad_w, 0, pad_h], mode="reflect")
        x = x.to(self._p("conv_in.weight").dtype).contiguous(memory_format=torch.channels_last).permute(0, 2, 3, 1)
        x = self._conv_nhwc(x, self._w("conv_in.weight", (0,)), padding=1)
        return self._body(x)[:, :h_inp, :w_inp, :]

    @torch.no_grad()
    def forward(self, x: torch.Tensor) -> torch.Tensor:
        return self.forward_nhwc(x)[..., :DIM].permute(0, 3, 1, 2)


def hbm_bytes_per_px(stage: int = 3) -> float:

    def msab(c: int) -> float:
        t = 2.0 * c
        if _AVX._tail and _AVX._tailx and (c in (32, 64) or (c == 128 and _AVX._dwmx)):
            b = t
            b += 2 * t
            return b + ((2 * t) if (_AVX._ffn and c in _AVX.FFN_FUSED_C) else (t + 4 * t + ((4 * t + 2 * t) if _AVX._ffn2 else (4 * t + 4 * t + 4 * t + 2 * t))))
        b = 2 * t
        if _AVX._tail and c in (32, 64):
            b += 3 * t
        else:
            b += (3 * t if _AVX._posemb else 5 * t)
            b += 3 * t
        if _AVX._ffn and c in _AVX.FFN_FUSED_C:
            b += 2 * t
        else:
            b += t + 4 * t
            b += (4 * t + 2 * t) if (c in (32, 64) and _AVX._ffn2) else (4 * t + 4 * t + 4 * t + 2 * t)
        return b

    per_stage = 2 * msab(32) + 2 * msab(64) / 4 + msab(128) / 16
    if _AVX._convgram and _AVX._qkv16 and _AVX._tail and _AVX._tailx and _AVX._conv_lds and _AVX._upfuse:
        per_stage -= 2 * 64.0
    t32, t64, t128 = 64.0, 128.0 / 4, 256.0 / 16
    convs = (2 * t32) + (3 * t32)
    convs += (t32 + t64) + (t64 + t128)
    if _AVX._upfuse:
        convs += (t128 + t64 + t64) + (t64 + t32 + t32)
    else:
        convs += (t128 + t64) + (2 * t64 + t64)
        convs += (t64 + t32) + (2 * t32 + t32)
    head = ((3 + t32) if _AVX._conv_in else (3 + 12) + (12 + t32)) + ((2 * t32 + 12) if (_AVX._specfuse and _AVX._conv_lds and _AVX._conv_in) else 3 * t32)
    return stage * (per_stage + convs) + head
```

include/avx.h:

```cpp
#ifndef AVX_H
#define AVX_H

#include <stddef.h>
#include <stdint.h>

#ifdef __cplusplus
extern "C" {
#endif

#define AVX_ABI_VERSION 1

typedef struct avx_ctx avx_ctx;

typedef enum avx_status {
    AVX_OK = 0,
    AVX_ERR_INVALID = -1,
    AVX_ERR_NO_DEVICE = -2,
    AVX_ERR_HIP = -3,
    AVX_ERR_UNSUPPORTED = -4,
    AVX_ERR_NOMEM = -5
} avx_status;

int avx_abi_version(void);
int avx_device_count(void);
// ... 17 lines not shown

int avx_timer_start(avx_ctx* ctx, void* stream);
int avx_timer_stop(avx_ctx* ctx, void* stream, float* out_ms);

enum { AVX_COLOR_MATRIX = 0, AVX_COLOR_CAT_MERGE = 1 };
enum { AVX_POST_NONE = 0, AVX_POST_GAUSS = 1, AVX_POST_ROWGAIN = 2, AVX_POST_STREAK = 3 };

typedef struct avx_dichromat_desc {
    uint32_t struct_size;
    int32_t color_mode;
    float matrix[9];
    float cat_alpha;
    float cat_beta;
    int32_t post_mode;
    int32_t ksize;
    const double* taps_host;
    const float* row_gain_host;
    int32_t row_gain_clamp;
    int32_t chroma_enable;
    float chroma_keep;
    int32_t variant;
    const float* streak_rows_host;
    int32_t streak_stride;
    int32_t in_f32;
} avx_dichromat_desc;

#define AVX_MAX_KSIZE 33

int avx_dichromat_u8(avx_ctx* ctx, const uint8_t* in_hwc, uint8_t* out_hwc, int n_frames, int H, int W,
                     const avx_dichromat_desc* desc, void* stream);

enum { AVX_LAUNCH_NONE = 0, AVX_LAUNCH_REFERENCE = 1, AVX_LAUNCH_TILED = 2, AVX_LAUNCH_MARCH = 3, AVX_LAUNCH_STREAK = 4 };

typedef struct avx_dichromat_launch_info {
    uint32_t struct_size;
    int32_t family;
    int32_t R;
    int32_t f64;
    int32_t NG;
    int32_t spec;
    int32_t sw, nstrips;
    int32_t ch, nchunks;
    int32_t xcd_remap;
    int32_t narrow;
    int32_t tuned_now;
    int32_t grid;
    int32_t per_cu;
} avx_dichromat_launch_info;

int avx_dichromat_last_launch(avx_ctx* ctx, avx_dichromat_launch_info* out);


int avx_percentile(avx_ctx* ctx, const float* data, size_t n, double q, double* out_host, void* stream);

int avx_spectral_integrate(avx_ctx* ctx, const void* hsi, int layout, int dtype, int H, int W, int B,
                           const float* weights_host, int K, float* out_planes, float* stats_host, void* stream);

int avx_plane_stats(avx_ctx* ctx, const float* planes, int K, size_t n, int adapt, float eps, float* stats_host, void* stream);

int avx_planes_gaussian_blur(avx_ctx* ctx, const float* in, float* out, int K, int H, int W, int ksize,
                             const double* taps_host, int scale_mode, void* stream);
int avx_planes_gaussian_blur_batch(avx_ctx* ctx, const float* in, size_t in_frame_stride, float* out, size_t out_frame_stride,
                                   int n_frames, int K, int H, int W, int ksize, const double* taps_host, int scale_mode,
                                   void* stream);

int avx_streak_planes_f32(avx_ctx* ctx, const float* src_planes, float* dst_planes, int H, int W, const float* rows_host,
                          int stride, void* stream);

int avx_rgb_to_hsi_lobes(avx_ctx* ctx, const void* in_hwc, int in_is_u8, int H, int W, int B, const float* gains_host,
                         float denom, float* out_hwb, void* stream);

enum { AVX_MAP_FALSECOLOR = 0, AVX_MAP_CUSTOM_MATRIX = 1, AVX_MAP_OPPONENT = 2, AVX_MAP_UV_PURPLE_YELLOW = 3, AVX_MAP_FALSECOLOR_UV_MIXED = 4 };
typedef struct avx_honeybee_desc {
    uint32_t struct_size;
    int32_t source;
    float rgb_matrix[9];
    const void* hsi;
    int32_t hsi_layout, hsi_dtype, bands;
    const float* weights_host;
    int32_t adaptation;
    float eps;
    int32_t blur_ksize;
    const double* blur_taps_host;
    int32_t mapping;
    float custom_matrix[9];
    float mixed_alpha;
    int32_t out_float;
    const float* catches;
    const void* catch_partials;
    int32_t n_catch_partials;
} avx_honeybee_desc;

int avx_honeybee_u8(avx_ctx* ctx, const uint8_t* in_hwc, uint8_t* out_hwc, int n_frames, int H, int W,
                    const avx_honeybee_desc* desc, float* debug_planes, void* stream);

int avx_catch_planes_up(avx_ctx* ctx, const float* planes_small, int h, int w, float* planes_out, int H, int W, void* partials_out, int* n_partials,
                        void* stream);


int avx_resize_hwc(avx_ctx* ctx, const void* src, int dtype, int H, int W, int C, void* dst, int Hd, int Wd, int interp, void* stream);

int avx_binocular_warp_u8(avx_ctx* ctx, const uint8_t* in_hwc, int H, int W, const float* xL_host, const float* xR_host, const float* ymap_host,
                          const float* wL_host, const float* wR_host, int Ho, int Wo, float* out_hwc_f32, void* stream);

int avx_cat_wide_u8(avx_ctx* ctx, const uint8_t* in_hwc_u8, uint8_t* out_hwc_u8, int n_frames, int H, int W, const avx_dichromat_desc* desc,
                    const float* d_xL, const float* d_xR, const float* d_ymap, const float* d_wL, const float* d_wR, void* stream);

int avx_center_zoom_u8(avx_ctx* ctx, const uint8_t* in_hwc_u8, uint8_t* out_hwc_u8, int n_frames, int H, int W, int x0, int y0, int cw, int ch,
                       void* stream);

int avx_split_compose_u8(avx_ctx* ctx, const uint8_t* original_hwc, const uint8_t* modified_hwc, uint8_t* out_hwc,
                         int H, int W, int draw_seam, void* stream);

int avx_draw_label_u8(avx_ctx* ctx, uint8_t* img_hwc, int H, int W, const int box_xyxy[4], const float* segments_host, int n_segments,
                      float outline_thickness, float text_thickness, int slot, void* stream);

typedef struct avx_gallery_tile {
    const void* src;
    int32_t dtype;
    int32_t H, W;
    int32_t h, w;
    int32_t seg_offset, seg_count;
} avx_gallery_tile;

int avx_gallery_compose_u8(avx_ctx* ctx, const avx_gallery_tile* tiles_host, int n_tiles, const float* segments_host, int n_segments,
                           int strip_h, int pad, int cols, const int bg_rgb[3], uint8_t* canvas_hwc, int Hc, int Wc, void* stream);

typedef struct avx_wall_layout avx_wall_layout;
int avx_wall_max_tiles(void);
int avx_wall_layout_create(avx_ctx* ctx, int H, int W, int h, int w, int n_tiles, const int* seg_offset, const int* seg_count,
                           const float* segments_host, int n_segments, int strip_h, int pad, int cols, const int bg_rgb[3],
                           avx_wall_layout** out_layout);
int avx_wall_layout_destroy(avx_ctx* ctx, avx_wall_layout* layout);
int avx_wall_canvas_size(const avx_wall_layout* layout, int* Hc, int* Wc);
int avx_wall_layout_info(const avx_wall_layout* layout, int* mode, int* staged, int* piece_px, size_t* lds_bytes);
int avx_wall_compose_u8(avx_ctx* ctx, const avx_wall_layout* layout, const uint8_t* const* src, size_t src_frame_stride, int n_frames,
                        uint8_t* canvas, size_t canvas_frame_stride, void* stream);

enum { AVX_YUV_BT601 = 0, AVX_YUV_BT709 = 1 };
int avx_i420_to_rgb_u8(avx_ctx* ctx, const uint8_t* yuv, uint8_t* rgb_hwc, int n_frames, int H, int W, int matrix, int full_range, void* stream);
int avx_rgb_to_i420_u8(avx_ctx* ctx, const uint8_t* rgb_hwc, uint8_t* yuv, int n_frames, int H, int W, int matrix, int full_range, void* stream);
int avx_yuv_coefficients(int matrix, int full_range, int dec_out[6], int enc_out[10]);

enum avx_pix_fmt {
    AVX_PIX_YUV420P = 0, AVX_PIX_NV12 = 1, AVX_PIX_YUV422P = 2, AVX_PIX_YUV444P = 3, AVX_PIX_GRAY = 4,
    AVX_PIX_YUV420P10LE = 5, AVX_PIX_YUV422P10LE = 6, AVX_PIX_YUV444P10LE = 7, AVX_PIX_P010LE = 8, AVX_PIX_FMT_COUNT = 9
};
size_t avx_yuv_frame_size(int fmt, int H, int W);
int avx_yuv_to_rgb_u8(avx_ctx* ctx, int fmt, const uint8_t* yuv, uint8_t* rgb_hwc, int n_frames, int H, int W, int matrix, int full_range, void* stream);
int avx_rgb_to_yuv_u8(avx_ctx* ctx, int fmt, const uint8_t* rgb_hwc, uint8_t* yuv, int n_frames, int H, int W, int matrix, int full_range, void* stream);
int avx_yuv_coefficients_d(int matrix, int full_range, int depth, int dec_out[6], int enc_out[10]);

enum avx_transfer { AVX_TRANSFER_PQ = 1, AVX_TRANSFER_HLG = 2 };
enum avx_tonemap { AVX_TONEMAP_CLIP = 0, AVX_TONEMAP_MOBIUS = 1 };
int avx_yuv_hdr_to_rgb_u8(avx_ctx* ctx, int fmt, const uint8_t* yuv, uint8_t* rgb_hwc, int n_frames, int H, int W, int full_range, int transfer,
                          int tonemap, double peak_nits, double sdr_white, void* stream);

int avx_yuv_to_rgb_scaled_u8(avx_ctx* ctx, int fmt, const uint8_t* yuv, uint8_t* rgb_hwc, int n_frames, int H, int W, int Hd, int Wd, int matrix,
                             int full_range, void* stream);

int avx_yuv_hdr_to_rgb_scaled_u8(avx_ctx* ctx, int fmt, const uint8_t* yuv, uint8_t* rgb_hwc, int n_frames, int H, int W, int Hd, int Wd,
                                 int full_range, int transfer, int tonemap, double peak_nits, double sdr_white, void* stream);

typedef struct avx_frame_metrics {
    uint32_t abs_hist[3][256];
    double   ssim[3];
} avx_frame_metrics;

int avx_frame_metrics_u8(avx_ctx* ctx, const uint8_t* a_hwc, const uint8_t* b_hwc, int n_frames, int H, int W,
                         int with_ssim, avx_frame_metrics* out_dev, void* stream);

typedef struct avx_plane_metrics_rec {
    uint32_t abs_hist[3][1024];
    double   ssim[3];
} avx_plane_metrics_rec;

int avx_plane_metrics(avx_ctx* ctx, int fmt_a, const uint8_t* a, int fmt_b, const uint8_t* b, int n_frames, int H, int W,
                      int with_ssim, avx_plane_metrics_rec* out_dev, void* stream);

typedef struct avx_ms_ssim_rec {
    double cs[3][5];
    double ssim[3][5];
} avx_ms_ssim_rec;

int avx_frame_metrics_ms_u8(avx_ctx* ctx, const uint8_t* a_hwc, const uint8_t* b_hwc, int n_frames, int H, int W,
                            avx_frame_metrics* out_dev, avx_ms_ssim_rec* ms_out_dev, void* stream);

int avx_remap_linear_planes(avx_ctx* ctx, const float* src_planes, int K, int H, int W, const float* mapx_dev,
                            const float* mapy_dev, float* dst_planes, float border_value, void* stream);

int avx_sobel3_plane(avx_ctx* ctx, const float* plane, int H, int W, float* gx, float* gy, void* stream);

typedef struct avx_mantis_desc {
    uint32_t struct_size;
    int32_t n_bands;
    const float* band_matrix_host;
    const float* band_lut_host;
    int32_t n_wavelengths;
    const float* lobe_gains_host;
    float lobe_denom;
    const float* band_weights_host;
    int32_t pano_new_w;
    int32_t hsi_small_h, hsi_small_w;
    float red_keep;
    float haze, haze_keep, haze_tint[3];
    int32_t pre_soft_ksize; const double* pre_soft_taps_host;
    float cos2_global, sin2_global;
    float orientation_mix, pol_linear_strength, pol_linear_gamma, pol_circular_strength;
    int32_t unsharp_ksize; const double* unsharp_taps_host; float unsharp_amount;
    float barcode_saturation, barcode_opacity, winner_take_most;
    const float* rows_host;
    float scan_row_gain; int32_t scan_ksize; const double* scan_taps_host;
    int32_t periph_ksize; const double* periph_taps_host;
    const float* xx_host; const float* yy_host;
    float periph_radius, periph_softness;
    const float* lin_hwc_in;
    int32_t out_float;
} avx_mantis_desc;

int avx_mantis_u8(avx_ctx* ctx, const uint8_t* in_hwc, uint8_t* out_baseline_hwc, uint8_t* out_hwc, int H, int W,
                  const avx_mantis_desc* desc, void* stream);
int avx_mantis_u8_batch(avx_ctx* ctx, const uint8_t* in_hwc, uint8_t* out_baseline_hwc, uint8_t* out_hwc, int n_frames, int H, int W,
                        const avx_mantis_desc* desc, void* stream);

int avx_uv_front_u8(avx_ctx* ctx, const uint8_t* in_hwc, int H, int W, int pano_new_w, float* lin_hwc_out,
                    uint8_t* baseline_hwc_out, void* stream);
int avx_panorama_warp_f32(avx_ctx* ctx, const float* src_hwc, int H, int W, int new_w, float* dst_hwc, void* stream);
typedef struct avx_band_stack_desc {
    uint32_t struct_size;
    int32_t n_bands;
    const float* band_matrix_host;
    int32_t n_wavelengths;
    const float* lobe_gains_host;
    float lobe_denom;
    const float* band_weights_host;
    int32_t small_h, small_w;
} avx_band_stack_desc;
int avx_band_stack(avx_ctx* ctx, const float* lin_hwc, int H, int W, const avx_band_stack_desc* desc,
                   float* stack_hwk_out, void* stream);
int avx_uv_front_u8_batch(avx_ctx* ctx, const uint8_t* in_hwc, int n_frames, size_t in_frame_stride, int H, int W, int pano_new_w,
                          float* lin_hwc_out, size_t lin_frame_stride, uint8_t* baseline_hwc_out, size_t baseline_frame_stride,
                          void* stream);
int avx_band_stack_batch(avx_ctx* ctx, const float* lin_hwc, int n_frames, size_t lin_frame_stride, int H, int W,
                         const avx_band_stack_desc* desc, float* stack_hwk_out, size_t stack_frame_stride, void* stream);
int avx_percentile_dev(avx_ctx* ctx, const float* data_dev, size_t n, double q, double* out_dev, void* stream);
int avx_percentiles_dev(avx_ctx* ctx, int count, const float* const* data_dev, const size_t* n, const double* q,
                        double* const* out_dev, void* stream);

enum { AVX_EW_MAX_INSN = 384, AVX_EW_MAX_PLANES = 24, AVX_EW_MAX_REGS = 32, AVX_EW_MAX_ACC = 16 };
enum {
    AVX_EW_CONST = 1, AVX_EW_SCALAR, AVX_EW_LOAD, AVX_EW_STORE,
    AVX_EW_ADD, AVX_EW_SUB, AVX_EW_MUL, AVX_EW_DIV, AVX_EW_MIN, AVX_EW_MAX, AVX_EW_POW, AVX_EW_ATAN2,
    AVX_EW_NEG, AVX_EW_ABS, AVX_EW_SQRT, AVX_EW_EXP, AVX_EW_LOG, AVX_EW_SIN, AVX_EW_COS, AVX_EW_FLOOR, AVX_EW_CEIL,
    AVX_EW_CLIP01, AVX_EW_TANH,
    AVX_EW_LT, AVX_EW_LE, AVX_EW_GT, AVX_EW_GE, AVX_EW_EQ, AVX_EW_AND, AVX_EW_OR, AVX_EW_NOT,
    AVX_EW_SELECT,
    AVX_EW_ACCMIN, AVX_EW_ACCMAX, AVX_EW_ACCSUM
};
enum { AVX_EW_OPCODE_MASK = 0x3f, AVX_EW_IMM_A = 0x40, AVX_EW_IMM_B = 0x80 };
enum {
    AVX_EW_PLANE_F32 = 0,
    AVX_EW_PLANE_U8,
    AVX_EW_PLANE_U8_LUT,
    AVX_EW_PLANE_COL,
    AVX_EW_PLANE_ROW,
    AVX_EW_PLANE_U8_ENC
};
enum { AVX_EW_ACC_MIN = 0, AVX_EW_ACC_MAX, AVX_EW_ACC_SUM, AVX_EW_ACC_MEAN };
typedef struct avx_ew_insn { uint8_t op, dst, a, b; uint32_t imm; } avx_ew_insn;
typedef struct avx_ew_plane { void* ptr; int32_t stride; int32_t kind; } avx_ew_plane;
typedef struct avx_ew_program {
    uint32_t struct_size;
    int32_t H, W;
    int32_t n_insn; const avx_ew_insn* insn_host;
    int32_t n_planes; const avx_ew_plane* planes_host;
    int32_t n_acc; const int32_t* acc_host;
    double* scalars_dev; int32_t n_scalars;
} avx_ew_program;
int avx_ew_run(avx_ctx* ctx, const avx_ew_program* program, void* stream);
enum { AVX_EW_MAX_FRAMES = 16 };
int avx_ew_run_batch(avx_ctx* ctx, const avx_ew_program* program, int n_frames, const size_t* plane_frame_stride_bytes_host,
                     size_t scalars_frame_stride, void* stream);
int avx_ew_spec_stats(unsigned long long* hits, unsigned long long* misses);


int avx_mst_gram(avx_ctx* ctx, const void* qkv, int dtype, size_t n_pix, int C, int heads, float* gram, float* nq, float* nk, void* stream);

int avx_mst_qkv_gram(avx_ctx* ctx, const void* x, const void* wpack, size_t n_pix, int C, void* v_out, float* gram, float* nq, float* nk,
                     void* stream);
int avx_mst_qkv_gram16(avx_ctx* ctx, const void* x, const void* wpack16, size_t n_pix, int C, void* v_out, float* gram, float* nq, float* nk,
                       void* stream);
int avx_mst_ln_gemm_gelu(avx_ctx* ctx, const void* x, const float* gamma, const float* beta, float eps, const void* wpack, size_t rows, int C,
                         void* out, void* stream);

int avx_mst_dw_gemm_add(avx_ctx* ctx, const void* hidden, const float* w_c9, const void* w2pack, const void* residual, void* out, int B, int H,
                        int W, int C, void* stream);

int avx_mst_conv_in_u8(avx_ctx* ctx, const uint8_t* frame_hwc, int H, int W, int pad_top, int pad_bottom, int pad_left, int pad_right,
                       const float* w_27x32_dev, void* out, void* stream);

int avx_mst_conv3x3_lds(avx_ctx* ctx, const void* x, const void* wpack16, const void* add, void* out, int B, int H, int W, int C, void* stream);
int avx_mst_conv3x3_lds_gram(avx_ctx* ctx, const void* x, const void* wpack16, const void* add, void* out, int H, int W, int C, const void* wqk16, float* gram,
                             float* nq, float* nk, void* stream);
int avx_mst_convt2x2_fuse_gram(avx_ctx* ctx, const void* x, const void* wpack, const float* bias, const void* skip, const void* wskip, void* out, int H, int W, int C,
                               const void* wqk16, float* gram, float* nq, float* nk, void* stream);
int avx_mst_down4x4(avx_ctx* ctx, const void* x, const void* wpack16, void* out, int B, int H, int W, int C, void* stream);

int avx_mst_attn_pack16(avx_ctx* ctx, const float* gram, const float* nq, const float* nk, const float* rescale, const float* wproj_t, int C, void* mpack,
                        void* stream);
int avx_mst_attn_tail(avx_ctx* ctx, const void* v, const void* x, const void* mpack16, const void* taps1_9xc, const void* taps2_9xc, const float* bias,
                      void* out, int B, int H, int W, int C, void* stream);
int avx_mst_attn_tail_x(avx_ctx* ctx, const void* x, const void* wvpack16, const void* mpack16, const void* taps1_9xc, const void* taps2_9xc,
                        const float* bias, void* out, int B, int H, int W, int C, void* stream);
int avx_mst_attn_tail_mx(avx_ctx* ctx, const void* x, const void* wvpack16, const void* mpack_mx, const void* dw1pack, const void* dw2pack,
                         const float* bias, void* out, int B, int H, int W, int C, void* stream);
int avx_mst_attn_tail_sp(avx_ctx* ctx, const void* x, const void* wvpack16, const void* mpack_mx, const void* dw1pack, const void* dw2pack,
                         const float* bias, void* out, int B, int H, int W, int C, void* stream);
int avx_mst_attn_pack_mx(avx_ctx* ctx, const float* gram, const float* nq, const float* nk, const float* rescale, const float* wproj_t, int C, void* mpack,
                         void* stream);


int avx_mst_conv3x3_lds_spectral(avx_ctx* ctx, const void* x, const void* wpack16, const void* add, int H, int W, int C, const float* weights_host, int crop_t,
                                 int crop_l, int Hc, int Wc, float* planes_out, void* partials_out, int* n_partials, void* stream);

int avx_mst_ffn_fused(avx_ctx* ctx, const void* x, const float* gamma, const float* beta, float eps, const void* w1pack, const void* taps_9xhid,
                      const void* w2pack, void* out, int B, int H, int W, int C, void* stream);
int avx_mst_ffn_fused_mx(avx_ctx* ctx, const void* x, const float* gamma, const float* beta, float eps, const void* w1pack, const void* dwpack,
                         const void* w2pack, void* out, int B, int H, int W, int C, void* stream);
int avx_mst_ffn_fused_sp(avx_ctx* ctx, const void* x, const float* gamma, const float* beta, float eps, const void* w1pack, const void* dwpack,
                         const void* w2pack, void* out, int B, int H, int W, int C, void* stream);
float avx_mst_gelu_prescale(void);

int avx_mst_tile_order(int frames, int ty, int tx, int nwg, int raster, long long* visit, int steps_cap, int* steps_out);

int avx_mst_rowgemm_add(avx_ctx* ctx, const void* a, const void* wpack, const void* a2, const void* wpack2, const void* add, void* out, size_t rows,
                        int C, void* stream);

int avx_mst_attn_pack(avx_ctx* ctx, const float* gram, const float* nq, const float* nk, const float* rescale, const float* wproj_t, int C,
                      void* mpack, void* stream);

int avx_mst_conv3x3_add(avx_ctx* ctx, const void* x, const void* wpack, const void* add, void* out, int B, int H, int W, int C, void* stream);

int avx_mst_posemb(avx_ctx* ctx, const void* v, const float* w1_c9, const float* w2_c9, const void* residual, const float* bias, void* out, int B,
                   int H, int W, int C, void* stream);

int avx_mst_convt2x2(avx_ctx* ctx, const void* x, const void* wpack, const float* bias, void* out, int B, int H, int W, int C, void* stream);
int avx_mst_convt2x2_fuse(avx_ctx* ctx, const void* x, const void* wpack, const float* bias, const void* skip, const void* wskip, void* out, int B, int H,
                          int W, int C, void* stream);

int avx_dwconv3x3_nhwc(avx_ctx* ctx, const void* x, const float* w_c9, void* y, int dtype, int B, int H, int W, int C, int gelu_out, void* stream);
int avx_dwconv3x3_nhwc_add(avx_ctx* ctx, const void* x, const float* w_c9, void* y, int B, int H, int W, int C, int gelu_out,
                           const void* residual, const float* bias, void* stream);

int avx_layernorm_rows(avx_ctx* ctx, const void* x, const float* gamma, const float* beta, void* y, int dtype, size_t rows, int C, float eps, void* stream);
int avx_layernorm_rows_grouped(avx_ctx* ctx, const void* x, const float* gamma, const float* beta, void* y, int dtype, size_t rows, int C, float eps,
                               int group, int real, void* stream);

int avx_get_table(int which, void* dst_host, size_t capacity);

#ifdef __cplusplus
}
#endif
#endif
```

Baseline: 433.5.

## Fuse u8 conv_in into its consumer conv3x3 kernels instead of materializing it

Stops writing the 32-channel f16 conv_in output to memory. The first embedding conv (with gram), the mapping residual add and the conv_out/spectral residual now recompute conv_in on the fly from the raw u8 frame with a small MFMA, either into the LDS input tile or as the residual. This removes one full-resolution kernel plus its 32-channel write and repeated reads, at the cost of redundant conv_in arithmetic on halos, extra LDS and more register pressure in the conv kernels.

New measurement: 440.6 (median of 6 runs). 1.02x the previous value.

```diff
diff --git a/animal-vision_amd/_lib.py b/animal-vision_amd/_lib.py
--- a/animal-vision_amd/_lib.py
+++ b/animal-vision_amd/_lib.py
@@ -335,6 +335,9 @@
     "avx_mst_conv3x3_lds": (_i, [_vp, _vp, _vp, _vp, _vp, _i, _i, _i, _i, _vp]),
     "avx_mst_down4x4": (_i, [_vp, _vp, _vp, _vp, _i, _i, _i, _i, _vp]),
     "avx_mst_conv3x3_lds_gram": (_i, [_vp, _vp, _vp, _vp, _vp, _i, _i, _i, _vp, _vp, _vp, _vp, _vp]),
+    "avx_mst_conv3x3_lds_cin": (_i, [_vp, _vp, _vp, _vp, _i, _i, _i, _i, _i, _i, _vp, _vp, _vp]),
+    "avx_mst_conv3x3_lds_spectral_cin": (_i, [_vp, _vp, _vp, _vp, _i, _i, _i, _i, _i, _i, _vp, _fp, _i, _i, _i, _i, _vp, _vp, ctypes.POINTER(ctypes.c_int), _vp]),
+    "avx_mst_conv3x3_lds_gram_cin": (_i, [_vp, _vp, _i, _i, _i, _i, _i, _i, _vp, _vp, _vp, _vp, _vp, _vp, _vp, _vp]),
     "avx_mst_convt2x2_fuse_gram": (_i, [_vp, _vp, _vp, _vp, _vp, _vp, _vp, _i, _i, _i, _vp, _vp, _vp, _vp, _vp]),
     "avx_mst_attn_pack16": (_i, [_vp, _vp, _vp, _vp, _vp, _vp, _i, _vp, _vp]),
     "avx_mst_attn_pack_mx": (_i, [_vp, _vp, _vp, _vp, _vp, _vp, _i, _vp, _vp]),
diff --git a/animal-vision_amd/csrc/mst_fused.hip b/animal-vision_amd/csrc/mst_fused.hip
--- a/animal-vision_amd/csrc/mst_fused.hip
+++ b/animal-vision_amd/csrc/mst_fused.hip
@@ -940,18 +940,84 @@
 
 
 struct SpecStat3 { float mn, mx; double sum; };
-template <int MINW, bool GRAM, bool SPEC = false>
+
+struct ConvInFrame { const uint8_t* frame; int H, W, pt, pl, Hp, Wp; };
+__device__ __forceinline__ half8_t conv_in_afrag(const float* __restrict__ w , int lane, int s) {
+    const int p = lane & 31, h = lane >> 5;
+    const int col = 16 * ((p % 8) / 4) + 4 * (p / 8) + p % 4;
+    const int tap0 = 5 * h, ntap = 5 - h;
+    half8_t a;
+#pragma unroll
+    for (int j = 0; j < 8; ++j) {
+        const int q = 8 * s + j, k = 3 * tap0 + q;
+        a[j] = q < 3 * ntap ? (_Float16)w[k * 32 + col] : (_Float16)0.f;
+    }
+    return a;
+}
+__device__ __forceinline__ unsigned conv_in_px(const uint8_t* __restrict__ frame, int idx, int last) {
+    const int late = idx == last ? 1 : 0;
+    unsigned v;
+    __builtin_memcpy(&v, frame + (unsigned)(idx * 3 - late), 4);
+    return (late ? v >> 8 : v) & 0xffffffu;
+}
+__device__ __forceinline__ unsigned conv_in_src(const ConvInFrame& f, int yy, int xx, bool want = true) {
+    const bool ok = want && yy >= 0 && yy < f.Hp && xx >= 0 && xx < f.Wp;
+    int sy = (ok ? yy : 0) - f.pt, sx = (ok ? xx : 0) - f.pl;
+    sy = sy < 0 ? -sy : (sy >= f.H ? 2 * (f.H - 1) - sy : sy);
+    sx = sx < 0 ? -sx : (sx >= f.W ? 2 * (f.W - 1) - sx : sx);
+    const unsigned v = conv_in_px(f.frame, sy * f.W + sx, f.H * f.W - 1);
+    return ok ? v : 0u;
+}
+__device__ __forceinline__ void conv_in_fetch(const ConvInFrame& f, int y, int x, int h, unsigned raw[5]) {
+#pragma unroll
+    for (int t = 0; t < 5; ++t) {
+        const int tap = 5 * h + (t < 5 - h ? t : 0);
+        raw[t] = conv_in_src(f, y + tap / 3 - 1, x + tap % 3 - 1, t < 5 - h);
+    }
+}
+__device__ __forceinline__ void conv_in_mfma(const unsigned raw[5], half8_t a0, half8_t a1, uint4 o[2]) {
+    const float inv255 = 1.0f / 255.0f;
+    float v[16];
+    v[15] = 0.f;
+#pragma unroll
+    for (int t = 0; t < 5; ++t)
+#pragma unroll
+        for (int c = 0; c < 3; ++c) v[3 * t + c] = (float)((raw[t] >> (8 * c)) & 0xffu) * inv255;
+    const half8_t b0 = __builtin_bit_cast(half8_t, uint4{pack_f16(v[0], v[1]), pack_f16(v[2], v[3]), pack_f16(v[4], v[5]), pack_f16(v[6], v[7])});
+    const half8_t b1 = __builtin_bit_cast(half8_t, uint4{pack_f16(v[8], v[9]), pack_f16(v[10], v[11]), pack_f16(v[12], v[13]), pack_f16(v[14], v[15])});
+    float16_t d;
+#pragma unroll
+    for (int vv = 0; vv < 16; ++vv) d[vv] = 0.f;
+    d = mfma16(a0, b0, d);
+    d = mfma16(a1, b1, d);
+    unsigned q[8];
+#pragma unroll
+    for (int vv = 0; vv < 8; ++vv) q[vv] = pack_f16(d[2 * vv], d[2 * vv + 1]);
+    o[0] = uint4{q[0], q[1], q[2], q[3]};
+    o[1] = uint4{q[4], q[5], q[6], q[7]};
+}
+
+template <int MINW, bool GRAM, bool SPEC = false, bool CINR = false, bool CINX = false>
 __global__ __launch_bounds__(kFT, MINW) void k_mst_conv3x3_lds(const __half* __restrict__ x , const uint4* __restrict__ wpack ,
                                                                const __half* __restrict__ add , __half* __restrict__ out, int B, int H, int W,
                                                                const uint4* __restrict__ wqk , float* __restrict__ partial ,
                                                                const float* __restrict__ specw = nullptr ,
                                                                float* __restrict__ planes = nullptr , SpecStat3* __restrict__ spart = nullptr ,
-                                                               int crop_t = 0, int crop_l = 0, int Hc = 0, int Wc = 0, int order = AVX_TILE_ORDER_RASTER ) {
-    constexpr int C = 32, PP = C * 2 + 16, RP = (HS * PP + 255) / 256 * 256, NFILL = (HS * HS * 4 + kFT - 1) / kFT;
+                                                               int crop_t = 0, int crop_l = 0, int Hc = 0, int Wc = 0, int order = AVX_TILE_ORDER_RASTER ,
+                                                               ConvInFrame cf = ConvInFrame{nullptr, 0, 0, 0, 0, 0, 0} , const float* __restrict__ cw = nullptr ) {
+    static_assert(!(CINR && CINX), "the frame stands in for the residual or for the input");
+    constexpr bool CIN = CINR || CINX;
+    constexpr int C = 32, PP = C * 2 + 16, RP = (HS * PP + 255) / 256 * 256, NFILL = CINX ? 1 : (HS * HS * 4 + kFT - 1) / kFT;
+    constexpr int SS = HS + 2;
     __shared__ __align__(16) unsigned char xt[HS * RP];
     __shared__ uint4 wl[18 * 64];
+    __shared__ uint4 cwl[CIN ? 2 * 64 : 1];
+    __shared__ unsigned st[CINX ? SS * SS : 1];
     const int tid = threadIdx.x, lane = tid & 63, wave = tid >> 6, p = lane & 31, h = lane >> 5;
     for (int i = tid; i < 18 * 64; i += kFT) wl[i] = wpack[i];
+    if constexpr (CIN) {
+        if (tid < 2 * 64) cwl[tid] = __builtin_bit_cast(uint4, conv_in_afrag(cw, lane, wave));
+    }
     __shared__ uint4 wq[GRAM ? 4 * 64 : 1];
     float16_t G;
     float nq = 0.f, nk = 0.f;
@@ -971,11 +1037,17 @@
         f_rel[k] = (unsigned)(((q / HS) * W + q % HS) * C + 8 * part) * 2u;
     }
     auto fetch = [&](const Tile& t) {
+        int tq = tid;
+        if constexpr (CINR) asm volatile("" : "+v"(tq));
         if (t.y0 >= 1 && t.y0 + HS - 1 <= H && t.x0 >= 1 && t.x0 + HS - 1 <= W) {
             const char* origin = reinterpret_cast<const char*>(x + ((t.b * H + t.y0 - 1) * (size_t)W + t.x0 - 1) * C);
 #pragma unroll
             for (int k = 0; k < NFILL; ++k) {
                 unsigned o = f_rel[k];
+                if constexpr (CINR) {
+                    const int it = tq + k * kFT, itc = it < HS * HS * 4 ? it : 0, q = itc >> 2, part = itc & 3;
+                    o = (unsigned)(((q / HS) * W + q % HS) * C + 8 * part) * 2u;
+                }
                 asm volatile("" : "+v"(o));
                 pre[k] = *reinterpret_cast<const uint4*>(origin + o);
             }
@@ -983,7 +1055,7 @@
         }
 #pragma unroll
         for (int k = 0; k < NFILL; ++k) {
-            const int it = tid + k * kFT, q = it >> 2, part = it & 3;
+            const int it = tq + k * kFT, q = it >> 2, part = it & 3;
             const int yy = t.y0 - 1 + q / HS, xx = t.x0 - 1 + q % HS;
             const bool ok = it < HS * HS * 4 && yy >= 0 && yy < H && xx >= 0 && xx < W;
             const int yc = yy < 0 ? 0 : (yy >= H ? H - 1 : yy), xc = xx < 0 ? 0 : (xx >= W ? W - 1 : xx);
@@ -992,27 +1064,99 @@
             pre[k] = r;
         }
     };
+    unsigned praw = 0u;
+    const int s_i = tid / SS, s_j = tid - s_i * SS;
+    auto fetch_src = [&](const Tile& t) {
+        if (tid >= SS * SS) return;
+        const int sy0 = t.y0 - 2 - cf.pt, sx0 = t.x0 - 2 - cf.pl;
+        if (sy0 >= 0 && sy0 + SS < cf.H && sx0 >= 0 && sx0 + SS <= cf.W) {
+            unsigned v;
+            __builtin_memcpy(&v, cf.frame + (unsigned)(((sy0 + s_i) * cf.W + sx0 + s_j) * 3), 4);
+            praw = v;
+            return;
+        }
+        praw = conv_in_src(cf, t.y0 - 2 + s_i, t.x0 - 2 + s_j);
+    };
+    unsigned rraw[5] = {0u, 0u, 0u, 0u, 0u};
+    auto fetch_res = [&](const Tile& t) {
+        unsigned* raw = rraw;
+        int lq = tid;
+        asm volatile("" : "+v"(lq));
+        const int h = (lq >> 5) & 1, yl = t.y0 + 2 * (lq >> 6) + ((lq >> 4) & 1), xl = t.x0 + (lq & 15);
+        const bool alive = yl < H && xl < W;
+        const int yo = alive ? yl : 0, xo = alive ? xl : 0;
+        const int sy0 = t.y0 - 1 - cf.pt, sx0 = t.x0 - 1 - cf.pl;
+        if (sy0 >= 0 && sy0 + HS < cf.H && sx0 >= 0 && sx0 + HS <= cf.W) {
+            const int at = (yo - cf.pt) * cf.W + xo - cf.pl;
+#pragma unroll
+            for (int k = 0; k < 5; ++k) {
+                const int tap = h ? (k < 4 ? 5 + k : 5) : k;
+                unsigned v;
+                __builtin_memcpy(&v, cf.frame + (unsigned)((at + (tap / 3 - 1) * cf.W + tap % 3 - 1) * 3), 4);
+                raw[k] = v;
+            }
+            return;
+        }
+        conv_in_fetch(cf, yo, xo, h, raw);
+    };
     TileWalk ahead;
     ahead.init(blockIdx.x, gridDim.x, B, ty, tx, (GRAM || SPEC) ? (int)AVX_TILE_ORDER_RASTER : order);
     if (!ahead.live) return;
     Tile t = tile_at(ahead, TS, TS);
     ahead.advance();
-    fetch(t);
+    if constexpr (CINX) fetch_src(t);
+    else fetch(t);
+    if constexpr (CINR) fetch_res(t);
     for (;;) {
-#pragma unroll
-        for (int k = 0; k < NFILL; ++k) {
-            const int it = tid + k * kFT, q = it >> 2, part = it & 3;
-            if (it < HS * HS * 4) *reinterpret_cast<uint4*>(xt + (size_t)(q / HS) * RP + (size_t)(q % HS) * PP + 16 * part) = pre[k];
+        if constexpr (CINX) {
+            if (tid < SS * SS) st[tid] = praw & 0xffffffu;
+            __syncthreads();
+            const half8_t a0 = __builtin_bit_cast(half8_t, cwl[lane]), a1 = __builtin_bit_cast(half8_t, cwl[64 + lane]);
+            for (int g = wave; g < (HS * HS + 31) / 32; g += kFT / 64) {
+                const int q = g * 32 + p, qc = q < HS * HS ? q : 0, hi = qc / HS, hj = qc - hi * HS;
+                unsigned raw[5];
+#pragma unroll
+                for (int k = 0; k < 5; ++k) {
+                    const int o0 = (k / 3) * SS + k % 3, o1 = ((5 + (k < 4 ? k : 0)) / 3) * SS + (5 + (k < 4 ? k : 0)) % 3;
+                    const unsigned v = st[hi * SS + hj + (h ? o1 : o0)];
+                    raw[k] = (h && k == 4) ? 0u : v;
+                }
+                uint4 o[2];
+                conv_in_mfma(raw, a0, a1, o);
+                const int yy = t.y0 - 1 + hi, xx = t.x0 - 1 + hj;
+                if (!(yy >= 0 && yy < H && xx >= 0 && xx < W)) o[0] = o[1] = uint4{0, 0, 0, 0};
+                if (q < HS * HS) {
+                    uint4* dst = reinterpret_cast<uint4*>(xt + (size_t)hi * RP + (size_t)hj * PP + 32 * h);
+                    dst[0] = o[0]; dst[1] = o[1];
+                }
+            }
+        } else {
+#pragma unroll
+            for (int k = 0; k < NFILL; ++k) {
+                const int it = tid + k * kFT, q = it >> 2, part = it & 3;
+                if (it < HS * HS * 4) *reinterpret_cast<uint4*>(xt + (size_t)(q / HS) * RP + (size_t)(q % HS) * PP + 16 * part) = pre[k];
+            }
         }
         __syncthreads();
-        if (ahead.live) fetch(tile_at(ahead, TS, TS));
         {
             const int r = 2 * wave + (p >> 4), c = p & 15;
             const int yo = t.y0 + r, xo = t.x0 + c;
             const bool live = yo < H && xo < W;
+            uint4 ar[2] = {uint4{0, 0, 0, 0}, uint4{0, 0, 0, 0}};
+            if constexpr (CINR) {
+#pragma unroll
+                for (int k = 0; k < 5; ++k) rraw[k] = (h && k == 4) ? 0u : rraw[k] & 0xffffffu;
+                conv_in_mfma(rraw, __builtin_bit_cast(half8_t, cwl[lane]), __builtin_bit_cast(half8_t, cwl[64 + lane]), ar);
+            }
+            if (ahead.live) {
+                if constexpr (CINR) fetch_res(tile_at(ahead, TS, TS));
+                if constexpr (CINX) fetch_src(tile_at(ahead, TS, TS));
+                else fetch(tile_at(ahead, TS, TS));
+            }
             const size_t off = ((t.b * H + (live ? yo : 0)) * (size_t)W + (live ? xo : 0)) * C + 16 * h;
-            uint4 ar[2] = {uint4{0, 0, 0, 0}, uint4{0, 0, 0, 0}};
-            if (add) { ar[0] = reinterpret_cast<const uint4*>(add + off)[0]; ar[1] = reinterpret_cast<const uint4*>(add + off)[1]; }
+            if constexpr (!CIN) {
+                if (add) { ar[0] = reinterpret_cast<const uint4*>(add + off)[0]; ar[1] = reinterpret_cast<const uint4*>(add + off)[1]; }
+            }
             float16_t d;
 #pragma unroll
             for (int v = 0; v < 16; ++v) d[v] = 0.f;
@@ -1332,53 +1476,19 @@
 __global__ __launch_bounds__(256) void k_mst_conv_in_u8_mfma(const uint8_t* __restrict__ frame , const float* __restrict__ w ,
                                                              __half* __restrict__ out , int H, int W, int pt, int pl, int Hp, int Wp) {
     const int lane = threadIdx.x & 63, p = lane & 31, h = lane >> 5;
-    const int col = 16 * ((p % 8) / 4) + 4 * (p / 8) + p % 4;
-    const int tap0 = 5 * h, ntap = 5 - h;
-    half8_t af[2];
-#pragma unroll
-    for (int s = 0; s < 2; ++s)
-#pragma unroll
-        for (int j = 0; j < 8; ++j) {
-            const int q = 8 * s + j, k = 3 * tap0 + q;
-            af[s][j] = q < 3 * ntap ? (_Float16)w[k * 32 + col] : (_Float16)0.f;
-        }
-    int dy[5], dx[5];
-#pragma unroll
-    for (int t = 0; t < 5; ++t) {
-        const int tap = tap0 + (t < ntap ? t : 0);
-        dy[t] = tap / 3 - 1; dx[t] = tap % 3 - 1;
-    }
+    const half8_t a0 = conv_in_afrag(w, lane, 0), a1 = conv_in_afrag(w, lane, 1);
+    const ConvInFrame cf{frame, H, W, pt, pl, Hp, Wp};
     const size_t total = (size_t)Hp * Wp, ngroups = (total + 31) / 32;
-    const float inv255 = 1.0f / 255.0f;
     for (size_t g = (size_t)blockIdx.x * 4 + (threadIdx.x >> 6); g < ngroups; g += (size_t)gridDim.x * 4) {
         const size_t i = g * 32 + p, ic = i < total ? i : total - 1;
         const int y = (int)(ic / Wp), x = (int)(ic - (size_t)y * Wp);
-        float v[16];
-        v[15] = 0.f;
-#pragma unroll
-        for (int t = 0; t < 5; ++t) {
-            const int yy = y + dy[t], xx = x + dx[t];
-            const bool ok = t < ntap && yy >= 0 && yy < Hp && xx >= 0 && xx < Wp;
-            int sy = (ok ? yy : 0) - pt, sx = (ok ? xx : 0) - pl;
-            sy = sy < 0 ? -sy : (sy >= H ? 2 * (H - 1) - sy : sy);
-            sx = sx < 0 ? -sx : (sx >= W ? 2 * (W - 1) - sx : sx);
-            const uint8_t* q = frame + ((size_t)sy * W + sx) * 3;
-#pragma unroll
-            for (int c = 0; c < 3; ++c) v[3 * t + c] = ok ? (float)q[c] * inv255 : 0.f;
-        }
-        const half8_t b0 = __builtin_bit_cast(half8_t, uint4{pack_f16(v[0], v[1]), pack_f16(v[2], v[3]), pack_f16(v[4], v[5]), pack_f16(v[6], v[7])});
-        const half8_t b1 = __builtin_bit_cast(half8_t, uint4{pack_f16(v[8], v[9]), pack_f16(v[10], v[11]), pack_f16(v[12], v[13]), pack_f16(v[14], v[15])});
-        float16_t d;
-#pragma unroll
-        for (int vv = 0; vv < 16; ++vv) d[vv] = 0.f;
-        d = mfma16(af[0], b0, d);
-        d = mfma16(af[1], b1, d);
+        unsigned raw[5];
+        conv_in_fetch(cf, y, x, h, raw);
+        uint4 o[2];
+        conv_in_mfma(raw, a0, a1, o);
         if (i < total) {
-            unsigned o[8];
-#pragma unroll
-            for (int vv = 0; vv < 8; ++vv) o[vv] = pack_f16(d[2 * vv], d[2 * vv + 1]);
-            reinterpret_cast<uint4*>(out + i * 32 + 16 * h)[0] = uint4{o[0], o[1], o[2], o[3]};
-            reinterpret_cast<uint4*>(out + i * 32 + 16 * h)[1] = uint4{o[4], o[5], o[6], o[7]};
+            reinterpret_cast<uint4*>(out + i * 32 + 16 * h)[0] = o[0];
+            reinterpret_cast<uint4*>(out + i * 32 + 16 * h)[1] = o[1];
         }
     }
 }
@@ -1640,6 +1750,91 @@
     return AVX_OK;
 }
 
+static int conv_in_frame_check(avx_ctx* ctx, const char* fn, const uint8_t* frame_hwc, int H, int W, int pad_top, int pad_bottom, int pad_left, int pad_right, const float* w_27x32_dev,
+                               ConvInFrame* cf) {
+    AVX_REQUIRE(ctx, frame_hwc && w_27x32_dev && H > 1 && W > 1, "%s: NULL pointer or a frame too small to reflect", fn);
+    AVX_REQUIRE(ctx, pad_top >= 0 && pad_bottom >= 0 && pad_left >= 0 && pad_right >= 0 && pad_top < H && pad_bottom < H && pad_left < W && pad_right < W,
+                "%s: reflect padding must be smaller than the frame", fn);
+    AVX_REQUIRE(ctx, (long)(H + pad_top + pad_bottom) * (W + pad_left + pad_right) * 3 < (1l << 31), "%s: frame larger than 2 GiB", fn);
+    *cf = ConvInFrame{frame_hwc, H, W, pad_top, pad_left, H + pad_top + pad_bottom, W + pad_left + pad_right};
+    return AVX_OK;
+}
+
+extern "C" int avx_mst_conv3x3_lds_cin(avx_ctx* ctx, const void* x, const void* wpack16, const uint8_t* frame_hwc, int H, int W, int pad_top, int pad_bottom, int pad_left,
+                                       int pad_right, const float* w_27x32_dev, void* out, void* stream) {
+    if (!ctx) return AVX_ERR_INVALID;
+    AVX_REQUIRE(ctx, x && wpack16 && out, "avx_mst_conv3x3_lds_cin: NULL pointer");
+    ConvInFrame cf;
+    int rc = conv_in_frame_check(ctx, "avx_mst_conv3x3_lds_cin", frame_hwc, H, W, pad_top, pad_bottom, pad_left, pad_right, w_27x32_dev, &cf);
+    if (rc) return rc;
+    AVX_REQUIRE(ctx, ((((uintptr_t)x | (uintptr_t)wpack16 | (uintptr_t)out)) & 15u) == 0, "avx_mst_conv3x3_lds_cin: pointers must be 16-byte aligned");
+    AVX_REQUIRE(ctx, x != out, "avx_mst_conv3x3_lds_cin: in-place convolution is not possible");
+    AVX_HIP(ctx, hipSetDevice(ctx->device));
+    hipStream_t s = avx_pick_stream(ctx, stream);
+    const long total = (long)((cf.Hp + TS - 1) / TS) * ((cf.Wp + TS - 1) / TS);
+    const long cap = (long)ctx->num_cus * 3;
+    hipLaunchKernelGGL((k_mst_conv3x3_lds<6, false, false, true>), dim3((unsigned)(total < cap ? total : cap)), dim3(kFT), 0, s, (const __half*)x, (const uint4*)wpack16, (const __half*)nullptr,
+                       (__half*)out, 1, cf.Hp, cf.Wp, (const uint4*)nullptr, (float*)nullptr, (const float*)nullptr, (float*)nullptr, (SpecStat3*)nullptr, 0, 0, 0, 0, mst_tile_order(), cf,
+                       w_27x32_dev);
+    AVX_HIP(ctx, hipGetLastError());
+    return AVX_OK;
+}
+
+extern "C" int avx_mst_conv3x3_lds_spectral_cin(avx_ctx* ctx, const void* x, const void* wpack16, const uint8_t* frame_hwc, int H, int W, int pad_top, int pad_bottom, int pad_left,
+                                                int pad_right, const float* w_27x32_dev, const float* weights_host, int crop_t, int crop_l, int Hc, int Wc, float* planes_out,
+                                                void* partials_out, int* n_partials, void* stream) {
+    if (!ctx) return AVX_ERR_INVALID;
+    AVX_REQUIRE(ctx, x && wpack16 && weights_host && planes_out && partials_out && n_partials, "avx_mst_conv3x3_lds_spectral_cin: NULL pointer");
+    ConvInFrame cf;
+    int rc = conv_in_frame_check(ctx, "avx_mst_conv3x3_lds_spectral_cin", frame_hwc, H, W, pad_top, pad_bottom, pad_left, pad_right, w_27x32_dev, &cf);
+    if (rc) return rc;
+    AVX_REQUIRE(ctx, crop_t >= 0 && crop_l >= 0 && Hc > 0 && Wc > 0 && crop_t + Hc <= cf.Hp && crop_l + Wc <= cf.Wp, "avx_mst_conv3x3_lds_spectral_cin: the crop window must lie inside the padded frame");
+    AVX_REQUIRE(ctx, ((((uintptr_t)x | (uintptr_t)wpack16 | (uintptr_t)partials_out)) & 15u) == 0, "avx_mst_conv3x3_lds_spectral_cin: pointers must be 16-byte aligned");
+    AVX_HIP(ctx, hipSetDevice(ctx->device));
+    hipStream_t s = avx_pick_stream(ctx, stream);
+    avx_ws* ws = avx_workspace(ctx, s);
+    if (!ws) return AVX_ERR_NOMEM;
+    float wT[32 * 4];
+    for (int b = 0; b < 32; ++b)
+        for (int k = 0; k < 4; ++k) wT[b * 4 + k] = k < 3 ? weights_host[(size_t)k * 32 + b] : 0.0f;
+    float* dwT = nullptr;
+    rc = avx_const_upload(ctx, ws, 2, wT, sizeof(wT), s, (void**)&dwT);
+    if (rc) return rc;
+    const long total = (long)((cf.Hp + TS - 1) / TS) * ((cf.Wp + TS - 1) / TS);
+    const long cap = (long)ctx->num_cus * 2;
+    const long blocks = total < cap ? total : cap;
+    *n_partials = (int)blocks;
+    hipLaunchKernelGGL((k_mst_conv3x3_lds<4, false, true, true>), dim3((unsigned)blocks), dim3(kFT), 0, s, (const __half*)x, (const uint4*)wpack16, (const __half*)nullptr, (__half*)nullptr, 1,
+                       cf.Hp, cf.Wp, (const uint4*)nullptr, (float*)nullptr, (const float*)dwT, planes_out, (SpecStat3*)partials_out, crop_t, crop_l, Hc, Wc, (int)AVX_TILE_ORDER_RASTER, cf,
+                       w_27x32_dev);
+    AVX_HIP(ctx, hipGetLastError());
+    return AVX_OK;
+}
+
+extern "C" int avx_mst_conv3x3_lds_gram_cin(avx_ctx* ctx, const uint8_t* frame_hwc, int H, int W, int pad_top, int pad_bottom, int pad_left, int pad_right, const float* w_27x32_dev,
+                                            const void* wpack16, void* out, const void* wqk16, float* gram, float* nq, float* nk, void* stream) {
+    if (!ctx) return AVX_ERR_INVALID;
+    AVX_REQUIRE(ctx, wpack16 && out && wqk16 && gram && nq && nk, "avx_mst_conv3x3_lds_gram_cin: NULL pointer");
+    ConvInFrame cf;
+    int rc = conv_in_frame_check(ctx, "avx_mst_conv3x3_lds_gram_cin", frame_hwc, H, W, pad_top, pad_bottom, pad_left, pad_right, w_27x32_dev, &cf);
+    if (rc) return rc;
+    AVX_REQUIRE(ctx, ((((uintptr_t)wpack16 | (uintptr_t)out | (uintptr_t)wqk16)) & 15u) == 0, "avx_mst_conv3x3_lds_gram_cin: pointers must be 16-byte aligned");
+    AVX_HIP(ctx, hipSetDevice(ctx->device));
+    hipStream_t s = avx_pick_stream(ctx, stream);
+    avx_ws* ws = avx_workspace(ctx, s);
+    if (!ws) return AVX_ERR_NOMEM;
+    const long total = (long)((cf.Hp + TS - 1) / TS) * ((cf.Wp + TS - 1) / TS);
+    const long cap = (long)ctx->num_cus * 2;
+    const long blocks = total < cap ? total : cap;
+    rc = avx_ensure_scratch(ctx, ws, sizeof(float) * (size_t)blocks * 34 * 32);
+    if (rc) return rc;
+    float* partial = (float*)ws->d_scratch;
+    hipLaunchKernelGGL((k_mst_conv3x3_lds<4, true, false, false, true>), dim3((unsigned)blocks), dim3(kFT), 0, s, (const __half*)nullptr, (const uint4*)wpack16, (const __half*)nullptr, (__half*)out, 1,
+                       cf.Hp, cf.Wp, (const uint4*)wqk16, partial, (const float*)nullptr, (float*)nullptr, (SpecStat3*)nullptr, 0, 0, 0, 0, (int)AVX_TILE_ORDER_RASTER, cf, w_27x32_dev);
+    AVX_HIP(ctx, hipGetLastError());
+    return avx_mst_qkv_final_launch(ctx, partial, (int)blocks, 1, gram, nq, nk, s);
+}
+
 extern "C" int avx_mst_down4x4(avx_ctx* ctx, const void* x, const void* wpack16, void* out, int B, int H, int W, int C, void* stream) {
     if (!ctx) return AVX_ERR_INVALID;
     AVX_REQUIRE(ctx, x && wpack16 && out && B > 0 && H > 0 && W > 0, "avx_mst_down4x4: NULL pointer or empty tensor");
diff --git a/animal-vision_amd/ml/mst_plus_plus.py b/animal-vision_amd/ml/mst_plus_plus.py
--- a/animal-vision_amd/ml/mst_plus_plus.py
+++ b/animal-vision_amd/ml/mst_plus_plus.py
@@ -175,6 +175,7 @@
         self.DW_SPARSE_FFN_C = (32, 64, 128)
         self.DW_SPARSE_TAIL_C = (32, 64)
         self._specfuse = os.environ.get("AVX_MST_NO_SPEC_FUSE", "") == ""
+        self._cinfuse = os.environ.get("AVX_MST_NO_CONV_IN_FUSE", "") == ""
         self.FFN_FUSED_C = tuple(int(v) for v in os.environ.get("AVX_MST_FFN_FUSED_C", "32,64,128").split(",") if v)
         self._ctx = {}
 
@@ -351,6 +352,8 @@
 
         from .._lib import lib
 
+        if isinstance(add, tuple):
+            return self.conv3x3_lds_spectral_cin(x, wpack16, add, weights, crop)
         b, h, w, c = x.shape
         assert b == 1 and c == 32 and x.is_contiguous() and (add is None or add.is_contiguous())
         t, l, H, W = crop
@@ -364,6 +367,58 @@
         ctx._check(lib.avx_mst_conv3x3_lds_spectral(ctx._h, x.data_ptr(), wpack16.data_ptr(), add.data_ptr() if add is not None else None, h, w, c,
                                                     wh.ctypes.data_as(ctypes.POINTER(ctypes.c_float)), t, l, H, W, planes.data_ptr(), partials.data_ptr(), ctypes.byref(n),
                                                     torch.cuda.current_stream(x.device).cuda_stream))
+        return planes, partials, int(n.value)
+
+    def conv3x3_lds_gram_cin(self, src, wpack16: torch.Tensor, wqk16: torch.Tensor):
+        from .._lib import lib
+
+        frame, (t, b, l, r), w27 = src
+        H, W, _ = frame.shape
+        frame = frame.contiguous()
+        out = torch.empty((1, H + t + b, W + l + r, 32), dtype=torch.float16, device=frame.device)
+        g = torch.empty((1, 1, 32, 32), dtype=torch.float32, device=frame.device)
+        nq = torch.empty((1, 32), dtype=torch.float32, device=frame.device)
+        nk = torch.empty((1, 32), dtype=torch.float32, device=frame.device)
+        ctx = self.ctx(frame.device)
+        ctx._check(lib.avx_mst_conv3x3_lds_gram_cin(ctx._h, frame.data_ptr(), H, W, t, b, l, r, w27.data_ptr(), wpack16.data_ptr(), out.data_ptr(), wqk16.data_ptr(),
+                                                    g.data_ptr(), nq.data_ptr(), nk.data_ptr(), torch.cuda.current_stream(frame.device).cuda_stream))
+        return out, g, nq, nk
+
+    def conv3x3_lds_cin(self, x: torch.Tensor, wpack16: torch.Tensor, src) -> torch.Tensor:
+        from .._lib import lib
+
+        frame, (t, b, l, r), w27 = src
+        H, W, _ = frame.shape
+        assert x.shape == (1, H + t + b, W + l + r, 32)
+        x, frame = x.contiguous(), frame.contiguous()
+        out = torch.empty_like(x)
+        ctx = self.ctx(x.device)
+        ctx._check(lib.avx_mst_conv3x3_lds_cin(ctx._h, x.data_ptr(), wpack16.data_ptr(), frame.data_ptr(), H, W, t, b, l, r, w27.data_ptr(), out.data_ptr(),
+                                               torch.cuda.current_stream(x.device).cuda_stream))
+        return out
+
+    def conv3x3_lds_spectral_cin(self, x: torch.Tensor, wpack16: torch.Tensor, src, weights, crop):
+        import ctypes
+
+        import numpy as np
+
+        from .._lib import lib
+
+        frame, (t, b, l, r), w27 = src
+        H, W, _ = frame.shape
+        assert x.shape == (1, H + t + b, W + l + r, 32) and x.is_contiguous()
+        frame = frame.contiguous()
+        ct, cl, Hc, Wc = crop
+        ctx = self.ctx(x.device)
+        planes = torch.empty((3, Hc, Wc), dtype=torch.float32, device=x.device)
+        ncu = torch.cuda.get_device_properties(x.device).multi_processor_count
+        partials = torch.empty((ncu * 3, 3, 2), dtype=torch.float64, device=x.device)
+        wh = np.ascontiguousarray(weights, dtype=np.float32)
+        assert wh.shape == (3, 32)
+        n = ctypes.c_int(0)
+        ctx._check(lib.avx_mst_conv3x3_lds_spectral_cin(ctx._h, x.data_ptr(), wpack16.data_ptr(), frame.data_ptr(), H, W, t, b, l, r, w27.data_ptr(),
+                                                        wh.ctypes.data_as(ctypes.POINTER(ctypes.c_float)), ct, cl, Hc, Wc, planes.data_ptr(), partials.data_ptr(), ctypes.byref(n),
+                                                        torch.cuda.current_stream(x.device).cuda_stream))
         return planes, partials, int(n.value)
 
     def conv3x3_lds(self, x: torch.Tensor, wpack16: torch.Tensor, add: torch.Tensor = None) -> torch.Tensor:
@@ -773,15 +828,15 @@
         x = self._ms_msa(x, p + ".blocks.0.0", heads, pre)
         return self._ffn(x, p + ".blocks.0.1")
 
-    def _mst(self, x: torch.Tensor, p: str) -> torch.Tensor:
+    def _mst(self, x: torch.Tensor, p: str, src=None) -> torch.Tensor:
         pre = None
         ekey, a0 = p + ".embedding.weight", f"{p}.encoder_layers.0.0.blocks.0.0"
-        if _AVX.fused_ok(x) and x.shape[-1] == 32 and _AVX._conv_lds and _AVX._convgram and _AVX._qkv16 and _AVX._tail and _AVX._tailx:
+        if src is not None or (_AVX.fused_ok(x) and x.shape[-1] == 32 and _AVX._conv_lds and _AVX._convgram and _AVX._qkv16 and _AVX._tail and _AVX._tailx):
             wq = self._prep(ekey + ".frag9k16", lambda: torch.stack([pack_fragments16(self._w(ekey, (0, 1))[:, :, t // 3, t % 3].t().contiguous()) for t in range(9)]).contiguous())
             wqkv = self._prep(a0 + ".qkv", lambda: torch.cat([self._w(a0 + ".to_q.weight", (0, 1)), self._w(a0 + ".to_k.weight", (0, 1)),
                                                               self._w(a0 + ".to_v.weight", (0, 1))], 0).t().contiguous())
             wqk = self._prep(a0 + ".qkv.frag16", lambda: pack_qkv16(wqkv))
-            fea, g, nq, nk = _AVX.conv3x3_lds_gram(x, wq, None, wqk)
+            fea, g, nq, nk = _AVX.conv3x3_lds_gram(x, wq, None, wqk) if src is None else _AVX.conv3x3_lds_gram_cin(src, wq, wqk)
             pre = (g, nq, nk)
         else:
             fea = self._conv3(x, ekey)
@@ -839,30 +894,39 @@
                 cat = torch.cat([up, skip], dim=-1)
                 fea = (cat.reshape(b, h * w, c2) @ wf).reshape(b, h, w, c2 // 2)
             fea = self._msab(fea, f"{p}.decoder_layers.{i}.2", heads)
+        if src is not None:
+            return _AVX.conv3x3_lds_cin(fea, self._frag9k16(p + ".mapping.weight"), src)
         return self._conv3(fea, p + ".mapping.weight", add=x)
 
     @torch.no_grad()
     def forward_from_u8(self, frame: torch.Tensor, pads, spectral=None):
         w27 = self._prep("conv_in.w27x32", lambda: self._w("conv_in.weight", (0,)).permute(2, 3, 1, 0).reshape(27, PAD).float().contiguous())
-        x = _AVX.conv_in_u8(frame, pads, w27)
-        assert x.shape[1] % 8 == 0 and x.shape[2] % 8 == 0, "pad the frame to a multiple of 8 (predict_torch.py pads to 16)"
-        if spectral is None:
-            return self._body(x)
         H, W, _ = frame.shape
-        return self._body(x, spectral=(spectral, (pads[0], pads[2], H, W)))
+        assert (H + pads[0] + pads[1]) % 8 == 0 and (W + pads[2] + pads[3]) % 8 == 0, "pad the frame to a multiple of 8 (predict_torch.py pads to 16)"
+        spec = None if spectral is None else (spectral, (pads[0], pads[2], H, W))
+        if self.can_fuse_conv_in_consumers():
+            return self._body(None, spectral=spec, src=(frame, tuple(pads), w27))
+        return self._body(_AVX.conv_in_u8(frame, pads, w27), spectral=spec)
+
+    def can_fuse_conv_in_consumers(self) -> bool:
+        return (self.can_fuse_conv_in() and self.stage >= 1 and _AVX._cinfuse and _AVX._conv_lds and _AVX._convgram and _AVX._qkv16 and _AVX._tail and _AVX._tailx)
 
     def can_fuse_spectral(self) -> bool:
         return self.can_fuse_conv_in() and _AVX._conv_lds and _AVX._specfuse
 
-    def _body(self, x: torch.Tensor, spectral=None):
+    def _frag9k16(self, key: str) -> torch.Tensor:
+        return self._prep(key + ".frag9k16", lambda: torch.stack([pack_fragments16(self._w(key, (0, 1))[:, :, t // 3, t % 3].t().contiguous()) for t in range(9)]).contiguous())
+
+    def _body(self, x: torch.Tensor, spectral=None, src=None):
         hfe = x
         for s in range(self.stage):
-            hfe = self._mst(hfe, f"body.{s}")
+            hfe = self._mst(hfe, f"body.{s}", src if s == 0 else None)
+        key = "conv_out.weight"
         if spectral is not None:
-            key = "conv_out.weight"
-            wq = self._prep(key + ".frag9k16", lambda: torch.stack([pack_fragments16(self._w(key, (0, 1))[:, :, t // 3, t % 3].t().contiguous()) for t in range(9)]).contiguous())
-            return _AVX.conv3x3_lds_spectral(hfe.contiguous(), wq, x.contiguous(), spectral[0], spectral[1])
-        return self._conv3(hfe, "conv_out.weight", add=x)
+            return _AVX.conv3x3_lds_spectral(hfe.contiguous(), self._frag9k16(key), src if src is not None else x.contiguous(), spectral[0], spectral[1])
+        if src is not None:
+            return _AVX.conv3x3_lds_cin(hfe, self._frag9k16(key), src)
+        return self._conv3(hfe, key, add=x)
 
     def can_fuse_conv_in(self) -> bool:
         ref = self._p("conv_in.weight")
@@ -916,4 +980,6 @@
         convs += (t128 + t64) + (2 * t64 + t64)
         convs += (t64 + t32) + (2 * t32 + t32)
     head = ((3 + t32) if _AVX._conv_in else (3 + 12) + (12 + t32)) + ((2 * t32 + 12) if (_AVX._specfuse and _AVX._conv_lds and _AVX._conv_in) else 3 * t32)
+    if stage >= 1 and _AVX._cinfuse and _AVX._conv_in and _AVX._conv_lds and _AVX._convgram and _AVX._qkv16 and _AVX._tail and _AVX._tailx:
+        head += 3 * 3 - (4 * t32 + 3)
     return stage * (per_stage + convs) + head
diff --git a/include/avx.h b/include/avx.h
--- a/include/avx.h
+++ b/include/avx.h
@@ -343,6 +343,13 @@
 int avx_mst_conv3x3_lds(avx_ctx* ctx, const void* x, const void* wpack16, const void* add, void* out, int B, int H, int W, int C, void* stream);
 int avx_mst_conv3x3_lds_gram(avx_ctx* ctx, const void* x, const void* wpack16, const void* add, void* out, int H, int W, int C, const void* wqk16, float* gram,
                              float* nq, float* nk, void* stream);
+int avx_mst_conv3x3_lds_cin(avx_ctx* ctx, const void* x, const void* wpack16, const uint8_t* frame_hwc, int H, int W, int pad_top, int pad_bottom, int pad_left, int pad_right,
+                            const float* w_27x32_dev, void* out, void* stream);
+int avx_mst_conv3x3_lds_spectral_cin(avx_ctx* ctx, const void* x, const void* wpack16, const uint8_t* frame_hwc, int H, int W, int pad_top, int pad_bottom, int pad_left,
+                                     int pad_right, const float* w_27x32_dev, const float* weights_host, int crop_t, int crop_l, int Hc, int Wc, float* planes_out,
+                                     void* partials_out, int* n_partials, void* stream);
+int avx_mst_conv3x3_lds_gram_cin(avx_ctx* ctx, const uint8_t* frame_hwc, int H, int W, int pad_top, int pad_bottom, int pad_left, int pad_right, const float* w_27x32_dev,
+                                 const void* wpack16, void* out, const void* wqk16, float* gram, float* nq, float* nk, void* stream);
 int avx_mst_convt2x2_fuse_gram(avx_ctx* ctx, const void* x, const void* wpack, const float* bias, const void* skip, const void* wskip, void* out, int H, int W, int C,
                                const void* wqk16, float* gram, float* nq, float* nk, void* stream);
 int avx_mst_down4x4(avx_ctx* ctx, const void* x, const void* wpack16, void* out, int B, int H, int W, int C, void* stream);
```
